# enyen/dppo

Measured on AMD Instinct MI355X. Metric: PPO-update samples/sec (+ env-steps/sec of the K=20 sampler), hopper K=20 n_envs=512, higher is better.
Workload: dtype bf16; 1 GPU; hopper-medium-v2 ft_ppo_diffusion_mlp K=20 Kft=10 Ta=4 (BASELINE configs[1]); n_envs_per_gpu=512, minibatch_per_gpu=50000, rollout_rows_per_gpu=256000, parallelism=dp1 (env-sharded, RCCL grad all-reduce)

## Files before the change

### dppo_amd/csrc/api.hip

```cpp
#include <math.h>
#include <stdarg.h>
#include <stdio.h>
#include <string.h>

#include "fused.h"
#include "gemm.h"
#include "ppo.h"
#include "gaussian.h"
#include "gmm.h"
#include "idql.h"
#include "unet.h"
#include "sampler.h"

using namespace dppo;

static thread_local char g_err[512] = "";
static int fail(int code, const char* fmt, ...) {
  va_list ap;
  va_start(ap, fmt);
  vsnprintf(g_err, sizeof(g_err), fmt, ap);
  va_end(ap);
  return code;
}
namespace dppo {
// ... 321 lines not shown
  void* a1[MAX_BLOCKS];
  void* z1[MAX_BLOCKS];
  void* a2[MAX_BLOCKS];
  void* hpre[MAX_BLOCKS + 1];
  void* hE;
  float* out;
  int ldout;
  void* d_out;
  void* dh;
  void* dz1;
  float* dtemb;
  void* cin;
  void* ca;
  void* cz;
  void* d_enc;
  void* d_cz;
  void* dh_all[MAX_BLOCKS + 1];
  void* dz1_all[MAX_BLOCKS];
  float* ln_stats;
  const void* dh0_final;
  void* w0T;
  float* dobs;
  float* tile_colsum;
  int tiles;
  float* slab;
  size_t slab_used;
  SlabJobs slab_jobs;
  GemmTNGroup tn_group;
  BwdRoute route;
  hipStream_t join_s[2];
  int join_idx[2], n_join;
  float* part;
  float* lowrank;
  float* lowrank_u;
  double* post_counter;
  unsigned* tail_counter;
  size_t slab_floats, part_floats;
};

constexpr int REDUCE_BLOCKS = 256;
constexpr int POST_COUNTER_DOUBLES = 2;

static bool lowrank_top(const dppo_net_desc& d, int64_t M);
template <class P>
static int plan_route(const dppo_net_desc& d, int64_t M, int Kft, int flags, MlpBufs<P>& B);

static int g_dbg = 0;
template <class P>
static void carve_mlp(Carver& c, const dppo_net_desc& d, int64_t M, bool keep, bool bwd, MlpBufs<P>& B) {
  const size_t ES = P::ESIZE;
  const int H = d.hidden, nb = d.n_blocks;
  const int Kp0 = row_kp0(d), Kpo = round_up(d.out_dim, 64);
  memset(&B, 0, sizeof(B));
  BwdRoute& R = B.route;
  R.onehot_col = -1, R.lowrank = lowrank_top(d, M);
  R.one_block = fused_bwd_one_block<P>(d) && d.out_dim <= 128 && R.lowrank;
  R.merged = fused_ok<P>(d) && fused_can_merge<P>(d);
  R.fused = fused_ok<P>(d) && M > 0 && fused_rows_per_tile<P>(d, R.one_block) > 0;
  B.in = c.take((size_t)M * Kp0 * ES);
  const int nh = keep ? nb + 1 : (nb > 0 ? 2 : 1);
  float* hbuf[MAX_BLOCKS + 1];
  for (int i = 0; i < nh; ++i) hbuf[i] = (float*)c.take((size_t)M * H * 4);
  for (int b = 0; b <= nb; ++b) B.h[b] = keep ? hbuf[b] : hbuf[b & 1];
  void* a1s = nullptr;
  void* a2s = nullptr;
  for (int b = 0; b < nb; ++b) {
    if (keep || b == 0) {
      a1s = c.take((size_t)M * H * ES);
      a2s = c.take((size_t)M * H * ES);
    } else if (d.plain) {
      a2s = b == 1 ? c.take((size_t)M * H * ES) : B.a2[b - 2];
    }
    B.a1[b] = a1s;
    B.a2[b] = a2s;
    B.z1[b] = keep ? c.take((size_t)M * H * ES) : nullptr;
  }
  if (d.cond_hidden > 0) {
    const int Kpc = round_up(d.cond_dim, 64), C1p = round_up(d.cond_hidden, 64), Ep = round_up(d.cond_out, 64);
    B.cin = c.take((size_t)M * Kpc * ES);
    B.ca = c.take((size_t)M * C1p * ES);
    B.cz = keep ? c.take((size_t)M * C1p * ES) : nullptr;
    if (bwd) {
      B.d_enc = c.take((size_t)M * Ep * ES);
      B.d_cz = c.take((size_t)M * C1p * ES);
    }
  }
  if (d.use_layernorm && keep) B.ln_stats = (float*)c.take((size_t)nb * 2 * M * 2 * 4);
  B.hE = c.take((size_t)M * H * ES);
  for (int b = 0; b <= nb; ++b) B.hpre[b] = b == nb ? B.hE : (keep ? c.take((size_t)M * H * ES) : nullptr);
  B.ldout = round_up(d.out_dim, 16);
  B.out = (float*)c.take((size_t)M * B.ldout * 4);
  if (bwd) {
    B.d_out = c.take((size_t)M * Kpo * ES);
    B.dh = c.take((size_t)M * H * ES);
    B.dz1 = c.take((size_t)M * H * ES);
    B.dh_all[nb] = B.dh;
    for (int b = 0; b < nb; ++b) {
      B.dh_all[b] = c.take((size_t)M * H * ES);
      B.dz1_all[b] = b == 0 ? B.dz1 : c.take((size_t)M * H * ES);
    }
    const int mt = d.plain || d.out_dim > 128 ? 0 : fused_rows_per_tile<P>(d, R.one_block);
    B.tiles = mt > 0 ? (int)((M + mt - 1) / mt) : 0;
    B.tile_colsum = (float*)c.take((size_t)(2 * nb + 2 + (d.use_layernorm ? 4 * nb : 0)) * (B.tiles > 0 ? B.tiles : 1) * H * 4);
    const int tdp = round_up(d.time_dim > 0 ? d.time_dim : 1, 16);
    B.dtemb = d.kind == 0 ? (float*)c.take((size_t)M * tdp * 4) : nullptr;
    const size_t tiles_hh = (size_t)((H + 127) / 128) * ((H + 127) / 128);
    size_t splits_hh = (512 + tiles_hh - 1) / tiles_hh;
    const size_t alt = (size_t)128 * H * (size_t)(Kp0 > 128 ? Kp0 : 128);
    B.slab_floats = (size_t)2 * (nb > 0 ? nb : 1) * splits_hh * (size_t)H * H + 2 * alt;
    B.slab = (float*)c.take(B.slab_floats * 4);
    B.slab_used = 0, B.slab_jobs.n = 0, B.tn_group.n = 0, B.n_join = 0;
    B.part_floats = (size_t)REDUCE_BLOCKS * (H > 1024 ? H : 1024);
    B.part = (float*)c.take(B.part_floats * 4);
    B.lowrank = (float*)c.take((size_t)round_up(d.out_dim, 16) * H * 4);
    B.lowrank_u = (float*)c.take((size_t)round_up(d.out_dim, 16) * Kp0 * 4);
    B.post_counter = (double*)c.take(POST_COUNTER_DOUBLES * 8);
    B.tail_counter = (unsigned*)(B.post_counter + 1);
    B.w0T = c.take((size_t)round_up(d.cond_dim > 0 ? d.cond_dim : 1, 16) * H * ES);
    B.dobs = (float*)c.take((size_t)M * round_up(d.cond_dim > 0 ? d.cond_dim : 1, 16) * 4);
    plan_route<P>(d, M, 0, 0, B);
  }
}

static void fill_bias_off(const dppo_net_desc& d, const ParamLayout& pl, int* off) {
  off[0] = (int)pl.b0;
  for (int b = 0; b < d.n_blocks; ++b) off[1 + 2 * b] = (int)pl.l1b[b], off[2 + 2 * b] = (int)pl.l2b[b];
  off[1 + 2 * d.n_blocks] = (int)pl.bout;
}
static void fill_ln_off(const dppo_net_desc& d, const ParamLayout& pl, int* off) {
  for (int b = 0; b < d.n_blocks; ++b)
    off[4 * b] = (int)pl.n1w[b], off[4 * b + 1] = (int)pl.n1b[b], off[4 * b + 2] = (int)pl.n2w[b], off[4 * b + 3] = (int)pl.n2b[b];
}

template <class P>
static void cond_encode(const dppo_net_desc& d, const float* prm, const char* pk, const PackLayout& L, int64_t M,
                        const void* cin, MlpBufs<P>& B, void* in, float* enc_f32, int ld_enc, bool keep, hipStream_t s) {
  const ParamLayout pl = param_layout(d);
  GemmNT g;
  memset(&g, 0, sizeof(g));
  g.M = (int)M, g.N = d.cond_hidden, g.Kp = L.Kpc, g.ldx = L.Kpc, g.ldw = L.Kpc, g.ldo = L.C1p, g.act = d.act;
  g.X = cin, g.W = pk + L.Wc1, g.bias = prm + pl.c1b, g.out_act = B.ca, g.out_pre = keep ? B.cz : nullptr;
  launch_gemm_nt<P>(g, s);
  if (L.C1p > round_up(d.cond_hidden, 16)) launch_zero_cols<P>(B.ca, (int)M, round_up(d.cond_hidden, 16), L.C1p, L.C1p, s);
  memset(&g, 0, sizeof(g));
  g.M = (int)M, g.N = d.cond_out, g.Kp = L.C1p, g.ldx = L.C1p, g.ldw = L.C1p;
  g.X = B.ca, g.W = pk + L.Wc2, g.bias = prm + pl.c2b;
  if (in != nullptr) g.out_pre = (char*)in + (size_t)(d.act_flat + d.time_dim) * P::ESIZE, g.ldo = L.Kp0;
  if (enc_f32 != nullptr) g.out_f32 = enc_f32, g.ldo32 = ld_enc;
  launch_gemm_nt<P>(g, s);
}

template <class P>
static void mlp_forward(const dppo_net_desc& d, const float* prm, const char* pk, const PackLayout& L, int64_t M,
                        MlpBufs<P>& B, bool keep, hipStream_t s) {
  const ParamLayout pl = param_layout(d);
  const int H = d.hidden, nb = d.n_blocks;
  if (fused_ok<P>(d)) {
    FusedFwdArgs f;
    memset(&f, 0, sizeof(f));
    f.wstream = (const u32x4*)(pk + L.sstream), f.ostream = (const u32x4*)(pk + L.ostream), f.params = prm;
    fill_bias_off(d, pl, f.bias_off);
    f.in = B.in, f.ld_in = L.Kp0, f.M = (int)M, f.Kp0 = sampler_geom<P>(d).Kp0, f.nb = nb, f.act = d.act;
    f.out_dim = d.out_dim, f.out = B.out, f.ldout = B.ldout, f.in_valid = d.in_dim;
    f.use_ln = d.use_layernorm;
    if (d.use_layernorm) fill_ln_off(d, pl, f.ln_off);
    if (keep) {
      for (int b = 0; b < nb; ++b) {
        f.a1[b] = B.a1[b], f.a2[b] = B.a2[b];
        f.z1[b] = B.z1[b], f.hpre[b] = B.hpre[b];
      }
      f.hpre[nb] = B.hE;
      f.ln_stats = d.use_layernorm ? B.ln_stats : nullptr;
    }
    if (B.route.merged) {
      f.merge_top = 1, f.ks0v = (d.in_dim + P::KB - 1) / P::KB, f.hpre[nb] = nullptr;
      if (g_dbg & 64) f.hpre[0] = nullptr;
      if (g_dbg & 128) f.a2[0] = nullptr;
      if (g_dbg & 256) f.z1[0] = nullptr;
      f.ostream0 = (const u32x4*)(pk + L.ostream0), f.ostream2 = (const u32x4*)(pk + L.ostream2);
      f.cbias2 = (const float*)(pk + L.cbias2);
    }
    g_fused_fault = launch_fused_forward<P>(d, f, s);
    return;
  }
  if (d.plain) {
    GemmNT q;
    memset(&q, 0, sizeof(q));
    q.M = (int)M, q.X = B.in, q.ldx = L.Kp0, q.W = pk + L.W0, q.ldw = L.Kp0, q.Kp = L.Kp0, q.N = H, q.bias = prm + pl.b0;
    q.ldo = H, q.act = d.act, q.out_act = B.a1[0], q.out_pre = keep ? B.hpre[0] : nullptr;
    launch_gemm_nt<P>(q, s);
    for (int b = 0; b < nb; ++b) {
      memset(&q, 0, sizeof(q));
      q.M = (int)M, q.N = H, q.Kp = H, q.ldx = H, q.ldw = H, q.ldo = H, q.act = d.act;
      q.X = b == 0 ? B.a1[0] : B.a2[b - 1], q.W = pk + L.W1[b], q.bias = prm + pl.l1b[b];
      q.out_pre = keep ? B.z1[b] : nullptr, q.out_act = B.a2[b];
      launch_gemm_nt<P>(q, s);
    }
    memset(&q, 0, sizeof(q));
    q.M = (int)M, q.N = d.out_dim, q.Kp = H, q.ldx = H, q.ldw = H;
    q.X = B.a2[nb - 1], q.W = pk + L.Wout, q.bias = prm + pl.bout, q.out_f32 = B.out, q.ldo32 = B.ldout;
    launch_gemm_nt<P>(q, s);
    return;
  }
  GemmNT g;
  memset(&g, 0, sizeof(g));
  g.M = (int)M;
  g.X = B.in, g.ldx = L.Kp0, g.W = pk + L.W0, g.ldw = L.Kp0, g.Kp = L.Kp0, g.N = H, g.bias = prm + pl.b0;
  g.out_f32 = B.h[0], g.ldo32 = H, g.ldo = H, g.act = d.act;
  g.out_act = nb > 0 ? B.a1[0] : nullptr;
  g.out_pre = nb > 0 ? nullptr : B.hE;
  launch_gemm_nt<P>(g, s);
  for (int b = 0; b < nb; ++b) {
    memset(&g, 0, sizeof(g));
    g.M = (int)M, g.N = H, g.Kp = H, g.ldx = H, g.ldw = H, g.ldo = H, g.ldo32 = H, g.act = d.act;
    g.X = B.a1[b], g.W = pk + L.W1[b], g.bias = prm + pl.l1b[b];
    g.out_pre = keep ? B.z1[b] : nullptr, g.out_act = B.a2[b];
    launch_gemm_nt<P>(g, s);
    g.X = B.a2[b], g.W = pk + L.W2[b], g.bias = prm + pl.l2b[b];
    g.res = B.h[b], g.ldres = H;
    g.out_f32 = B.h[b + 1];
    g.out_act = b + 1 < nb ? B.a1[b + 1] : nullptr;
    g.out_pre = b + 1 < nb ? nullptr : B.hE;
    launch_gemm_nt<P>(g, s);
  }
  memset(&g, 0, sizeof(g));
  g.M = (int)M, g.N = d.out_dim, g.Kp = H, g.ldx = H, g.ldw = H;
  g.X = B.hE, g.W = pk + L.Wout, g.bias = prm + pl.bout, g.out_f32 = B.out, g.ldo32 = B.ldout;
  launch_gemm_nt<P>(g, s);
}

static int g_overlap = 1;
struct SideStream {
  hipStream_t s = nullptr;
  hipEvent_t fork = nullptr, join = nullptr;
  bool ok = false;
};
static SideStream* side_stream(int idx) {
  static SideStream tab[16][3];
  int dev = 0;
  if (hipGetDevice(&dev) != hipSuccess || dev < 0 || dev >= 16) return nullptr;
  SideStream& t = tab[dev][idx];
  if (!t.ok) {
    if (hipStreamCreateWithFlags(&t.s, hipStreamNonBlocking) != hipSuccess) return nullptr;
    if (hipEventCreateWithFlags(&t.fork, hipEventDisableTiming) != hipSuccess) return nullptr;
    if (hipEventCreateWithFlags(&t.join, hipEventDisableTiming) != hipSuccess) return nullptr;
    t.ok = true;
  }
  return &t;
}
static hipStream_t fork_side(hipStream_t main, int idx = 0) {
  const int mask = g_overlap == 1 ? 7 : g_overlap >> 1;
  SideStream* t = ((mask >> idx) & 1) ? side_stream(idx) : nullptr;
  if (t == nullptr) return main;
  (void)hipEventRecord(t->fork, main);
  (void)hipStreamWaitEvent(t->s, t->fork, 0);
  return t->s;
}
static void join_side(hipStream_t main, hipStream_t sidestream, int idx = 0) {
  if (sidestream == main) return;
  SideStream* t = side_stream(idx);
  (void)hipEventRecord(t->join, sidestream);
  (void)hipStreamWaitEvent(main, t->join, 0);
}

static int g_post_one = 1;
static int g_merge_top = 1;
static int g_lowrank_top = 1;
static int g_early_join = 1;
static int g_tn_group = 1;
static int g_tn_target = 256;
static int g_tn_max_splits = 128;
static int g_lowrank_ratio = 100;
static bool lowrank_top(const dppo_net_desc& d, int64_t M) {
  return g_lowrank_top && d.n_blocks >= 1 && M >= (int64_t)g_lowrank_ratio * d.out_dim;
}
static int g_mom_rider = 0;
constexpr int64_t MOM_RIDER_MAX_N = 16384;
static int g_temb_onehot = 1;
static int g_dw0 = 1;
static int g_side_tail = 1;
static int g_tail_post = 1;
template <class P>
static int plan_route(const dppo_net_desc& d, int64_t M, int Kft, int flags, MlpBufs<P>& B) {
  BwdRoute& R = B.route;
  const bool zeroed = flags & DPPO_ROUTE_IN_ZEROED, wants_dobs = flags & DPPO_ROUTE_IN_DOBS;
  const int Kp0 = row_kp0(d);
  const bool side = flags & DPPO_ROUTE_IN_SIDE;
  const bool oh = g_temb_onehot && d.kind == 0 && fused_ok<P>(d) && Kft >= 1 && !(d.cond_out > 0 && d.cond_out % 16) &&
                  Kp0 - d.in_dim >= Kft && (size_t)(d.hidden + d.time_dim) * Kft <= B.part_floats;
  R.onehot_col = oh ? d.in_dim : -1;
  const int room = 32 - (d.kind == 0 ? d.act_flat + d.cond_dim : d.in_dim);
  const int nhot = d.kind != 0 ? 0 : (room >= Kft ? Kft : room);
  R.dw0 = g_dw0 && P::ESIZE == 2 && zeroed && !wants_dobs && d.cond_hidden <= 0 && g_tn_group && g_post_one && R.fused &&
          R.one_block && fused_dw0_shape(d) && Kp0 >= 64 &&
          (size_t)fused_bwd_one_grid<P>(d, M) * d.hidden * 32 <= B.slab_floats / 2;
  if (d.kind == 0)
    R.dw0 = R.dw0 && oh && d.in_dim == d.act_flat + d.time_dim + d.cond_dim && d.act_flat % 4 == 0 && d.time_dim % 4 == 0 &&
            32 + d.time_dim <= 64 && nhot >= Kft - 1;
  else
    R.dw0 = R.dw0 && d.in_dim <= 32;
  if (R.dw0 && (g_dbg & 33))
    return fail(-1, "tuning knob 8, bits 0 and 5 (values 1 and 32: no dh_0 store) cannot run with the in-kernel dW0: set knob 37 to 0 first");
  R.dw0_nhot = R.dw0 ? nhot : 0;
  R.dw0_round = R.dw0 && d.kind == 0 && nhot < Kft;
  R.need_aux = d.kind == 0 && !oh;
  R.aux_side = R.need_aux && side;
  R.side_tail = R.dw0 && d.kind == 0 && side && g_side_tail && g_early_join && zeroed && !(g_dbg & 28);
  R.tail_post = R.side_tail && g_tail_post;
  R.post_one = g_post_one && (!oh || zeroed) && (R.lowrank || oh || R.merged || R.one_block);
  return 0;
}
template <class P>
static void flush_slabs(MlpBufs<P>& B, hipStream_t s, const SlotOuts* slots = nullptr, int slot_width = 0,
                        const LossArgs* fin = nullptr, bool defer_reduce = false) {
  if (B.tn_group.n > 0) {
    GemmTNGroup& gr = B.tn_group;
    gemm_tn_group_order(gr);
    launch_gemm_tn_group<P>(gr, s);
    gr.n = 0;
  }
  for (int i = 0; i + 1 < B.n_join; ++i) join_side(B.join_s[B.n_join - 1], B.join_s[i], B.join_idx[i]);
  if (B.n_join > 0) join_side(s, B.join_s[B.n_join - 1], B.join_idx[B.n_join - 1]);
  B.n_join = 0;
  if (defer_reduce) return;
  if (slots != nullptr || fin != nullptr) {
    TailReduce t;
    memset(&t, 0, sizeof(t));
    t.jobs = B.slab_jobs;
    if (slots != nullptr) t.colsum = B.tile_colsum, t.tiles = B.tiles, t.width = slot_width, t.slots = *slots;
    if (g_dbg & 4) t.jobs.n = 0;
    if (g_dbg & 8) t.slots.n_slots = 0;
    if (g_dbg & 16) fin = nullptr;
    launch_tail_reduce(t, fin, s);
  } else {
    launch_slab_reduce_batch(B.slab_jobs, s);
  }
  B.slab_jobs.n = 0, B.slab_used = 0;
}
template <class P>
static void weight_grad(const void* A, int lda, int N1, const void* Bm, int ldb, int N2, int64_t M, MlpBufs<P>& B,
                        float* gw, int ldgw, hipStream_t s, bool defer = false, int n2a = -1, float* gw2 = nullptr,
                        int ldgw2 = 0) {
  const bool swap = N1 <= 64 && N2 > 64;
  if (swap) {
    const void* tp = A;
    A = Bm, Bm = tp;
    int ti = lda;
    lda = ldb, ldb = ti;
    ti = N1, N1 = N2, N2 = ti;
  }
  const bool group = defer && g_tn_group;
  const bool thin = !group && gemm_tn_thin(N1, N2);
  const size_t N1s = (size_t)round_up(N1, 4);
  const size_t tiles = thin ? (size_t)((N1 + 511) / 512) : (size_t)((N1 + 127) / 128) * ((N2 + 127) / 128);
  int64_t splits = (g_tn_target + tiles - 1) / tiles;
  const int64_t max_splits = (M + 63) / 64;
  if (splits > max_splits) splits = max_splits;
  if (splits > g_tn_max_splits) splits = g_tn_max_splits;
  if ((size_t)splits * N1s * N2 > B.slab_floats - B.slab_used || B.slab_jobs.n + 2 > MAX_SLAB_JOBS ||
      B.tn_group.n >= MAX_TN_JOBS)
    flush_slabs(B, s);
  while (splits > 1 && (size_t)splits * N1s * N2 > B.slab_floats) --splits;
  if (splits >= 8) splits = splits / 8 * 8;
  int64_t rps = (M + splits - 1) / splits;
  rps = (rps + 63) / 64 * 64;
  const int64_t need = (M + rps - 1) / rps;
  if (need < splits) splits = need >= 8 ? (need + 7) / 8 * 8 : need;
  GemmTN t;
  memset(&t, 0, sizeof(t));
  t.A = A, t.B = Bm, t.M = (int)M, t.N1 = N1, t.N2 = N2, t.lda = lda, t.ldb = ldb;
  float* sub = B.slab + B.slab_used;
  B.slab_used += (size_t)splits * N1s * N2;
  t.slab = sub, t.ldc = N2, t.splits = (int)splits, t.rows_per_split = (int)rps;
  if (group)
    B.tn_group.j[B.tn_group.n++] = t;
  else
    launch_gemm_tn<P>(t, s);
  SlabJob& j = B.slab_jobs.j[B.slab_jobs.n++];
  j.slab = sub, j.out = gw, j.splits = (int)splits, j.rows = N1, j.cols = N2, j.lds = N2, j.ldo = ldgw, j.transpose = swap ? 1 : 0;
  j.c0 = 0, j.wide = 0;
  if (n2a >= 0 && !swap) {
    j.cols = n2a;
    SlabJob& j2 = B.slab_jobs.j[B.slab_jobs.n++];
    j2 = j;
    j2.out = gw2, j2.ldo = ldgw2, j2.c0 = n2a, j2.cols = N2 - n2a;
  }
  if (!defer) flush_slabs(B, s);
}

template <class P>
static void time_embedding_grad(const dppo_net_desc& d, const float* prm, const char* pk, const PackLayout& L, int64_t M,
                                MlpBufs<P>& B, const void* dh0, float* grad, const int32_t* krow, const dppo_step* ksteps,
                                int Kft, hipStream_t s) {
  const ParamLayout pl = param_layout(d);
  const int H = d.hidden, td = d.time_dim;
  GemmNT g;
  memset(&g, 0, sizeof(g));
  g.M = (int)M, g.N = td, g.Kp = H, g.ldx = H, g.ldw = H;
  g.X = dh0, g.W = pk + L.W0tT, g.out_f32 = B.dtemb, g.ldo32 = L.tdp;
  launch_gemm_nt<P>(g, s);
  int sblocks = (int)(B.part_floats / ((size_t)Kft * td)) - 1;
  sblocks = sblocks > REDUCE_BLOCKS ? REDUCE_BLOCKS : (sblocks < 1 ? 1 : sblocks);
  launch_temb_segsum(B.dtemb, L.tdp, krow, M, Kft, td, B.part, sblocks, s);
  float* G = B.part + (size_t)sblocks * Kft * td;
  launch_slab_reduce(B.part, sblocks, (size_t)Kft * td, G, 1.f, s);
  launch_time_backward(prm + pl.te1_w, prm + pl.te1_b, prm + pl.te2_w, G, ksteps, Kft, td, grad + pl.te1_w,
                       grad + pl.te1_b, grad + pl.te2_w, grad + pl.te2_b, s);
}

template <class P>
static void cond_backward(const dppo_net_desc& d, const float* prm, const char* pk, const PackLayout& L, int64_t M,
                          MlpBufs<P>& B, const void* dh0, const void* cin, float* grad, hipStream_t s) {
  const ParamLayout pl = param_layout(d);
  const int H = d.hidden;
  GemmNT g;
  memset(&g, 0, sizeof(g));
  g.M = (int)M, g.N = d.cond_out, g.Kp = H, g.ldx = H, g.ldw = H, g.ldo = L.Ep;
  g.X = dh0, g.W = pk + L.W0eT, g.out_pre = B.d_enc;
  launch_gemm_nt<P>(g, s);
  if (L.Ep > round_up(d.cond_out, 16))
    launch_zero_cols<P>(B.d_enc, (int)M, round_up(d.cond_out, 16), L.Ep, L.Ep, s);
  weight_grad<P>(B.d_enc, L.Ep, d.cond_out, B.ca, L.C1p, d.cond_hidden, M, B, grad + pl.c2w, d.cond_hidden, s);
  launch_colsum<P>(B.d_enc, (int)M, d.cond_out, L.Ep, B.part, REDUCE_BLOCKS, grad + pl.c2b, 1.f, s);
  memset(&g, 0, sizeof(g));
  g.M = (int)M, g.N = d.cond_hidden, g.Kp = L.Ep, g.ldx = L.Ep, g.ldw = L.Ep, g.ldo = L.C1p;
  g.X = B.d_enc, g.W = pk + L.Wc2T, g.out_pre = B.d_cz, g.dsrc_kind = 2, g.dsrc_ld = L.C1p, g.dact = d.act;
  g.dsrc = d.act == DPPO_ACT_RELU ? B.ca : B.cz;
  launch_gemm_nt<P>(g, s);
  weight_grad<P>(B.d_cz, L.C1p, d.cond_hidden, cin, L.Kpc, d.cond_dim, M, B, grad + pl.c1w, d.cond_dim, s);
  launch_colsum<P>(B.d_cz, (int)M, d.cond_hidden, L.C1p, B.part, REDUCE_BLOCKS, grad + pl.c1b, 1.f, s);
// ... 673 lines not shown
  double* partial;
  const size_t need = carve_bc<P>(c, d, M, B, brow, krow, &partial);
  if ((int64_t)need > wsb) return fail(-1, "workspace too small: need %zu bytes, got %lld", need, (long long)wsb);
  if (int e = plan_route<P>(d, M, Kft, DPPO_ROUTE_IN_SIDE | (d_obs ? DPPO_ROUTE_IN_DOBS : 0), B)) return e;
  const PackLayout L = pack_layout<P>(d, 0);
  br.temb = (const float*)(pk + L.temb), br.ksteps = steps;
  br.Kft = Kft, br.AF = d.act_flat, br.td = d.time_dim, br.cond = d.cond_dim, br.M = M, br.obs_in_a = 1;
  br.inA = B.in, br.KpA = L.Kp0, br.brow = brow, br.krow = krow, br.onehot0 = B.route.onehot_col;
  if (d.cond_hidden > 0) br.obs_in_a = 0, br.inC = B.cin, br.KpC = L.Kpc;
  launch_build_rows<P>(br, s);
  if (d.cond_hidden > 0) cond_encode<P>(d, prm, pk, L, M, B.cin, B, B.in, nullptr, 0, true, s);
  mlp_forward<P>(d, prm, pk, L, M, B, true, s);
  loss(B, L, partial);
  mlp_backward<P>(d, prm, pk, L, M, B, grad, krow, steps, Kft, s);
  if (d.cond_hidden > 0) cond_backward<P>(d, prm, pk, L, M, B, B.dh0_final, B.cin, grad, s);
  if (d_obs) obs_grad<P>(d, prm, M, B, d_obs, s);
  return check_launch();
}
template <class P>
static int bc_impl(const dppo_net_desc& d, const float* prm, const char* pk, const dppo_diffusion_cfg& cfg,
                   const dppo_step* ksteps, int Kft, const float* obs, const float* chains, int64_t Bn, float* grad,
                   double* loss, void* ws, int64_t wsb, hipStream_t s) {
  const int64_t M = Bn * Kft;
  BuildRows br;
  memset(&br, 0, sizeof(br));
  br.chains = chains, br.obs = obs;
  return denoise_train<P>(d, prm, pk, br, ksteps, Kft, M, grad, nullptr, ws, wsb, s,
                          [&](MlpBufs<P>& B, const PackLayout& L, double* partial) {
                            BcArgs ba;
                            ba.eps = B.out, ba.lde = B.ldout, ba.chains = chains, ba.ksteps = ksteps, ba.cfg = cfg, ba.Kft = Kft;
                            ba.AF = d.act_flat, ba.M = M, ba.d_eps = B.d_out, ba.ldde = L.Kpo, ba.loss = loss, ba.partial = partial;
                            launch_bc_loss<P>(ba, s);
                          });
}
int dppo_bc_loss_fwd_bwd(const dppo_net_desc* actor, int prec, const float* params, const void* packed,
                         const dppo_diffusion_cfg* cfg, const dppo_step* ksteps, int Kft, const float* obs,
                         const float* chains, int64_t B, float* grad, double* loss, void* workspace,
                         int64_t workspace_bytes, dppo_stream_t stream) {
  if (int e = check_net(actor)) return e;
  if (int e = check_prec(prec)) return e;
  if (actor->kind != 0) return fail(-1, "dppo_bc_loss_fwd_bwd needs an actor descriptor");
  if (!params || !packed || !cfg || !ksteps || !obs || !chains || !grad || !loss || !workspace) return fail(-1, "null pointer");
  if (B < 1 || Kft < 1 || B * Kft > 0x7fffffff) return fail(-1, "B*Kft out of range");
  if (Kft > 1024) return fail(-1, "Kft out of range");
  if ((int64_t)Kft * actor->time_dim > 65536 || time_backward_lds_bytes(Kft, actor->time_dim) > 156 * 1024)
    return fail(-1, "Kft * time_dim = %d too large for the time-embedding backward (LDS)", Kft * actor->time_dim);
#define CALL(P)                                                                                                       \
  bc_impl<P>(*actor, params, (const char*)packed, *cfg, ksteps, Kft, obs, chains, B, grad, loss, workspace, workspace_bytes, \
             (hipStream_t)stream)
  return DPPO_DISPATCH(prec, CALL);
#undef CALL
}
int dppo_axpy(float* y, const float* x, double alpha, int64_t n, dppo_stream_t stream) {
  if (!y || !x || n < 0) return fail(-1, "bad argument");
  launch_axpy(y, x, (float)alpha, n, (hipStream_t)stream);
  return check_launch();
}

int64_t dppo_denoise_mse_workspace_bytes(const dppo_net_desc* actor, int prec, int64_t N) {
  return dppo_bc_loss_workspace_bytes(actor, prec, N, 1);
}
template <class P>
static int mse_impl(const dppo_net_desc& d, const float* prm, const char* pk, const dppo_step* tsteps, int n_time,
                    const float* obs, const float* pairs, const int64_t* kinds, int64_t M, float* grad, double* loss,
                    void* ws, int64_t wsb, hipStream_t s, float* d_obs = nullptr) {
  BuildRows br;
  memset(&br, 0, sizeof(br));
  br.kinds = kinds, br.chains = pairs, br.obs = obs;
  return denoise_train<P>(d, prm, pk, br, tsteps, n_time, M, grad, d_obs, ws, wsb, s,
                          [&](MlpBufs<P>& B, const PackLayout& L, double* partial) {
                            MseArgs ma;
                            ma.eps = B.out, ma.lde = B.ldout, ma.pairs = pairs, ma.AF = d.act_flat, ma.M = M, ma.d_eps = B.d_out;
                            ma.ldde = L.Kpo, ma.loss = loss, ma.partial = partial;
                            launch_mse_loss<P>(ma, s);
                          });
}
static int mse_entry(const dppo_net_desc* actor, int prec, const float* params, const void* packed,
                             const dppo_step* tsteps, int n_time, const float* obs, const float* pairs,
                             const int64_t* kinds, int64_t N, float* grad, double* loss, void* workspace,
                             int64_t workspace_bytes, dppo_stream_t stream, float* d_obs) {
  if (int e = check_net(actor)) return e;
  if (int e = check_prec(prec)) return e;
  if (actor->kind != 0) return fail(-1, "dppo_denoise_mse_fwd_bwd needs an actor descriptor");
  if (d_obs && actor->cond_hidden > 0) return fail(-1, "d_obs with a cond_mlp actor is not built");
  if (!params || !packed || !tsteps || !obs || !pairs || !kinds || !grad || !loss || !workspace)
    return fail(-1, "null pointer");
  if (N < 1 || N > 0x7fffffff || n_time < 1 || n_time > 1024) return fail(-1, "N / n_time out of range");
  if (time_backward_lds_bytes(n_time, actor->time_dim) > 156 * 1024)
    return fail(-1, "n_time * time_dim = %d too large for the time-embedding backward (LDS)", n_time * actor->time_dim);
#define CALL(P)                                                                                                        \
  mse_impl<P>(*actor, params, (const char*)packed, tsteps, n_time, obs, pairs, kinds, N, grad, loss, workspace, \
              workspace_bytes, (hipStream_t)stream, d_obs)
  return DPPO_DISPATCH(prec, CALL);
#undef CALL
}
int dppo_denoise_mse_fwd_bwd(const dppo_net_desc* actor, int prec, const float* params, const void* packed,
                             const dppo_step* tsteps, int n_time, const float* obs, const float* pairs,
                             const int64_t* kinds, int64_t N, float* grad, double* loss, void* workspace,
                             int64_t workspace_bytes, dppo_stream_t stream) {
  return mse_entry(actor, prec, params, packed, tsteps, n_time, obs, pairs, kinds, N, grad, loss, workspace, workspace_bytes,
                   stream, nullptr);
}
int dppo_denoise_mse_fwd_bwd_obs(const dppo_net_desc* actor, int prec, const float* params, const void* packed,
                                 const dppo_step* tsteps, int n_time, const float* obs, const float* pairs,
                                 const int64_t* kinds, int64_t N, float* grad, double* loss, void* workspace,
                                 int64_t workspace_bytes, dppo_stream_t stream, float* d_obs) {
  if (!d_obs) return fail(-1, "null pointer");
  return mse_entry(actor, prec, params, packed, tsteps, n_time, obs, pairs, kinds, N, grad, loss, workspace, workspace_bytes,
                   stream, d_obs);
}

int dppo_gae(const double* reward, const float* values, const float* terminated, const float* last_values, int n_steps,
             int n_envs, double gamma, double gae_lambda, double reward_scale_const, double* adv64, double* ret64,
             float* adv32, float* ret32, dppo_stream_t stream) {
  if (!reward || !values || !terminated || !last_values) return fail(-1, "null pointer");
  if (n_steps < 1 || n_envs < 1) return fail(-1, "empty rollout");
  launch_gae(reward, values, terminated, last_values, n_steps, n_envs, gamma, gae_lambda, reward_scale_const, adv64,
             ret64, adv32, ret32, (hipStream_t)stream);
  return check_launch();
}

template <class P>
struct PpoWs {
  MlpBufs<P> A, C;
  int32_t *brow, *krow;
  int32_t* brow_c;
  double* moments;
  float* loss_tab;
  double* loss_partial;
  double* loss_partial_v;
};
template <class P>
static size_t carve_ppo(Carver& c, const dppo_net_desc& a, const dppo_net_desc& cr, int64_t N, PpoWs<P>& W) {
  W.moments = (double*)c.take((8 + 2 * ADV_MOMENT_BLOCKS) * sizeof(double));
  W.loss_tab = (float*)c.take(2 * 1024 * sizeof(float));
  W.loss_partial = (double*)c.take((size_t)loss_blocks(N) * 8 * sizeof(double));
  W.loss_partial_v = (double*)c.take((size_t)loss_blocks(N) * 8 * sizeof(double));
  W.brow = (int32_t*)c.take((size_t)N * 4);
  W.brow_c = (int32_t*)c.take((size_t)N * 4);
  W.krow = (int32_t*)c.take((size_t)N * 4);
  carve_mlp<P>(c, a, N, true, true, W.A);
  carve_mlp<P>(c, cr, N, true, true, W.C);
  return al256(c.off);
}
int64_t dppo_ppo_workspace_bytes(const dppo_net_desc* actor, const dppo_net_desc* critic, int prec, int64_t N) {
  if (check_net(actor) || check_net(critic) || check_prec(prec)) return -1;
  if (N < 2 || N > 0x7fffffff) return fail(-1, "N out of range");
  return ws_bytes(prec, [&](Carver& c, auto p) {
    PpoWs<decltype(p)> W;
    return carve_ppo<decltype(p)>(c, *actor, *critic, N, W);
  });
}

template <class P>
static int ppo_impl(const dppo_net_desc& a, const dppo_net_desc& cr, const float* ap, const char* ak, const float* cp,
                    const char* ck, const dppo_diffusion_cfg& dcfg, const dppo_ppo_cfg& pcfg, const dppo_step* ksteps,
                    const float* obs_k, const float* chains_k, const float* returns_k, const float* values_k,
                    const float* adv_k, const float* logprobs_k, const int64_t* inds, const int64_t* kinds, int64_t N,
                    const double* gmom, float* agrad, float* cgrad, double* stats, void* ws, int64_t wsb, hipStream_t s,
                    const dppo_obs_io* oio = nullptr, const dppo_dp_hook* hook = nullptr) {
  Carver c{(char*)ws, 0, (size_t)wsb};
  PpoWs<P> W;
  const size_t need = carve_ppo<P>(c, a, cr, N, W);
  if ((int64_t)need > wsb) return fail(-1, "workspace too small: need %zu bytes, got %lld", need, (long long)wsb);
  const PackLayout LA = pack_layout<P>(a, 0), LC = pack_layout<P>(cr, 0);
  const int Kft = pcfg.ft_denoising_steps;
  const int dobs_a = oio && oio->d_obs_actor ? DPPO_ROUTE_IN_DOBS : 0, dobs_c = oio && oio->d_obs_critic ? DPPO_ROUTE_IN_DOBS : 0;
  if (int e = plan_route<P>(a, N, Kft, DPPO_ROUTE_IN_ZEROED | DPPO_ROUTE_IN_SIDE | dobs_a, W.A)) return e;
  if (int e = plan_route<P>(cr, N, Kft, DPPO_ROUTE_IN_ZEROED | dobs_c, W.C)) return e;
  const bool own_rows = a.cond_hidden == 0;
  hipStream_t s2 = own_rows ? fork_side(s) : s;
  BuildRows br;
  memset(&br, 0, sizeof(br));
  br.zero_b = W.moments, br.n_zero_b = 32;
  br.zero_a = W.A.post_counter, br.n_zero_a = POST_COUNTER_DOUBLES;
  br.zero_c = W.C.post_counter, br.n_zero_c = POST_COUNTER_DOUBLES;
  if (Kft <= 1024) br.loss_tab = W.loss_tab, br.pcfg = pcfg;
  br.inds = inds, br.kinds = kinds, br.chains = chains_k, br.obs = obs_k, br.temb = (const float*)(ak + LA.temb);
  br.ksteps = ksteps;
  br.Kft = Kft, br.AF = a.act_flat, br.td = a.time_dim, br.cond = a.cond_dim, br.M = N;
  br.inA = W.A.in, br.KpA = LA.Kp0, br.inC = W.C.in, br.KpC = LC.Kp0, br.brow = W.brow, br.krow = W.krow;
  br.obs_in_a = a.cond_hidden > 0 ? 0 : 1;
  br.onehot0 = W.A.route.onehot_col;
  const bool mom_rider = gmom == nullptr && (g_mom_rider == 1 || (g_mom_rider == 0 && N <= MOM_RIDER_MAX_N));
  if (mom_rider) br.mom_adv = adv_k, br.mom_out = W.moments, br.n_zero_b = 8;
  const float* obs_c = oio && oio->obs_critic ? oio->obs_critic : nullptr;
  const bool split = s2 != s || obs_c != nullptr;
  if (split) {
    BuildRows bc = br;
    bc.zero_a = bc.zero_b = nullptr, bc.n_zero_a = bc.n_zero_b = 0, bc.loss_tab = nullptr, bc.mom_adv = nullptr;
    br.zero_c = nullptr, br.n_zero_c = 0;
    bc.inA = nullptr, bc.brow = W.brow_c, bc.krow = nullptr;
    if (obs_c) bc.obs = obs_c;
    bc.cond = cr.cond_dim;
    launch_build_rows<P>(bc, s2);
    br.inC = nullptr;
  }
  launch_build_rows<P>(br, s);
  if (a.cond_hidden > 0) cond_encode<P>(a, ap, ak, LA, N, W.C.in, W.A, W.A.in, nullptr, 0, true, s);
  if (gmom == nullptr && !mom_rider) launch_adv_moments(adv_k, W.brow, N, W.moments, s);
  if (!own_rows) s2 = fork_side(s);
  LossArgs la;
  memset(&la, 0, sizeof(la));
  la.eps = W.A.out, la.lde = W.A.ldout, la.vnew = W.C.out, la.ldv = W.C.ldout, la.brow = W.brow, la.krow = W.krow;
  la.gathered = kinds != nullptr;
  la.chains = chains_k, la.logprobs_k = logprobs_k, la.returns_k = returns_k, la.values_k = values_k, la.adv_k = adv_k;
  la.ksteps = ksteps, la.dcfg = dcfg, la.pcfg = pcfg, la.AF = a.act_flat, la.N = N;
  la.moments = gmom ? gmom : W.moments;
  if (mom_rider) la.mom_blocks = ADV_RIDER_BLOCKS, la.moments_out = W.moments;
  la.tab = Kft <= 1024 ? W.loss_tab : nullptr;
  la.d_eps = W.A.d_out, la.ldde = LA.Kpo, la.d_v = W.C.d_out, la.lddv = LC.Kpo, la.stats = stats;
  const bool two_streams = s2 != s;
  mlp_forward<P>(cr, cp, ck, LC, N, W.C, true, s2);
  if (two_streams) {
    la.part = 2, la.partial = W.loss_partial_v;
    if (split) la.brow = W.brow_c;
    if (gmom == nullptr) la.n_count = (double)N;
    launch_ppo_loss<P>(la, s2);
    const LossArgs lv = la;
    la.brow = W.brow, la.n_count = 0;
    mlp_backward<P>(cr, cp, ck, LC, N, W.C, cgrad, nullptr, nullptr, 0, s2, &lv);
    if (oio && oio->d_obs_critic) obs_grad<P>(cr, cp, N, W.C, oio->d_obs_critic, s2);
    if (hook && hook->critic_grads_enqueued) hook->critic_grads_enqueued(hook->user, (dppo_stream_t)s2);
  }
  mlp_forward<P>(a, ap, ak, LA, N, W.A, true, s);
  la.part = two_streams ? 1 : 3, la.partial = W.loss_partial;
  launch_ppo_loss<P>(la, s);
  if (!two_streams) {
    mlp_backward<P>(cr, cp, ck, LC, N, W.C, cgrad, nullptr, nullptr, 0, s);
    if (oio && oio->d_obs_critic) obs_grad<P>(cr, cp, N, W.C, oio->d_obs_critic, s);
    if (hook && hook->critic_grads_enqueued) hook->critic_grads_enqueued(hook->user, (dppo_stream_t)s);
  }
  if (two_streams && g_early_join) W.A.join_s[W.A.n_join] = s2, W.A.join_idx[W.A.n_join++] = 0;
  mlp_backward<P>(a, ap, ak, LA, N, W.A, agrad, W.krow, ksteps, Kft, s, &la);
  if (a.cond_hidden > 0) cond_backward<P>(a, ap, ak, LA, N, W.A, W.A.dh0_final, W.C.in, agrad, s);
  if (oio && oio->d_obs_actor) obs_grad<P>(a, ap, N, W.A, oio->d_obs_actor, s);
  if (!(two_streams && g_early_join) || W.A.n_join > 0) join_side(s, s2);
  W.A.n_join = 0;
  return check_launch();
}

static bool hipStreamIsCapturing_safe(hipStream_t s) {
  hipStreamCaptureStatus st = hipStreamCaptureStatusNone;
  return hipStreamIsCapturing(s, &st) == hipSuccess && st != hipStreamCaptureStatusNone;
}
static int check_obs_io(const dppo_obs_io* io, const int64_t* kinds, bool actor_has_encoder) {
  if (!io) return 0;
  if (kinds == nullptr) return fail(-1, "the _obs entries take pre-gathered samples (kinds), one observation row per sample");
  if (actor_has_encoder && (io->obs_critic || io->d_obs_actor)) return fail(-1, "d_obs / obs_critic with a cond_mlp actor is not built");
  return 0;
}
static int ppo_entry(const dppo_net_desc* actor, const dppo_net_desc* critic, int prec, const float* actor_params,
                          const void* actor_packed, const float* critic_params, const void* critic_packed,
                          const dppo_diffusion_cfg* dcfg, const dppo_ppo_cfg* pcfg, const dppo_step* ksteps,
                          const float* obs_k, const float* chains_k, const float* returns_k, const float* values_k,
                          const float* adv_k, const float* logprobs_k, const int64_t* inds, const int64_t* kinds,
                          int64_t N, const double* global_moments, float* actor_grad, float* critic_grad,
                          double* stats, void* workspace, int64_t workspace_bytes, dppo_stream_t stream, const dppo_obs_io* io,
                          const dppo_dp_hook* hook = nullptr) {
  if (int e = check_net(actor)) return e;
  if (int e = check_net(critic)) return e;
  if (int e = check_prec(prec)) return e;
  if (actor->kind != 0 || critic->kind != 1 || critic->out_dim != 1)
    return fail(-1, "descriptor kinds must be (actor, critic with out_dim 1)");
  if (actor->cond_dim != critic->cond_dim && !(io && io->obs_critic))
    return fail(-1, "actor and critic observe different cond_dim");
  if (!actor_params || !actor_packed || !critic_params || !critic_packed || !dcfg || !pcfg || !ksteps || !obs_k ||
      !chains_k || !returns_k || !values_k || !adv_k || !logprobs_k || !actor_grad || !critic_grad || !stats ||
      !workspace)
    return fail(-1, "null pointer");
  if (int e = check_obs_io(io, kinds, actor->cond_hidden > 0)) return e;
  if ((inds == nullptr) == (kinds == nullptr)) return fail(-1, "pass exactly one of inds (rollout mode) / kinds (gathered mode)");
  if (N < 2 || N > 0x7fffffff) return fail(-1, "N out of range");
  if (pcfg->ft_denoising_steps < 1 || pcfg->ft_denoising_steps > 1024) return fail(-1, "Kft out of range");
  if ((int64_t)pcfg->ft_denoising_steps * actor->time_dim > 65536 ||
      time_backward_lds_bytes(pcfg->ft_denoising_steps, actor->time_dim) > 156 * 1024)
    return fail(-1, "Kft * time_dim too large");
  if (pcfg->horizon_steps * pcfg->action_dim != actor->act_flat) return fail(-1, "Ta*Da != act_flat");
  if (pcfg->reward_horizon < 1) return fail(-1, "reward_horizon must be >= 1");
#define CALL(P)                                                                                                        \
  ppo_impl<P>(*actor, *critic, actor_params, (const char*)actor_packed, critic_params, (const char*)critic_packed, *dcfg,     \
              *pcfg, ksteps, obs_k, chains_k, returns_k, values_k, adv_k, logprobs_k, inds, kinds, N, global_moments, actor_grad, critic_grad, stats, \
              workspace, workspace_bytes, (hipStream_t)stream, io, hook)
  return DPPO_DISPATCH(prec, CALL);
#undef CALL
}
int dppo_ppo_loss_fwd_bwd_dp(const dppo_net_desc* actor, const dppo_net_desc* critic, int prec, const float* actor_params,
                             const void* actor_packed, const float* critic_params, const void* critic_packed,
                             const dppo_diffusion_cfg* dcfg, const dppo_ppo_cfg* pcfg, const dppo_step* ksteps,
                             const float* obs_k, const float* chains_k, const float* returns_k, const float* values_k,
                             const float* adv_k, const float* logprobs_k, const int64_t* inds, const int64_t* kinds,
                             int64_t N, const double* global_moments, float* actor_grad, float* critic_grad,
                             double* stats, void* workspace, int64_t workspace_bytes, dppo_stream_t stream,
                             const dppo_dp_hook* hook) {
  if (hipStreamIsCapturing_safe((hipStream_t)stream) && hook && hook->critic_grads_enqueued)
    return fail(-1, "dppo_ppo_loss_fwd_bwd_dp: a collective cannot be queued from inside a stream capture");
  return ppo_entry(actor, critic, prec, actor_params, actor_packed, critic_params, critic_packed, dcfg, pcfg, ksteps, obs_k,
                   chains_k, returns_k, values_k, adv_k, logprobs_k, inds, kinds, N, global_moments, actor_grad, critic_grad,
                   stats, workspace, workspace_bytes, stream, nullptr, hook);
}
int dppo_ppo_loss_fwd_bwd(const dppo_net_desc* actor, const dppo_net_desc* critic, int prec, const float* actor_params,
                          const void* actor_packed, const float* critic_params, const void* critic_packed,
                          const dppo_diffusion_cfg* dcfg, const dppo_ppo_cfg* pcfg, const dppo_step* ksteps,
                          const float* obs_k, const float* chains_k, const float* returns_k, const float* values_k,
                          const float* adv_k, const float* logprobs_k, const int64_t* inds, const int64_t* kinds,
                          int64_t N, const double* global_moments, float* actor_grad, float* critic_grad,
                          double* stats, void* workspace, int64_t workspace_bytes, dppo_stream_t stream) {
  return ppo_entry(actor, critic, prec, actor_params, actor_packed, critic_params, critic_packed, dcfg, pcfg, ksteps, obs_k,
                   chains_k, returns_k, values_k, adv_k, logprobs_k, inds, kinds, N, global_moments, actor_grad, critic_grad,
                   stats, workspace, workspace_bytes, stream, nullptr);
}
int dppo_ppo_loss_fwd_bwd_obs(const dppo_net_desc* actor, const dppo_net_desc* critic, int prec, const float* actor_params,
                              const void* actor_packed, const float* critic_params, const void* critic_packed,
                              const dppo_diffusion_cfg* dcfg, const dppo_ppo_cfg* pcfg, const dppo_step* ksteps,
                              const float* obs_k, const float* chains_k, const float* returns_k, const float* values_k,
                              const float* adv_k, const float* logprobs_k, const int64_t* kinds, int64_t N,
                              const double* global_moments, float* actor_grad, float* critic_grad, double* stats,
                              void* workspace, int64_t workspace_bytes, dppo_stream_t stream, const dppo_obs_io* io) {
  if (!io) return fail(-1, "null pointer");
  return ppo_entry(actor, critic, prec, actor_params, actor_packed, critic_params, critic_packed, dcfg, pcfg, ksteps, obs_k,
                   chains_k, returns_k, values_k, adv_k, logprobs_k, nullptr, kinds, N, global_moments, actor_grad, critic_grad,
                   stats, workspace, workspace_bytes, stream, io);
}

static int check_gauss(const dppo_net_desc* actor, const dppo_gaussian_cfg* cfg, const float* logvar) {
  if (int e = check_net(actor)) return e;
  if (actor->kind != 1) return fail(-1, "the Gaussian actor is a kind-1 (observation trunk) descriptor");
  if (!cfg) return fail(-1, "null cfg");
  if (cfg->horizon_steps * cfg->action_dim != actor->out_dim) return fail(-1, "Ta*Da != actor out_dim");
  if (cfg->std_mode != 0 && cfg->std_mode != 1) return fail(-1, "std_mode must be 0 (fixed) or 1 (learned per dimension)");
  if (cfg->std_mode == 1 && !logvar) return fail(-1, "std_mode 1 needs logvar");
  if (cfg->std_mode == 0 && !(cfg->fixed_std > 0)) return fail(-1, "fixed_std must be positive");
  return 0;
}
template <class P>
static size_t carve_gauss(Carver& c, const dppo_net_desc& a, const dppo_net_desc* cr, int64_t N, bool train, MlpBufs<P>& A,
                          MlpBufs<P>& Cb, double*& moments, double*& scratch, double*& partial) {
  moments = (double*)c.take(4 * sizeof(double));
  scratch = (double*)c.take(2 * 64 * sizeof(double));
  partial = (double*)c.take((size_t)gauss_blocks(N) * (8 + a.out_dim) * sizeof(double));
  carve_mlp<P>(c, a, N, train, train, A);
  if (cr) carve_mlp<P>(c, *cr, N, train, train, Cb);
  return al256(c.off);
}
int64_t dppo_gaussian_workspace_bytes(const dppo_net_desc* actor, const dppo_net_desc* critic, int prec, int64_t N) {
  if (check_net(actor) || (critic && check_net(critic)) || check_prec(prec)) return -1;
  if (N < 1 || N > 0x7fffffff) return fail(-1, "N out of range");
  return ws_bytes(prec, [&](Carver& c, auto p) {
    MlpBufs<decltype(p)> A, Cb;
    double *m, *sc, *pa;
    return carve_gauss<decltype(p)>(c, *actor, critic, N, critic != nullptr, A, Cb, m, sc, pa);
  });
}
template <class P>
static int gauss_infer_impl(const dppo_net_desc& d, const float* prm, const char* pk, const dppo_gaussian_cfg& cfg,
                            const float* logvar, const float* obs, const float* noise, const float* actions, int64_t N,
                            float* out_actions, float* out_mean, float* out_logp, void* ws, int64_t wsb, hipStream_t s) {
  Carver c{(char*)ws, 0, (size_t)wsb};
  MlpBufs<P> A, Cb;
  double *m, *sc, *pa;
  const size_t need = carve_gauss<P>(c, d, nullptr, N, false, A, Cb, m, sc, pa);
  if (!ws || (int64_t)need > wsb) return fail(-1, "workspace too small: need %zu bytes, got %lld", need, (long long)wsb);
  const PackLayout L = pack_layout<P>(d, 0);
  launch_build_direct<P>(nullptr, nullptr, obs, nullptr, 0, 0, d.cond_dim, N, A.in, L.Kp0, s);
  mlp_forward<P>(d, prm, pk, L, N, A, false, s);
  GaussArgs g;
  memset(&g, 0, sizeof(g));
  g.cfg = cfg, g.mean_pre = A.out, g.ldm = A.ldout, g.logvar = logvar, g.N = N, g.AF = d.out_dim;
  if (out_actions) {
    g.noise = noise, g.out_actions = out_actions, g.out_mean = out_mean;
    launch_gauss_sample(g, s);
  } else {
    g.actions = actions, g.out_logp = out_logp;
    launch_gauss_logprob(g, s);
  }
  return check_launch();
}
int dppo_gaussian_sample(const dppo_net_desc* actor, int prec, const float* params, const void* packed,
                         const dppo_gaussian_cfg* cfg, const float* logvar, const float* obs, const float* noise,
                         int64_t B, float* actions, float* mean_out, void* workspace, int64_t workspace_bytes,
// ... 774 lines not shown
    return fail(-1, "Q descriptor does not pair with obs_dim=%d: in_dim=%d must be obs_dim + the action width", obs_dim, q->in_dim);
#define CALL(P)                                                                                                                  \
  idql_fwd_impl<P>(*q, q_params, (const char*)q1_packed, (const char*)q2_packed, obs, obs_dim, obs_rows, actions, N, double_q != 0, \
                   q1_out, q2_out, workspace, workspace_bytes, (hipStream_t)stream)
  return DPPO_DISPATCH(prec, CALL);
#undef CALL
}
int dppo_idql_select(const float* q1, const float* q2, const float* v, int v_per_env, const float* candidates, const float* u,
                     int64_t B, int S, int width, int mode, double h, uint64_t seed, float* actions, int32_t* idx,
                     dppo_stream_t stream) {
  if (!q1 || !candidates || !actions) return fail(-1, "null pointer");
  if (mode != 0 && mode != 1) return fail(-1, "mode must be 0 (argmax) or 1 (expectile exploration)");
  if (mode == 1 && !v) return fail(-1, "mode 1 needs v");
  if (B < 1 || S < 1 || width < 1 || B * (int64_t)S > 0x7fffffff) return fail(-1, "B, S, width out of range");
  if (!(h >= 0.0 && h <= 1.0)) return fail(-1, "critic_hyperparam tau=%g outside [0, 1]", h);
  IdqlSelect a;
  memset(&a, 0, sizeof(a));
  a.q1 = q1, a.q2 = q2, a.v = v, a.cand = candidates, a.u = u, a.B = B, a.S = S, a.AF = width, a.mode = mode;
  a.v_per_env = v_per_env ? 1 : 0, a.h = (float)h, a.seed_lo = (uint32_t)seed, a.seed_hi = (uint32_t)(seed >> 32);
  a.actions = actions, a.idx = idx;
  launch_idql_select(a, (hipStream_t)stream);
  return check_launch();
}
int dppo_polyak(float* target, const float* source, double tau, int64_t n, dppo_stream_t stream) {
  if (!target || !source) return fail(-1, "null pointer");
  if (n < 1) return fail(-1, "n out of range");
  if (!(tau >= 0.0 && tau <= 1.0)) return fail(-1, "tau=%g outside [0, 1]", tau);
  launch_polyak(target, source, (float)(1.0 - tau), (float)tau, n, (hipStream_t)stream);
  return check_launch();
}

int dppo_grad_sq_norm(const float* grad, int64_t n, double* scratch, double* out, dppo_stream_t stream) {
  if (!grad || !scratch || !out || n < 1) return fail(-1, "bad argument");
  launch_sq_norm(grad, n, scratch, out, (hipStream_t)stream);
  return check_launch();
}

int dppo_adamw_step(float* params, const float* grad, float* exp_avg, float* exp_avg_sq, int64_t n, int step, double lr,
                    double beta1, double beta2, double eps, double weight_decay, const double* sq_norm, double max_norm,
                    dppo_stream_t stream) {
  if (!params || !grad || !exp_avg || !exp_avg_sq || n < 1 || step < 1) return fail(-1, "bad argument");
  const double bc1 = 1.0 - pow(beta1, (double)step), bc2 = 1.0 - pow(beta2, (double)step);
  launch_adamw(params, grad, exp_avg, exp_avg_sq, n, (float)(1.0 - lr * weight_decay), (float)(1.0 - beta1), (float)beta2,
               (float)(1.0 - beta2), (float)(lr / bc1), (float)sqrt(bc2), (float)eps, sq_norm, (float)max_norm,
               (hipStream_t)stream);
  return check_launch();
}


int dppo_adamw_step_dev(float* params, const float* grad, float* exp_avg, float* exp_avg_sq, int64_t n, int32_t* step_dev,
                        const float* lr_dev, double beta1, double beta2, double eps, double weight_decay,
                        const double* sq_norm, double max_norm, dppo_stream_t stream) {
  if (!params || !grad || !exp_avg || !exp_avg_sq || !step_dev || !lr_dev || n < 1) return fail(-1, "bad argument");
  launch_adamw_dev(params, grad, exp_avg, exp_avg_sq, n, step_dev, lr_dev, beta1, beta2, (float)eps, weight_decay, sq_norm,
                   (float)max_norm, (hipStream_t)stream);
  return check_launch();
}

int dppo_adamw_step_multi(const dppo_adamw_slot* slots, int n_slots, dppo_stream_t stream) {
  if (!slots || n_slots < 1 || n_slots > 4) return fail(-1, "1..4 slots");
  AdamwSlots a;
  memset(&a, 0, sizeof(a));
  for (int i = 0; i < n_slots; ++i) {
    const dppo_adamw_slot& q = slots[i];
    if (!q.params || !q.grad || !q.exp_avg || !q.exp_avg_sq || !q.step_dev || !q.lr_dev || q.n < 1)
      return fail(-1, "bad argument in slot %d", i);
    AdamwSlot& t = a.s[i];
    t.p = q.params, t.g = q.grad, t.m = q.exp_avg, t.v = q.exp_avg_sq, t.n = q.n, t.step_dev = q.step_dev;
    t.lr_dev = q.lr_dev, t.beta1 = q.beta1, t.beta2 = q.beta2, t.weight_decay = q.weight_decay, t.eps = (float)q.eps;
    t.max_norm = (float)q.max_norm, t.sq_norm = q.sq_norm;
  }
  a.n = n_slots;
  launch_adamw_multi(a, (hipStream_t)stream);
  return check_launch();
}

int dppo_stats_split(const double* stats, float* hi_lo, dppo_stream_t stream) {
  if (!stats || !hi_lo) return fail(-1, "null pointer");
  launch_stats_split(stats, hi_lo, DPPO_STAT_COUNT, (hipStream_t)stream);
  return check_launch();
}
int dppo_stats_merge(const float* hi_lo, double* stats, int world, dppo_stream_t stream) {
  return dppo_stats_merge_n(hi_lo, stats, world, 2, stream);
}
int dppo_stats_merge_n(const float* hi_lo, double* stats, int world, int n_avg, dppo_stream_t stream) {
  if (!stats || !hi_lo || world < 1 || n_avg < 0 || DPPO_STAT_ADV_MEAN + n_avg > DPPO_STAT_COUNT) return fail(-1, "bad argument");
  launch_stats_merge(hi_lo, stats, DPPO_STAT_COUNT, DPPO_STAT_ADV_MEAN, n_avg, 1.0 / world, (hipStream_t)stream);
  return check_launch();
}

int dppo_probe_arm(int kernel_id, int max_launches) {
  if (probe_arm(kernel_id, max_launches)) return fail(-1, "probe already armed or bad size");
  return 0;
}
int dppo_probe_collect(double* total_ms_host, int* launches_host, double* flops_host) {
  if (!total_ms_host || !launches_host || !flops_host) return fail(-1, "null pointer");
  if (probe_collect(total_ms_host, launches_host, flops_host)) return fail(-1, "probe not armed / event error");
  return 0;
}
int dppo_probe_collect_bytes(double* total_ms_host, int* launches_host, double* flops_host, double* bytes_host) {
  if (!total_ms_host || !launches_host || !flops_host || !bytes_host) return fail(-1, "null pointer");
  if (probe_collect(total_ms_host, launches_host, flops_host, bytes_host)) return fail(-1, "probe not armed / event error");
  return 0;
}

static int retired_knob(int knob) {
  return fail(-1, "tuning knob %d is retired: the code it selected was removed (DESIGN.md section 13)", knob);
}
int dppo_tune_set(int knob, int value) {
  switch (knob) {
    case 0: set_gemm_nt_variant(value); return 0;
    case 1: g_use_fused = value; return 0;
    case 2: g_overlap = value; return 0;
    case 3:
      if (value < 1) break;
      g_tn_target = value;
      return 0;
    case 4:
      if (value < 1) break;
      g_tn_max_splits = value;
      return 0;
    case 5: set_gemm_tn_variant(value); return 0;
    case 6: set_gemm_tn_thin(value); return 0;
    case 7: set_fused_short_tiles(value); return 0;
    case 8: g_dbg = value; return 0;
    case 9: case 10: return retired_knob(knob);
    case 11: g_temb_onehot = value; return 0;
    case 12: g_tn_group = value; return 0;
    case 13: g_pack_one = value; return 0;
    case 14: g_early_join = value; return 0;
    case 15: set_sampler_l0_lds(value); return 0;
    case 16: g_lowrank_top = value; return 0;
    case 17: g_merge_top = value; return 0;
    case 18: g_post_one = value; return 0;
    case 20: dppo::set_vis_mfma_attn(value); return 0;
    case 21: set_gemm_nt_small(value); return 0;
    case 22: set_fused_merge_fwd(value); return 0;
    case 23: set_fused_bwd_one(value); return 0;
    case 25: set_fused_compact(value); return 0;
    case 26: set_gemm_tn_nbuf(value); return 0;
    case 27: set_sampler_split(value); return 0;
    case 28: set_sampler_split_pre_sweep(value); return 0;
    case 29: set_sampler_split_spin_limit(value); return 0;
    case 30:
      if (value < 1) break;
      g_lowrank_ratio = value;
      return 0;
    case 31: case 32: case 33: case 34: case 35: return retired_knob(knob);
    case 36: g_mom_rider = value; return 0;
    case 37: g_dw0 = value; return 0;
    case 38: g_side_tail = value; return 0;
    case 39: case 40: return retired_knob(knob);
    case 41: g_tail_post = value; return 0;
    default: break;
  }
  return fail(-1, "unknown tuning knob %d", knob);
}

template <class P>
static int route_mask(const dppo_net_desc& d, int64_t M, int Kft, int flags, int* mask_out) {
  Carver c{nullptr, 0, 0};
  MlpBufs<P> B;
  carve_mlp<P>(c, d, M, true, true, B);
  if (int e = plan_route<P>(d, M, Kft, flags, B)) return e;
  const BwdRoute& R = B.route;
  const bool bit[12] = {R.fused,   R.one_block,    R.lowrank,   R.merged,   R.onehot_col >= 0, R.dw0,
                        R.dw0_nhot > 0, R.dw0_round, R.need_aux, R.side_tail, R.tail_post, R.post_one};
  *mask_out = 0;
  for (int i = 0; i < 12; ++i) *mask_out |= bit[i] ? 1 << i : 0;
  return 0;
}
int dppo_backward_route(const dppo_net_desc* net, int prec, int64_t M, int Kft, int flags, int* mask_out) {
  if (int e = check_net(net)) return e;
  if (int e = check_prec(prec)) return e;
  if (!mask_out || M < 1 || M > 0x7fffffff || Kft < 0 || Kft > 1024 || (flags & ~7)) return fail(-1, "bad argument");
#define CALL(P) route_mask<P>(*net, M, Kft, flags, mask_out)
  return DPPO_DISPATCH(prec, CALL);
#undef CALL
}

int dppo_gemm_nt_raw(int prec, const void* X, const void* W, const float* bias, int64_t M, int N, int Kp, float* out_f32,
                     void* out_elem, int ldo, int act, dppo_stream_t stream) {
  if (int e = check_prec(prec)) return e;
  if (!X || !W || M < 1 || M > 0x7fffffff || N < 1) return fail(-1, "bad argument");
  const int es = prec == DPPO_PREC_F32 ? 4 : 2;
  if (Kp < 1 || (Kp * es) % 128) return fail(-1, "Kp must be a multiple of %d", 128 / es);
  if (ldo < ((N + 15) & ~15)) return fail(-1, "ldo too small");
  GemmNT g;
  memset(&g, 0, sizeof(g));
  g.X = X, g.W = W, g.bias = bias, g.M = (int)M, g.N = N, g.Kp = Kp, g.ldx = Kp, g.ldw = Kp;
  g.out_f32 = out_f32, g.ldo32 = ldo, g.out_act = out_elem, g.ldo = ldo, g.act = act;
  if (prec == DPPO_PREC_F32)
    launch_gemm_nt<F32>(g, (hipStream_t)stream);
  else
    launch_gemm_nt<BF16>(g, (hipStream_t)stream);
  return check_launch();
}

int dppo_gemm_tn_raw(int prec, const void* A, int lda, int N1, const void* B, int ldb, int N2, int64_t M,
                     int rows_per_split, float* slab, float* C, dppo_stream_t stream) {
  if (int e = check_prec(prec)) return e;
  if (!A || !B || !slab || !C || M < 1 || M > 0x7fffffff || N1 < 1 || N2 < 1) return fail(-1, "bad argument");
  if (rows_per_split < 64 || rows_per_split % 64) return fail(-1, "rows_per_split must be a multiple of 64");
  const int es = prec == DPPO_PREC_F32 ? 4 : 2;
  if (lda < N1 || ldb < N2) return fail(-1, "lda / ldb smaller than N1 / N2");
  if ((lda * es) % 16 || (ldb * es) % 16) return fail(-1, "lda and ldb must be multiples of %d", 16 / es);
  GemmTN t;
  memset(&t, 0, sizeof(t));
  t.A = A, t.B = B, t.M = (int)M, t.N1 = N1, t.N2 = N2, t.lda = lda, t.ldb = ldb, t.slab = slab, t.ldc = N2;
  t.rows_per_split = rows_per_split, t.splits = (int)((M + rows_per_split - 1) / rows_per_split);
  if (prec == DPPO_PREC_F32)
    launch_gemm_tn<F32>(t, (hipStream_t)stream);
  else
    launch_gemm_tn<BF16>(t, (hipStream_t)stream);
  launch_slab_reduce_2d(slab, t.splits, N1, N2, N2, C, N2, 1.f, (hipStream_t)stream);
  return check_launch();
}

int dppo_gemm_nt_desc_raw(int prec, const dppo_gemm_nt_desc* d, dppo_stream_t stream) {
  if (int e = check_prec(prec)) return e;
  if (!d || !d->X || !d->W) return fail(-1, "null pointer");
  if (!d->out_f32 && !d->out_pre && !d->out_act) return fail(-1, "null pointer: no output");
  if (d->M < 1 || d->M > 0x7fffffff || d->N < 1) return fail(-1, "bad argument: M / N");
  const int es = prec == DPPO_PREC_F32 ? 4 : 2;
  if (d->Kp < 1 || (d->Kp * es) % 128) return fail(-1, "Kp must be a multiple of %d", 128 / es);
  if (d->ldx < d->Kp || d->ldw < d->Kp) return fail(-1, "ldx / ldw smaller than Kp");
  if ((d->ldx * es) % 16 || (d->ldw * es) % 16) return fail(-1, "ldx and ldw must be multiples of %d", 16 / es);
  const int nst = (d->N + 15) & ~15;
  if (d->dsrc_kind < 0 || d->dsrc_kind > 2) return fail(-1, "dsrc_kind must be 0, 1 or 2");
  if (d->dsrc_kind != 0 && !d->dsrc) return fail(-1, "null pointer: dsrc");
  if (d->dsrc_kind != 0 && (d->dsrc_ld < nst || d->dsrc_ld % 4)) return fail(-1, "dsrc_ld too small or not a multiple of 4");
  if (d->res && (d->ldres < nst || d->ldres % 4)) return fail(-1, "ldres too small or not a multiple of 4");
  if (d->add && (d->ldadd < nst || d->ldadd % 4)) return fail(-1, "ldadd too small or not a multiple of 4");
  if (d->out_f32 && (d->ldo32 < nst || d->ldo32 % 4)) return fail(-1, "ldo32 too small or not a multiple of 4");
  if ((d->out_pre || d->out_act) && (d->ldo < nst || d->ldo % 4)) return fail(-1, "ldo too small or not a multiple of 4");
  if (d->act < 0 || d->act > ACT_NONE || d->dact < 0 || d->dact > ACT_NONE) return fail(-1, "act / dact must be 0, 1 or 2");
  GemmNT g;
  memset(&g, 0, sizeof(g));
  g.X = d->X, g.W = d->W, g.bias = d->bias, g.M = (int)d->M, g.N = d->N, g.Kp = d->Kp, g.ldx = d->ldx, g.ldw = d->ldw;
  g.dsrc = d->dsrc_kind ? d->dsrc : nullptr, g.dsrc_kind = d->dsrc_kind, g.dsrc_ld = d->dsrc_ld, g.dact = d->dact;
  g.res = d->res, g.ldres = d->ldres, g.add = d->add, g.ldadd = d->ldadd;
  g.out_f32 = d->out_f32, g.ldo32 = d->ldo32, g.out_pre = d->out_pre, g.out_act = d->out_act, g.ldo = d->ldo, g.act = d->act;
  if (prec == DPPO_PREC_F32)
    launch_gemm_nt<F32>(g, (hipStream_t)stream);
  else
    launch_gemm_nt<BF16>(g, (hipStream_t)stream);
  return check_launch();
}

static int tn_job_checked(const dppo_gemm_tn_job& j, int es, GemmTN& t) {
  if (!j.A || !j.B || !j.slab) return fail(-1, "null pointer");
  if (j.M < 1 || j.M > 0x7fffffff || j.N1 < 1 || j.N2 < 1) return fail(-1, "bad argument: M / N1 / N2");
  if (j.rows_per_split < 64 || j.rows_per_split % 64) return fail(-1, "rows_per_split must be a multiple of 64");
  if (j.lda < 1 || j.ldb < 1 || (j.lda * es) % 16 || (j.ldb * es) % 16)
    return fail(-1, "lda and ldb must be multiples of %d", 16 / es);
  if (j.ncol_a < 0 || j.ncol_b < 0 || (j.ncol_a * es) % 16 || (j.ncol_b * es) % 16)
    return fail(-1, "ncol_a and ncol_b must be multiples of %d", 16 / es);
  if ((j.ncol_a > 0 ? j.ncol_a : j.lda) < j.N1 || (j.ncol_b > 0 ? j.ncol_b : j.ldb) < j.N2)
    return fail(-1, "lda / ldb (ncol_a / ncol_b) smaller than N1 / N2");
  memset(&t, 0, sizeof(t));
  t.A = j.A, t.B = j.B, t.M = (int)j.M, t.N1 = j.N1, t.N2 = j.N2, t.lda = j.lda, t.ldb = j.ldb, t.slab = j.slab, t.ldc = j.N2;
  t.rows_per_split = j.rows_per_split, t.splits = (int)((j.M + j.rows_per_split - 1) / j.rows_per_split);
  t.ncol_a = j.ncol_a, t.ncol_b = j.ncol_b;
  return 0;
}

int dppo_gemm_tn_group_raw(int prec, const dppo_gemm_tn_job* jobs, int n, float* const* C_out, dppo_stream_t stream) {
  if (int e = check_prec(prec)) return e;
  if (!jobs || !C_out) return fail(-1, "null pointer");
  if (n < 1 || n > MAX_TN_JOBS) return fail(-1, "n must be 1..%d", MAX_TN_JOBS);
  const int es = prec == DPPO_PREC_F32 ? 4 : 2;
  GemmTNGroup gr;
  memset(&gr, 0, sizeof(gr));
  for (int i = 0; i < n; ++i) {
    if (!C_out[i]) return fail(-1, "null pointer: C_out[%d]", i);
    if (int e = tn_job_checked(jobs[i], es, gr.j[i])) return e;
  }
  gr.n = n;
  gemm_tn_group_order(gr);
  if (prec == DPPO_PREC_F32)
    launch_gemm_tn_group<F32>(gr, (hipStream_t)stream);
  else
    launch_gemm_tn_group<BF16>(gr, (hipStream_t)stream);
  for (int i = 0; i < n; ++i) {
    const dppo_gemm_tn_job& j = jobs[i];
    const int splits = (int)((j.M + j.rows_per_split - 1) / j.rows_per_split);
    launch_slab_reduce_2d(j.slab, splits, j.N1, j.N2, j.N2, C_out[i], j.N2, 1.f, (hipStream_t)stream);
  }
  return check_launch();
}

int dppo_gemm_tn_job_raw(int prec, const dppo_gemm_tn_job* job, float* C, dppo_stream_t stream) {
  if (int e = check_prec(prec)) return e;
  if (!job || !C) return fail(-1, "null pointer");
  GemmTN t;
  if (int e = tn_job_checked(*job, prec == DPPO_PREC_F32 ? 4 : 2, t)) return e;
  if (prec == DPPO_PREC_F32)
    launch_gemm_tn<F32>(t, (hipStream_t)stream);
  else
    launch_gemm_tn<BF16>(t, (hipStream_t)stream);
  launch_slab_reduce_2d(t.slab, t.splits, t.N1, t.N2, t.N2, C, t.N2, 1.f, (hipStream_t)stream);
  return check_launch();
}
```

### dppo_amd/csrc/fused.h

```cpp
#pragma once
#include "common.h"
#include "sampler.h"

namespace dppo {

struct FusedGeom {
  int KSB0;
  int KpB0;
  int total_pos;
  size_t frags_per_wave;
};
template <class P>
FusedGeom fused_geom(const dppo_net_desc& d);

struct FusedFwdArgs {
  const u32x4* wstream;
  const u32x4* ostream;
  const float* params;
  int bias_off[2 + 2 * MAX_BLOCKS];
  int ln_off[4 * MAX_BLOCKS];
  int use_ln;
  float* ln_stats;
  const void* in;
  int ld_in;
  int M, Kp0, nb, act, out_dim;
  int in_valid;
  int consts_lds;
  void* a1[MAX_BLOCKS];
  void* a2[MAX_BLOCKS];
  void* z1[MAX_BLOCKS];
  void* hpre[MAX_BLOCKS + 1];
  float* out;
  int ldout;
  int merge_top, ks0v;
  const u32x4* ostream0;
  const u32x4* ostream2;
  const float* cbias2;
};

struct FusedBwdArgs {
  const u32x4* bstream;
  const void* d_out;
  int ld_dout;
  int M, KpB0, nb, act;
  int out_valid;
  const float* params;
  int ln_off[4 * MAX_BLOCKS];
  int use_ln;
  const float* ln_stats;
  const void* m1[MAX_BLOCKS];
  const void* m0[MAX_BLOCKS];
  void* dh[MAX_BLOCKS + 1];
  void* dz1[MAX_BLOCKS];
  float* colsum;
  int dout_slot;
  int dbg;
  int one_block;
  float* dw0_slab;
  const void* xc;
  int ld_xc, xc_af, xc_skip, dw0_round;
};
template <class P>
int fused_bwd_one_grid(const dppo_net_desc& d, int64_t M);
bool fused_dw0_shape(const dppo_net_desc& d);

template <class P>
int launch_fused_forward(const dppo_net_desc& d, const FusedFwdArgs& a, hipStream_t s);
template <class P>
int launch_fused_backward(const dppo_net_desc& d, const FusedBwdArgs& a, hipStream_t s);
void set_fused_short_tiles(int v);
void set_fused_merge_fwd(int v);
template <class P>
bool fused_can_merge(const dppo_net_desc& d);
template <class P>
int fused_rows_per_tile(const dppo_net_desc& d, bool one_block = false);
template <class P>
bool fused_bwd_one_block(const dppo_net_desc& d);
void set_fused_bwd_one(int v);
void set_fused_compact(int v);

struct PackLayer {
  const float* W;
  u32x4* stream;
  int rs, cs;
  int in_valid, KS, pos0;
  int total_pos;
};
inline PackLayer pack_layer(const float* W, int rs, int cs, int in_valid, int KS, int pos0, u32x4* stream, int total_pos) {
  PackLayer L;
  L.W = W, L.stream = stream, L.rs = rs, L.cs = cs, L.in_valid = in_valid, L.KS = KS, L.pos0 = pos0, L.total_pos = total_pos;
  return L;
}
struct PackStream {
  PackLayer layer[2 * (1 + 2 * MAX_BLOCKS)];
  int n_layers, TPW;
};
template <class P>
void launch_pack_stream(const PackStream& d, hipStream_t s);

struct SlotOuts {
  float* out[6 * MAX_BLOCKS + 2];
  int n[6 * MAX_BLOCKS + 2];
  int n_slots;
};
void launch_reduce_slots(const float* in, int tiles, int n, const SlotOuts& o, hipStream_t s);

}
```

### dppo_amd/csrc/fused.hip

```cpp
#include <type_traits>

#include "fused.h"
#include "gemm.h"
#include "tile_ln.h"
#include "pack_dev.h"

#ifndef DPPO_BWD_LATE
#define DPPO_BWD_LATE 1
#endif
#ifndef DPPO_BWD_PREFETCH
#define DPPO_BWD_PREFETCH 1
#endif
#ifndef DPPO_FLAGS
#define DPPO_FLAGS 1
#endif

namespace dppo {

#ifdef DPPO_STAMPS
__device__ unsigned long long g_stamps[8][32];
#define STAMP(i)                                                                   \
  do {                                                                             \
    if (blockIdx.x == 0 && lane == 0 && tile == (int)gridDim.x) g_stamps[wid][i] = clock64(); \
  } while (0)
#else
#define STAMP(i) \
  do {           \
  } while (0)
#endif

namespace {

typedef __attribute__((address_space(3))) uint32_t lds_u32;
__device__ __forceinline__ uint32_t flag_load(lds_u32* f) {
  return (uint32_t)__builtin_amdgcn_readfirstlane((int)__hip_atomic_load(f, __ATOMIC_RELAXED, __HIP_MEMORY_SCOPE_WORKGROUP));
}

__device__ __forceinline__ int kmask16(int rb) {
  const int n = rb >> 4;
  const int p = n & (-n);
  return (p > 16 ? 16 : p) - 1;
}

template <int TPW, int MR>
constexpr int ring_depth() {
  return (TPW >= 8 || TPW * MR > 16) ? 2 : 4;
}

template <int MT>
__device__ __forceinline__ void load_tile(char* dst, int rb, int km, const char* src, int ld_bytes, int row0, int M) {
  const int nch = rb >> 4, vch = ld_bytes >> 4;
  int t0 = threadIdx.x;
  asm volatile("" : "+v"(t0));
  for (int q = t0; q < MT * nch; q += 512) {
    const int row = q / nch, c = q - row * nch;
    const int grow = row0 + row;
    u32x4 v = (u32x4){0, 0, 0, 0};
    if (c < vch && grow < M) v = *(const u32x4*)(src + (size_t)grow * ld_bytes + c * 16);
    *(u32x4*)(dst + row * rb + ((c ^ (row & km)) << 4)) = v;
  }
}

template <class P, int TPW, int MR, int PD>
struct Engine {
  u32x4 ring[PD][TPW];
  const u32x4* stream;
  int total, pos;

  __device__ __forceinline__ void prime(const u32x4* s, int total_pos, int pos0 = 0) {
    stream = s;
    total = total_pos;
    pos = pos0;
#pragma unroll
    for (int p = 0; p < PD; ++p)
#pragma unroll
      for (int tp = 0; tp < TPW; ++tp) ring[p][tp] = s[((size_t)(pos0 + p) * TPW + tp) * 64];
  }
  __device__ __forceinline__ void run(f32x4 (&acc)[TPW][MR], const char* src, int rb, int km, int nks, int r, int g,
                                      lds_u32* flags = nullptr, uint32_t need = 0) {
    uint32_t ready = 0xffu;
    const int kpp_shift = 28 - __builtin_clz((unsigned)(nks | 8));
    if (flags != nullptr) {
      ready = 0;
#pragma unroll
      for (int i = 0; i < 8; ++i)
        if ((int32_t)(flag_load(flags + i) - need) >= 0) ready |= 1u << i;
      asm volatile("" ::: "memory");
    }
    for (int k0 = 0; k0 < nks; k0 += PD) {
      if (ready != 0xffu) {
        const int p_lo = k0 >> kpp_shift, p_hi = (k0 + PD - 1) >> kpp_shift;
        const uint32_t grp = ((2u << p_hi) - 1u) & ~((1u << p_lo) - 1u);
        if (grp & ~ready) {
          for (int p = p_lo; p <= p_hi; ++p)
            while ((int32_t)(flag_load(flags + p) - need) < 0) __builtin_amdgcn_s_sleep(1);
          ready |= grp;
          asm volatile("" ::: "memory");
        }
      }
#pragma unroll
      for (int p = 0; p < PD; ++p) {
        const int ks = k0 + p;
        u32x4 xb[MR];
#pragma unroll
        for (int m = 0; m < MR; ++m) xb[m] = *(const u32x4*)(src + (16 * m + r) * rb + (((ks * 4 + g) ^ (r & km)) << 4));
#pragma unroll
        for (int tp = 0; tp < TPW; ++tp)
#pragma unroll
          for (int m = 0; m < MR; ++m) acc[tp][m] = P::mma(ring[p][tp], xb[m], acc[tp][m]);
        int np = pos + ks + PD;
        np = np < total ? np : np - total;
        const u32x4* w = stream + (size_t)np * TPW * 64;
#pragma unroll
        for (int tp = 0; tp < TPW; ++tp) ring[p][tp] = w[tp * 64];
      }
    }
    pos += nks;
    if (pos >= total) pos -= total;
  }
};

__device__ __forceinline__ void hand_over(lds_u32* flags, int wid, int lane, uint32_t seq) {
  asm volatile("" ::: "memory");
  if (lane == 0) __hip_atomic_store(flags + wid, seq, __ATOMIC_RELAXED, __HIP_MEMORY_SCOPE_WORKGROUP);
  asm volatile("" ::: "memory");
}

template <class P, int TPW, int MR, int S1, int KSH, int S2, bool AUX = false>
struct CEngine {
  static constexpr int PD = 4, T = S1 + KSH + S2, HOLES = (PD - T % PD) % PD, TT = T + HOLES;
  static_assert(KSH % PD == 0 && KSH >= 2 * PD && S1 >= 1 && S1 <= PD && S2 >= 0 && S2 <= PD && T >= PD, "CEngine layout");
  u32x4 ring[PD][TPW];
  const u32x4* stream;
  const u32x4* aux;
  int aux_stride;
  unsigned ln;
  int p1, pl, p2;

  template <int SLOT, int N>
  __device__ __forceinline__ void fetch_ct() {
    unsigned ln = this->ln;
    asm volatile("" : "+v"(ln));
    if constexpr (N < S1 + KSH || (N < T && !(AUX && S2 > 0))) {
      const int q = N < S1 ? p1 + N : (N < S1 + KSH ? pl + (N - S1) : p2 + (N - S1 - KSH));
      const u32x4* w = stream + (size_t)q * TPW * 64;
#pragma unroll
      for (int tp = 0; tp < TPW; ++tp) ring[SLOT][tp] = (w + tp * 64)[ln];
    } else if constexpr (N < T) {
      const u32x4* w = aux + (size_t)((N - S1 - KSH) * TPW) * aux_stride;
#pragma unroll
      for (int tp = 0; tp < TPW; ++tp) ring[SLOT][tp] = (w + (size_t)tp * aux_stride)[ln];
    }
  }
  template <int SLOT, int C>
  __device__ __forceinline__ void refill_ct() {
    fetch_ct<SLOT, (C + PD >= TT ? C + PD - TT : C + PD)>();
  }
  template <int SLOT>
// ... 352 lines not shown
  Engine<P, TPW, MR, PD> eng;
  eng.prime(a.wstream + (size_t)wid * total * TPW * 64 + lane, total);

  const int ntiles = (M + MT - 1) / MT;
  for (int tile = blockIdx.x; tile < ntiles; tile += gridDim.x) {
    const int row0 = tile * MT;
    STAMP(0);
    load_tile<MT>(xin, in_rb, in_km, (const char*)a.in, a.ld_in * ES, row0, M);
    __syncthreads();
    STAMP(1);

    f32x4 h[TPW][MR], acc[TPW][MR];
    auto bias_init = [&](int layer) {
      const float* srcL = biasL + layer * H;
      const float* srcG = a.params + a.bias_off[layer];
#pragma unroll
      for (int tp = 0; tp < TPW; ++tp) {
        f32x4 b;
        if (bias_lds) {
          b = lds_load((const f32x4*)(srcL + wbase + feat_off<P>(g, tp)));
        } else {
#pragma unroll
          for (int e = 0; e < 4; ++e) b[e] = glb_load(srcG + wbase + feat_off<P>(g, tp) + e);
        }
#pragma unroll
        for (int m = 0; m < MR; ++m) acc[tp][m] = b;
      }
    };
    auto put_block_input = [&](int b) {
      if constexpr (LN) {
        if (a.hpre[b] != nullptr) emit<P, TPW, MR>(h, ACT_NONE, nullptr, a.hpre[b], H, wbase, g, r, row0, M);
        float mean[MR], rstd[MR];
        ln_forward<P, TPW, MR>(h, acc, a.params + a.ln_off[4 * b], a.params + a.ln_off[4 * b + 1], H, wbase, g, r, wid,
                               lnred, mean, rstd);
        if (a.ln_stats != nullptr && wid == 0 && g == 0) {
#pragma unroll
          for (int m = 0; m < MR; ++m)
            if (row0 + 16 * m + r < M)
              *(float2*)(a.ln_stats + (((size_t)(2 * b) * M) + row0 + 16 * m + r) * 2) = make_float2(mean[m], rstd[m]);
        }
        emit<P, TPW, MR>(acc, ACT, bufA, a.a1[b], H, wbase, g, r, row0, M);
      } else {
        emit<P, TPW, MR>(h, ACT, bufA, a.a1[b], H, wbase, g, r, row0, M, a.hpre[b]);
      }
    };
    bias_init(0);
    eng.run(acc, xin, in_rb, in_km, KS0, r, g);
    STAMP(2);
#pragma unroll
    for (int tp = 0; tp < TPW; ++tp)
#pragma unroll
      for (int m = 0; m < MR; ++m) h[tp][m] = acc[tp][m];
    if (nb > 0)
      put_block_input(0);
    else
      emit<P, TPW, MR>(h, ACT_NONE, bufA, a.hpre[0], H, wbase, g, r, row0, M);
    STAMP(3);
    if (FLAGS && nb > 0)
      hand_over(flags, wid, lane, ++seq);
    else
      __syncthreads();
    STAMP(4);
    for (int b = 0; b < nb; ++b) {
      bias_init(1 + 2 * b);
      eng.run(acc, bufA, HRB, 15, KSH, r, g, FLAGS ? flags : nullptr, seq);
      STAMP(5);
      if constexpr (LN) {
        if (a.z1[b] != nullptr) emit<P, TPW, MR>(acc, ACT_NONE, nullptr, a.z1[b], H, wbase, g, r, row0, M);
        float mean[MR], rstd[MR];
        ln_forward<P, TPW, MR>(acc, acc, a.params + a.ln_off[4 * b + 2], a.params + a.ln_off[4 * b + 3], H, wbase, g, r,
                               wid, lnred, mean, rstd);
        if (a.ln_stats != nullptr && wid == 0 && g == 0) {
#pragma unroll
          for (int m = 0; m < MR; ++m)
            if (row0 + 16 * m + r < M)
              *(float2*)(a.ln_stats + (((size_t)(2 * b + 1) * M) + row0 + 16 * m + r) * 2) = make_float2(mean[m], rstd[m]);
        }
      }
      emit<P, TPW, MR>(acc, ACT, bufB, a.a2[b], H, wbase, g, r, row0, M, LN ? nullptr : a.z1[b]);
      STAMP(6);
      if constexpr (FLAGS)
        hand_over(flags, wid, lane, ++seq);
      else
        __syncthreads();
      STAMP(7);
      bias_init(2 + 2 * b);
      eng.run(acc, bufB, HRB, 15, KSH, r, g, FLAGS ? flags : nullptr, seq);
      STAMP(8);
#pragma unroll
      for (int tp = 0; tp < TPW; ++tp)
#pragma unroll
        for (int m = 0; m < MR; ++m) h[tp][m] += acc[tp][m];
      if (b + 1 < nb)
        put_block_input(b + 1);
      else
        emit<P, TPW, MR>(h, ACT_NONE, bufA, a.hpre[nb], H, wbase, g, r, row0, M);
      STAMP(9);
      if (FLAGS && b + 1 < nb)
        hand_over(flags, wid, lane, ++seq);
      else
        __syncthreads();
      STAMP(10);
    }
    int r_ = r, g_ = g, lane_ = lane;
    asm volatile("" : "+v"(r_), "+v"(g_), "+v"(lane_));
    auto out_items = [&](auto from_lds) {
      const int r = r_, g = g_, lane = lane_;
      const u32x4* os = a.ostream + lane;
      for (int it = wid; it < MR * OT * KSPLIT; it += SAMPLER_WAVES) {
        const int m = it % MR, to = (it / MR) % OT, kh = it / (MR * OT);
        f32x4 oacc = (f32x4){0.f, 0.f, 0.f, 0.f};
#pragma unroll 8
        for (int c = 0; c < KPER; ++c) {
          const int ks = kh * KPER + c;
          u32x4 wf;
          if constexpr (decltype(from_lds)::value)
            wf = woutL[(ks * OT + to) * 64 + lane];
          else
            wf = os[(size_t)(ks * OT + to) * 64];
          const u32x4 xb = *(const u32x4*)(bufA + (16 * m + r) * HRB + (((ks * 4 + g) ^ (r & 15)) << 4));
          oacc = P::mma(wf, xb, oacc);
        }
#pragma unroll
        for (int e = 0; e < 4; ++e) part[(((kh * MR + m) * OT + to) * 16 + 4 * g + e) * 16 + r] = oacc[e];
      }
    };
    if (wout_lds)
      out_items(std::true_type{});
    else
      out_items(std::false_type{});
    STAMP(11);
    __syncthreads();
    STAMP(12);
    int tid_ = tid;
    asm volatile("" : "+v"(tid_));
    for (int idx = tid_; idx < MT * a.out_dim; idx += 512) {
      const int row = idx / a.out_dim, j = idx - row * a.out_dim;
      const int m = row >> 4, rr = row & 15, to = j >> 4, jj = j & 15;
      float s;
      if (bias_lds)
        s = lds_load(biasL + (1 + 2 * nb) * H + j);
      else
        s = glb_load(a.params + a.bias_off[1 + 2 * nb] + j);
#pragma unroll
      for (int kh = 0; kh < KSPLIT; ++kh) s += part[(((kh * MR + m) * OT + to) * 16 + jj) * 16 + rr];
      if (row0 + row < M) a.out[(size_t)(row0 + row) * a.ldout + j] = s;
    }
    STAMP(13);
    __syncthreads();
    STAMP(14);
  }
}

template <class P, int TPW, int MR, int OT, int ACT, int S1>
__device__ __forceinline__ void fused_forward_merged_body(const FusedFwdArgs& a) {
  constexpr int PD = ring_depth<TPW, MR>(), ES = P::ESIZE, KB = P::KB;
  static_assert(S1 == 0 || PD == 4, "the compact walk is written for a ring of four positions");
  constexpr int H = 128 * TPW, KSH = H / KB, HRB = H * ES, MT = 16 * MR;
  constexpr bool WIDE = OT > 1;
  constexpr int KSPLIT = WIDE ? SAMPLER_WAVES / OT : (MR * OT >= 8 ? 1 : 8 / (MR * OT));
  constexpr int KPER = KSH / KSPLIT, NITEMS = MR * OT * KSPLIT, NI = (NITEMS + SAMPLER_WAVES - 1) / SAMPLER_WAVES;
  constexpr int S2 = WIDE ? KPER / TPW : 0;
  static_assert(!WIDE || (S1 > 0 && SAMPLER_WAVES % OT == 0 && KPER % TPW == 0 && S2 >= 1 && S2 <= 4), "wide merged head: layout");
  constexpr bool FLAGS = DPPO_FLAGS;
  extern __shared__ __attribute__((aligned(16))) char smem[];
  const int tid = threadIdx.x, lane = tid & 63;
  const int wid = __builtin_amdgcn_readfirstlane(tid >> 6);
  const int r = lane & 15, g = lane >> 4;
  const int Kp0 = a.Kp0, M = a.M, ks0v = a.ks0v;
  const int in_rb = WIDE ? ks0v * 64 : Kp0 * ES, in_km = kmask16(in_rb), KS0 = Kp0 / KB;
  const int total = KS0 + 2 * KSH;
  char* bufA = smem;
  char* bufB = bufA + MT * HRB;
  float* part = (float*)bufA;
  static_assert(KSPLIT * MR * OT * 16 * 16 * 4 <= MT * HRB, "out-layer partials must fit in buffer A");
  lds_u32* flags = (lds_u32*)(bufB + MT * HRB);
  float* biasL = (float*)(bufB + MT * HRB + 64);
  u32x4* woutL = (u32x4*)(biasL + ((2 * H + OT * 16 + 3) & ~3));
  u32x4* w0cL = woutL + (WIDE ? 0 : KSH * OT * 64);
  char* xin = WIDE ? (char*)(w0cL + ks0v * OT * 64) : bufB;
  const int wbase = wid * 16 * TPW;
  const int to_w = wid % OT, kh_w = wid / OT;
  for (int idx = tid; idx < 2 * H; idx += 512) biasL[idx] = a.params[a.bias_off[idx / H] + idx % H];
  for (int idx = tid; idx < OT * 16; idx += 512) biasL[2 * H + idx] = idx < a.out_dim ? a.cbias2[idx] : 0.f;
  if constexpr (!WIDE)
    for (int idx = tid; idx < KSH * OT * 64; idx += 512) woutL[idx] = a.ostream2[idx];
  for (int idx = tid; idx < ks0v * OT * 64; idx += 512) w0cL[idx] = a.ostream0[idx];
  if (tid < 16) flags[tid] = 0;
  uint32_t seq = 0;

  typename std::conditional<(S1 > 0), CEngine<P, TPW, MR, (S1 > 0 ? S1 : 1), KSH, S2, WIDE>, Engine<P, TPW, MR, PD>>::type eng;
  if constexpr (S1 > 0) {
    if constexpr (WIDE) eng.set_aux(a.ostream2 + ((size_t)(kh_w * KPER) * OT + to_w) * 64, OT * 64);
    eng.prime(a.wstream + (size_t)wid * total * TPW * 64, lane, 0, KS0, 0);
  } else {
    eng.prime(a.wstream + (size_t)wid * total * TPW * 64 + lane, total - KSH);
  }

  const int ntiles = (M + MT - 1) / MT;
  for (int tile = blockIdx.x; tile < ntiles; tile += gridDim.x) {
    const int row0 = tile * MT;
    STAMP(0);
    load_tile<MT>(xin, in_rb, in_km, (const char*)a.in, a.ld_in * ES, row0, M);
    __syncthreads();
    STAMP(1);
    f32x4 acc[TPW][MR];
    auto bias_init = [&](int layer) {
#pragma unroll
      for (int tp = 0; tp < TPW; ++tp) {
        const f32x4 b = *(const f32x4*)(biasL + layer * H + wbase + feat_off<P>(g, tp));
#pragma unroll
        for (int m = 0; m < MR; ++m) acc[tp][m] = b;
      }
    };
    bias_init(0);
    if constexpr (S1 > 0)
      eng.short1(acc, xin, in_rb, in_km, r, g);
    else
      eng.run(acc, xin, in_rb, in_km, KS0, r, g);
    STAMP(2);
    f32x4 o1[WIDE ? 1 : NI];
    if constexpr (!WIDE) {
#pragma unroll
      for (int i = 0; i < NI; ++i) {
        const int it = wid + SAMPLER_WAVES * i;
        o1[i] = (f32x4){0.f, 0.f, 0.f, 0.f};
        if (it < MR * OT) {
          const int m = it % MR, to = it / MR;
          for (int ks = 0; ks < ks0v; ++ks) {
            const u32x4 xb = *(const u32x4*)(xin + (16 * m + r) * in_rb + (((ks * 4 + g) ^ (r & in_km)) << 4));
            o1[i] = P::mma(w0cL[(ks * OT + to) * 64 + lane], xb, o1[i]);
          }
        }
      }
    }
    emit<P, TPW, MR>(acc, ACT, bufA, a.a1[0], H, wbase, g, r, row0, M, a.hpre[0]);
    STAMP(3);
    if constexpr (FLAGS)
      hand_over(flags, wid, lane, ++seq);
    else
      __syncthreads();
    STAMP(4);
    bias_init(1);
    if constexpr (S1 > 0) {
      eng.wide(acc, bufA, HRB, 15, r, g, FLAGS ? flags : nullptr, seq);
      if constexpr (!WIDE) eng.end_tile();
    } else {
      eng.run(acc, bufA, HRB, 15, KSH, r, g, FLAGS ? flags : nullptr, seq);
    }
    STAMP(5);
    emit<P, TPW, MR>(acc, ACT, bufB, a.a2[0], H, wbase, g, r, row0, M, a.z1[0]);
    STAMP(6);
    __syncthreads();
    STAMP(7);
    int r_ = r, g_ = g, lane_ = lane;
    asm volatile("" : "+v"(r_), "+v"(g_), "+v"(lane_));
    if constexpr (WIDE) {
      f32x4 ow[MR];
#pragma unroll
      for (int m = 0; m < MR; ++m) ow[m] = (f32x4){0.f, 0.f, 0.f, 0.f};
      if (kh_w == 0) {
        for (int ks = 0; ks < ks0v; ++ks) {
          const u32x4 wf = w0cL[(ks * OT + to_w) * 64 + lane_];
#pragma unroll
          for (int m = 0; m < MR; ++m) {
            const u32x4 xb = *(const u32x4*)(xin + (16 * m + r_) * in_rb + (((ks * 4 + g_) ^ (r_ & in_km)) << 4));
            ow[m] = P::mma(wf, xb, ow[m]);
          }
        }
      }
      if constexpr (S1 > 0) {
        eng.aux_all(ow, bufB, HRB, 15, kh_w * KPER, r_, g_);
        eng.end_tile();
      }
#pragma unroll
      for (int m = 0; m < MR; ++m)
#pragma unroll
        for (int e = 0; e < 4; ++e) part[(((kh_w * MR + m) * OT + to_w) * 16 + 4 * g_ + e) * 16 + r_] = ow[m][e];
    } else
#pragma unroll
    for (int i = 0; i < NI; ++i) {
      const int it = wid + SAMPLER_WAVES * i;
      if (it < NITEMS) {
        const int m = it % MR, to = (it / MR) % OT, kh = it / (MR * OT);
        f32x4 oacc = o1[i];
#pragma unroll 8
        for (int c = 0; c < KPER; ++c) {
          const int ks = kh * KPER + c;
          const u32x4 xb = *(const u32x4*)(bufB + (16 * m + r_) * HRB + (((ks * 4 + g_) ^ (r_ & 15)) << 4));
          oacc = P::mma(woutL[(ks * OT + to) * 64 + lane_], xb, oacc);
        }
#pragma unroll
        for (int e = 0; e < 4; ++e) part[(((kh * MR + m) * OT + to) * 16 + 4 * g_ + e) * 16 + r_] = oacc[e];
      }
    }
    STAMP(11);
    __syncthreads();
    STAMP(12);
    int tid_ = tid;
    asm volatile("" : "+v"(tid_));
    for (int idx = tid_; idx < MT * a.out_dim; idx += 512) {
      const int row = idx / a.out_dim, j = idx - row * a.out_dim;
      const int m = row >> 4, rr = row & 15, to = j >> 4, jj = j & 15;
      float s = biasL[2 * H + j];
#pragma unroll
      for (int kh = 0; kh < KSPLIT; ++kh) s += part[(((kh * MR + m) * OT + to) * 16 + jj) * 16 + rr];
      if (row0 + row < M)
        a.out[(size_t)(row0 + row) * a.ldout + j] = s;
    }
    STAMP(13);
    __syncthreads();
    STAMP(14);
  }
}

template <class P, int TPW, int MR, int OT, int ACT, int S1>
__global__ __launch_bounds__(512, 2) void fused_forward_merged_kernel(const FusedFwdArgs a) {
  fused_forward_merged_body<P, TPW, MR, OT, ACT, S1>(a);
}

template <class P, int TPW, int MR, bool LN, int ACT, int OCC>
__global__ __launch_bounds__(512, 2 * OCC) void fused_backward_kernel(const FusedBwdArgs a) {
  constexpr int ES = P::ESIZE, KB = P::KB;
  constexpr bool FETCH_LATE = OCC > 1 || (DPPO_BWD_LATE && TPW * MR >= 16 && ES == 2 && !LN);
  constexpr int PD = (FETCH_LATE && OCC == 1) ? 4 : 2;
  constexpr int H = 128 * TPW, KSH = H / KB, HRB = H * ES, MT = 16 * MR;
  extern __shared__ __attribute__((aligned(16))) char smem[];
  const int tid = threadIdx.x, lane = tid & 63;
  const int wid = __builtin_amdgcn_readfirstlane(tid >> 6);
  constexpr bool FLAGS = !LN && DPPO_FLAGS;
#ifndef DPPO_NO_SETPRIO
  if (!FLAGS && wid >= 4) __builtin_amdgcn_s_setprio(1);
#endif
  const int r = lane & 15, g = lane >> 4;
  const int nb = a.nb, M = a.M;
  const int in_rb = a.KpB0 * ES, in_km = kmask16(in_rb), KSB0 = a.KpB0 / KB;
  const int total = nb >= 1 ? 2 * KSB0 + (2 * nb - 1) * KSH : KSB0;
  char* bufA = smem;
  char* bufB = bufA + MT * HRB;
  char* xin = bufB;
  lds_u32* flags = (lds_u32*)(bufB + MT * HRB);
  float* lnred = (float*)(bufB + MT * HRB + 64);
  constexpr int DRED_COLS = 128;
  float* dred = lnred + (LN ? LN_WAVES * 2 * MR * 16 : 0);
  const int wbase = wid * 16 * TPW;
  const int ntiles = (M + MT - 1) / MT;

  Engine<P, TPW, MR, PD> eng;
  eng.prime(a.bstream + (size_t)wid * total * TPW * 64 + lane, total);
  if (tid < 16) flags[tid] = 0;
  uint32_t seq = 0;

  auto colsum = [&](const f32x4 (&v)[TPW][MR], int slot, int tile) {
#pragma unroll
    for (int tp = 0; tp < TPW; ++tp) {
      f32x4 s = v[tp][0];
#pragma unroll
      for (int m = 1; m < MR; ++m) s += v[tp][m];
#pragma unroll
      for (int e = 0; e < 4; ++e) {
        s[e] = row16_sum(s[e]);
      }
      if (r == 0) *(f32x4*)(a.colsum + ((size_t)slot * ntiles + tile) * H + wbase + feat_off<P>(g, tp)) = s;
    }
  };
  auto colsum1 = [&](const f32x4 (&v)[TPW], int slot, int tile) {
#pragma unroll
    for (int tp = 0; tp < TPW; ++tp) {
      f32x4 s = v[tp];
#pragma unroll
      for (int e = 0; e < 4; ++e) {
        s[e] = row16_sum(s[e]);
      }
      if (r == 0) *(f32x4*)(a.colsum + ((size_t)slot * ntiles + tile) * H + wbase + feat_off<P>(g, tp)) = s;
    }
  };
  auto load_stats = [&](int which, int row0, float (&mean)[MR], float (&rstd)[MR]) {
#pragma unroll
    for (int m = 0; m < MR; ++m) {
      const int grow = row0 + 16 * m + r;
      const float2 st = *(const float2*)(a.ln_stats + ((size_t)which * M + (grow < M ? grow : M - 1)) * 2);
      mean[m] = st.x, rstd[m] = st.y;
    }
  };

  for (int tile = blockIdx.x; tile < ntiles; tile += gridDim.x) {
    const int row0 = tile * MT;
    STAMP(16);
    load_tile<MT>(xin, in_rb, in_km, (const char*)a.d_out, a.ld_dout * ES, row0, M);
    __syncthreads();
    STAMP(17);
    if (a.dout_slot >= 0) {
      typedef typename P::elem_t E;
      for (int c = lane; c < a.out_valid; c += 64) {
        const int cb = c * ES;
        float t = 0.f;
        for (int row = wid; row < MT; row += SAMPLER_WAVES)
          t += P::to_f32(*(const E*)(xin + row * in_rb + ((((cb >> 4) ^ (row & in_km)) << 4) | (cb & 15))));
        dred[wid * DRED_COLS + c] = t;
      }
    }
    f32x4 dh[TPW][MR], acc[TPW][MR];
    auto zero_acc = [&]() {
#pragma unroll
      for (int tp = 0; tp < TPW; ++tp)
#pragma unroll
        for (int m = 0; m < MR; ++m) acc[tp][m] = (f32x4){0.f, 0.f, 0.f, 0.f};
    };
    zero_acc();
    eng.run(acc, xin, in_rb, in_km, KSB0, r, g);
    STAMP(18);
#pragma unroll
    for (int tp = 0; tp < TPW; ++tp)
#pragma unroll
      for (int m = 0; m < MR; ++m) dh[tp][m] = acc[tp][m];
    emit<P, TPW, MR>(dh, ACT_NONE, nb >= 1 ? nullptr : bufA, a.dh[nb], H, wbase, g, r, row0, M);
    STAMP(19);
    colsum(dh, 0, tile);
    STAMP(20);
    auto dout_sums = [&]() {
      if (a.dout_slot >= 0 && tid < a.out_valid) {
        float t = 0.f;
#pragma unroll
        for (int w = 0; w < SAMPLER_WAVES; ++w) t += dred[w * DRED_COLS + tid];
        a.colsum[((size_t)a.dout_slot * ntiles + tile) * H + tid] = t;
      }
    };
    const bool defer_sums = FLAGS && nb >= 1;
    if (!defer_sums) {
      __syncthreads();
      dout_sums();
    }
    STAMP(21);
    char* pa = bufA;
    char* pb = bufB;
    for (int b = nb - 1; b >= 0; --b) {
      const bool top = b == nb - 1;
      u32x4 d[MR][Chunks<P, TPW>::CH];
      if constexpr (!FETCH_LATE) fetch<P, ACT == ACT_RELU && !LN, TPW>(d, a.m1[b], H, wbase, g, r, row0, M);
      zero_acc();
      eng.run(acc, top ? xin : pa, top ? in_rb : HRB, top ? in_km : 15, top ? KSB0 : KSH, r, g,
              FLAGS && !top ? flags : nullptr, seq);
      if constexpr (FETCH_LATE) fetch<P, ACT == ACT_RELU && !LN, TPW>(d, a.m1[b], H, wbase, g, r, row0, M);
      STAMP(22);
      if constexpr (LN) {
        float mean[MR], rstd[MR];
        f32x4 dga[TPW], dbe[TPW];
        load_stats(2 * b + 1, row0, mean, rstd);
        ln_backward<P, TPW, MR>(acc, d, a.params + a.ln_off[4 * b + 2], a.params + a.ln_off[4 * b + 3], mean, rstd, ACT, H,
                                wbase, g, r, wid, lnred, dga, dbe);
        const int ls = (2 * nb + 1) + 4 * (nb - 1 - b);
        colsum1(dga, ls + 2, tile);
        colsum1(dbe, ls + 3, tile);
      } else {
#pragma unroll
        for (int tp = 0; tp < TPW; ++tp)
#pragma unroll
          for (int m = 0; m < MR; ++m)
#pragma unroll
            for (int e = 0; e < 4; ++e) acc[tp][m][e] *= grad_at<P, ACT>(d, tp, m, e);
      }
      if (top) {
        char* t = pa;
        pa = pb, pb = t;
      }
      emit<P, TPW, MR>(acc, ACT_NONE, pb, a.dz1[b], H, wbase, g, r, row0, M);
      STAMP(23);
      colsum(acc, (nb + 1) + (nb - 1 - b), tile);
      STAMP(24);
      if constexpr (FLAGS)
        hand_over(flags, wid, lane, ++seq);
// ... 214 lines not shown
        for (int e = 0; e < 4; ++e) acc[tp][m][e] *= grad_at<P, ACT>(d, tp, m, e);
    if constexpr (COMPACT) {
      eng.short2(acc, xin, in_rb, in_km, r, g);
      eng.end_tile();
    } else {
      eng.run(acc, xin, in_rb, in_km, KSB0, r, g);
    }
    if constexpr (PF) {
      if (tile + (int)gridDim.x < ntiles) {
        tile_prefetch(tile + gridDim.x);
        warm_rows(a.m1[0], tile + gridDim.x);
      }
    }
    if constexpr (DW0) {
      dw0_accumulate<TPW, MR, DW0 == 2>(acc, stage_w, xw, cacc, lane, a.xc_af, a.xc_skip);
    } else {
      emit<P, TPW, MR>(acc, ACT_NONE, nullptr, a.dh[0], H, wbase, g, r, row0, M);
    }
    STAMP(27);
    colsum(acc, 1, tile);
    STAMP(28);
    __syncthreads();
    STAMP(29);
  }
  if constexpr (DW0) {
    float* sl = a.dw0_slab + (size_t)blockIdx.x * H * 32;
#pragma unroll
    for (int i = 0; i < TPW * 2; ++i) {
      const f32x4 c = cacc[i * 64 + lane];
#pragma unroll
      for (int e = 0; e < 4; ++e) sl[(size_t)(wbase + 16 * (i >> 1) + 4 * g + e) * 32 + 16 * (i & 1) + r] = c[e];
    }
  }
}

#ifdef DPPO_STAMPS
extern "C" int dppo_debug_stamps(unsigned long long* out) {
  return (int)hipMemcpyFromSymbol(out, HIP_SYMBOL(g_stamps), sizeof(unsigned long long) * 8 * 32);
}
#endif

static int g_short_tiles = 0;
void set_fused_short_tiles(int v) { g_short_tiles = v; }
template <class P>
static bool short_tiles(int hidden, int ln, int bit) {
  return P::ESIZE == 2 && hidden == 512 && !ln && ((g_short_tiles >> bit) & 1);
}
template <class P>
static int pick_mr(int hidden) {
  const int tpw = hidden / 128;
  if (hidden % 128) return 0;
  if (P::ESIZE == 2) return tpw == 2 ? 8 : (tpw == 4 ? 4 : (tpw == 8 ? 2 : 0));
  return tpw == 2 ? 4 : (tpw == 4 ? 2 : (tpw == 8 ? 1 : 0));
}
template <class P>
static int pick_mr_bwd(int hidden, int ln) {
  if (short_tiles<P>(hidden, ln, 0)) return 2;
  if (P::ESIZE == 2 && hidden == 256 && !ln && ((g_short_tiles >> 3) & 1)) return 2;
  int mr = pick_mr<P>(hidden);
  if (hidden >= 1024 && mr > 1) mr /= 2;
  if (P::ESIZE == 2 && hidden == 256) mr /= 2;
  if (ln && mr > 1) mr /= 2;
  return mr;
}
static int g_bwd_one = 1;
void set_fused_bwd_one(int v) { g_bwd_one = v; }
template <class P>
bool fused_bwd_one_block(const dppo_net_desc& d) {
  return g_bwd_one && !d.plain && !d.use_layernorm && d.n_blocks == 1 && d.hidden % 128 == 0 && d.hidden <= 1024 &&
         pick_mr<P>(d.hidden) > 0;
}
template bool fused_bwd_one_block<F32>(const dppo_net_desc&);
template bool fused_bwd_one_block<BF16>(const dppo_net_desc&);
template <class P>
int fused_rows_per_tile(const dppo_net_desc& d, bool one_block) {
  return 16 * (one_block ? pick_mr<P>(d.hidden) : pick_mr_bwd<P>(d.hidden, d.use_layernorm));
}
template int fused_rows_per_tile<F32>(const dppo_net_desc&, bool);
template int fused_rows_per_tile<BF16>(const dppo_net_desc&, bool);

template <class P>
FusedGeom fused_geom(const dppo_net_desc& d) {
  FusedGeom g;
  const int pd = sampler_pd(d.hidden);
  g.KpB0 = round_up(round_up(d.out_dim, 64), pd * P::KB);
  g.KSB0 = g.KpB0 / P::KB;
  g.total_pos = d.n_blocks >= 1 ? 2 * g.KSB0 + (2 * d.n_blocks - 1) * (d.hidden / P::KB) : g.KSB0;
  g.frags_per_wave = (size_t)g.total_pos * (d.hidden / 128);
  return g;
}
template FusedGeom fused_geom<F32>(const dppo_net_desc&);
template FusedGeom fused_geom<BF16>(const dppo_net_desc&);

constexpr int NUM_CUS = 256;

template <class K>
static void raise_lds(K kern, DevLatch& done) {
  if (done.need()) {
    (void)hipFuncSetAttribute((const void*)kern, hipFuncAttributeMaxDynamicSharedMemorySize, 160 * 1024);
    done.done();
  }
}

template <class P, int TPW, int MR, int OT, bool LN, int ACT, int OCC = 1>
static int launch_fwd_cfg(const FusedFwdArgs& a, hipStream_t s) {
  constexpr int ES = P::ESIZE, MT = 16 * MR, H = 128 * TPW;
  size_t lds = 2 * (size_t)MT * H * ES + 64 + (LN ? (size_t)LN_WAVES * MR * 16 * 4 : 0);
  constexpr size_t cap = 160 * 1024 / OCC;
  if (lds > cap || a.Kp0 > H) return -2;
  FusedFwdArgs b = a;
  const size_t bias_bytes = ((size_t)((1 + 2 * a.nb) * H + OT * 16 + 3) & ~(size_t)3) * 4;
  const size_t wout_bytes = (size_t)(H / P::KB) * OT * 64 * 16;
  b.consts_lds = 0;
  if (lds + bias_bytes <= cap) {
    b.consts_lds |= 1, lds += bias_bytes;
    if (lds + wout_bytes <= cap) b.consts_lds |= 2, lds += wout_bytes;
  }
  static DevLatch attr;
  raise_lds(fused_forward_kernel<P, TPW, MR, OT, LN, ACT, OCC>, attr);
  const int ntiles = (a.M + MT - 1) / MT;
  const bool probe = probe_begin(PROBE_FUSED_FWD, s);
  hipLaunchKernelGGL((fused_forward_kernel<P, TPW, MR, OT, LN, ACT, OCC>),
                     dim3(ntiles < NUM_CUS * OCC ? ntiles : NUM_CUS * OCC), dim3(512), lds, s, b);
  if (probe) probe_end(s, 2.0 * a.M * ((double)a.in_valid * H + 2.0 * a.nb * H * H + (double)H * a.out_dim));
  return 0;
}

template <class P>
static size_t merged_lds(int hidden, int out_tiles, int ks0v) {
  const int mr = pick_mr<P>(hidden);
  return 2 * (size_t)16 * mr * hidden * P::ESIZE + 64 + (((size_t)2 * hidden + out_tiles * 16 + 3) & ~(size_t)3) * 4 +
         ((size_t)(out_tiles > 1 ? 0 : hidden / P::KB) + ks0v) * out_tiles * 64 * 16 +
         (out_tiles > 1 ? (size_t)16 * mr * ks0v * 64 : 0);
}
static int g_merge_fwd = 1;
static int g_merge_wide = 1;
void set_fused_merge_fwd(int v) { g_merge_fwd = v & 1, g_merge_wide = (v & 2) ? 0 : 1; }
int fused_compact_on();
static int round_up_i(int x, int m) { return (x + m - 1) / m * m; }
template <class P>
bool fused_can_merge(const dppo_net_desc& d) {
  if (!g_merge_fwd || d.plain || d.use_layernorm || d.n_blocks != 1 || d.hidden % 128 || pick_mr<P>(d.hidden) == 0) return false;
  const int ks0v = (d.in_dim + P::KB - 1) / P::KB;
  if (d.out_dim > 16) {
    constexpr int PD = 4;
    return g_merge_wide && fused_compact_on() && d.out_dim <= 64 && d.hidden == 512 && ks0v >= 1 && ks0v <= 3 &&
           round_up_i(d.in_dim, PD * P::KB) / P::KB >= ks0v && merged_lds<P>(d.hidden, 4, ks0v) <= 160 * 1024;
  }
  return d.hidden <= 512 && merged_lds<P>(d.hidden, 1, ks0v) <= 160 * 1024;
}
template bool fused_can_merge<F32>(const dppo_net_desc&);
template bool fused_can_merge<BF16>(const dppo_net_desc&);

template <class P, int TPW, int MR, int ACT, int S1, int OT = 1>
static int launch_fwd_merged_cfg2(const FusedFwdArgs& a, hipStream_t s) {
  constexpr int MT = 16 * MR, H = 128 * TPW;
  const size_t lds = merged_lds<P>(H, OT, a.ks0v);
  if (lds > 160 * 1024 || a.Kp0 > H || a.nb != 1) return -2;
  static DevLatch attr;
  const int ntiles = (a.M + MT - 1) / MT;
  raise_lds(fused_forward_merged_kernel<P, TPW, MR, OT, ACT, S1>, attr);
  const bool probe = probe_begin(PROBE_FUSED_FWD, s);
  hipLaunchKernelGGL((fused_forward_merged_kernel<P, TPW, MR, OT, ACT, S1>), dim3(ntiles < NUM_CUS ? ntiles : NUM_CUS), dim3(512),
                     lds, s, a);
  if (probe) probe_end(s, 2.0 * a.M * ((double)a.in_valid * H + 2.0 * a.nb * H * H + (double)H * a.out_dim));
  return 0;
}
template <class P, int TPW, int MR, int ACT>
static int launch_fwd_merged_cfg(const FusedFwdArgs& a, hipStream_t s) {
  if (a.out_dim > 16) {
    if constexpr (TPW == 4) {
      if (a.ks0v == 1) return launch_fwd_merged_cfg2<P, TPW, MR, ACT, 1, 4>(a, s);
      if (a.ks0v == 2) return launch_fwd_merged_cfg2<P, TPW, MR, ACT, 2, 4>(a, s);
      if (a.ks0v == 3) return launch_fwd_merged_cfg2<P, TPW, MR, ACT, 3, 4>(a, s);
    }
    return -1;
  }
  if constexpr (ring_depth<TPW, MR>() == 4) {
    if (fused_compact_on() && a.ks0v == 1) return launch_fwd_merged_cfg2<P, TPW, MR, ACT, 1>(a, s);
    if (fused_compact_on() && a.ks0v == 2) return launch_fwd_merged_cfg2<P, TPW, MR, ACT, 2>(a, s);
  }
  return launch_fwd_merged_cfg2<P, TPW, MR, ACT, 0>(a, s);
}

template <class P>
int launch_fused_forward(const dppo_net_desc& d, const FusedFwdArgs& a, hipStream_t s) {
  const int tpw = d.hidden / 128, mr = pick_mr<P>(d.hidden);
  const int nt = (d.out_dim + 15) / 16, ot = nt <= 1 ? 1 : (nt <= 4 ? 4 : (nt <= 8 ? 8 : 0));
  if (mr == 0 || ot == 0 || a.M <= 0) return -1;
  const bool relu = a.act == ACT_RELU;
  if (a.merge_top) {
#define DPPO_FWDM(T, R) \
  if (tpw == T && mr == R) return relu ? launch_fwd_merged_cfg<P, T, R, ACT_RELU>(a, s) : launch_fwd_merged_cfg<P, T, R, ACT_MISH>(a, s);
    if constexpr (P::ESIZE == 2) {
      DPPO_FWDM(2, 8) DPPO_FWDM(4, 4)
    } else {
      DPPO_FWDM(2, 4) DPPO_FWDM(4, 2)
    }
#undef DPPO_FWDM
    return -1;
  }
  if constexpr (P::ESIZE == 2) {
    if (short_tiles<P>(d.hidden, a.use_ln, 1) && ot == 1)
      return relu ? launch_fwd_cfg<P, 4, 2, 1, false, ACT_RELU, 2>(a, s) : launch_fwd_cfg<P, 4, 2, 1, false, ACT_MISH, 2>(a, s);
    if (d.hidden == 256 && !a.use_ln && ot == 1 && ((g_short_tiles >> 2) & 1))
      return relu ? launch_fwd_cfg<P, 2, 4, 1, false, ACT_RELU, 2>(a, s) : launch_fwd_cfg<P, 2, 4, 1, false, ACT_MISH, 2>(a, s);
  }
#define DPPO_FWD(T, R, O) \
  if (tpw == T && mr == R && ot == O)                                                                                  \
    return a.use_ln ? (relu ? launch_fwd_cfg<P, T, R, O, true, ACT_RELU>(a, s) : launch_fwd_cfg<P, T, R, O, true, ACT_MISH>(a, s)) \
                    : (relu ? launch_fwd_cfg<P, T, R, O, false, ACT_RELU>(a, s) : launch_fwd_cfg<P, T, R, O, false, ACT_MISH>(a, s));
  if constexpr (P::ESIZE == 2) {
    DPPO_FWD(2, 8, 1) DPPO_FWD(2, 8, 4) DPPO_FWD(4, 4, 1) DPPO_FWD(4, 4, 4) DPPO_FWD(8, 2, 1) DPPO_FWD(8, 2, 4)
    DPPO_FWD(2, 8, 8) DPPO_FWD(4, 4, 8) DPPO_FWD(8, 2, 8)
  } else {
    DPPO_FWD(2, 4, 1) DPPO_FWD(2, 4, 4) DPPO_FWD(4, 2, 1) DPPO_FWD(4, 2, 4) DPPO_FWD(8, 1, 1) DPPO_FWD(8, 1, 4)
    DPPO_FWD(2, 4, 8) DPPO_FWD(4, 2, 8) DPPO_FWD(8, 1, 8)
  }
#undef DPPO_FWD
  return -1;
}
template int launch_fused_forward<F32>(const dppo_net_desc&, const FusedFwdArgs&, hipStream_t);
template int launch_fused_forward<BF16>(const dppo_net_desc&, const FusedFwdArgs&, hipStream_t);

template <class P, int TPW, int MR, bool LN, int ACT, int OCC = 1>
static int launch_bwd_cfg(const FusedBwdArgs& a, hipStream_t s) {
  constexpr int ES = P::ESIZE, MT = 16 * MR, H = 128 * TPW;
  const size_t lds = 2 * (size_t)MT * H * ES + 64 + (LN ? (size_t)LN_WAVES * 2 * MR * 16 * 4 : 0) + SAMPLER_WAVES * 128 * 4;
  if (lds > 160 * 1024 / OCC || a.KpB0 > H || a.KpB0 > 128) return -2;
  static DevLatch attr;
  raise_lds(fused_backward_kernel<P, TPW, MR, LN, ACT, OCC>, attr);
  const int ntiles = (a.M + MT - 1) / MT;
  const bool probe = probe_begin(PROBE_FUSED_BWD, s);
  hipLaunchKernelGGL((fused_backward_kernel<P, TPW, MR, LN, ACT, OCC>), dim3(ntiles < NUM_CUS * OCC ? ntiles : NUM_CUS * OCC),
                     dim3(512), lds, s, a);
  if (probe) probe_end(s, 2.0 * a.M * ((double)a.out_valid * H + 2.0 * a.nb * H * H));
  return 0;
}

static int g_compact = 1;
void set_fused_compact(int v) { g_compact = v; }
int fused_compact_on() { return g_compact; }
static size_t bwd_one_dw0_lds(int MT, int H) {
  return (size_t)MT * H * 2 + (size_t)MT * 64 + 64 + SAMPLER_WAVES * 32 * 4 + (size_t)MT * 128 + SAMPLER_WAVES * 2048 +
         (size_t)SAMPLER_WAVES * (H / 128) * 2 * 64 * 16;
}
template <class P, int TPW, int MR, int ACT, bool COMPACT, int DW0 = 0>
static int launch_bwd_one_cfg2(const FusedBwdArgs& a, hipStream_t s) {
  constexpr int ES = P::ESIZE, MT = 16 * MR, H = 128 * TPW;
  const size_t lds = DW0 ? bwd_one_dw0_lds(MT, H) : 2 * (size_t)MT * H * ES + 64 + SAMPLER_WAVES * 128 * 4;
  if (lds > 160 * 1024 || a.KpB0 > H || a.KpB0 > 128 || a.nb != 1) return -2;
  if ((DW0 != 0) != (a.dw0_slab != nullptr) || (DW0 == 2) != (a.dw0_round != 0)) return -4;
  if (DW0 && (a.xc == nullptr || a.ld_xc < 64 || a.ld_xc % 8 || a.xc_af % 4 || a.xc_skip % 4 || a.xc_skip < 0 || a.dh[0] != nullptr ||
              32 + a.xc_skip > 64 || a.out_valid > 32))
    return -4;
  static DevLatch attr;
  raise_lds(fused_backward_one_kernel<P, TPW, MR, ACT, COMPACT, DW0>, attr);
  const int ntiles = (a.M + MT - 1) / MT;
  const bool probe = probe_begin(PROBE_FUSED_BWD, s);
  hipLaunchKernelGGL((fused_backward_one_kernel<P, TPW, MR, ACT, COMPACT, DW0>), dim3(ntiles < NUM_CUS ? ntiles : NUM_CUS),
                     dim3(512), lds, s, a);
  if (probe) probe_end(s, 2.0 * a.M * ((double)a.out_valid * H + 2.0 * a.nb * H * H));
  return 0;
}
template <class P, int TPW, int MR, int ACT>
static int launch_bwd_one_cfg(const FusedBwdArgs& a, hipStream_t s) {
  if constexpr (ring_depth<TPW, MR>() == 4) {
    if constexpr (P::ESIZE == 2) {
      if (a.dw0_slab != nullptr)
        return !(g_compact && a.out_valid <= P::KB) ? -4
               : a.dw0_round                        ? launch_bwd_one_cfg2<P, TPW, MR, ACT, true, 2>(a, s)
                                                    : launch_bwd_one_cfg2<P, TPW, MR, ACT, true, 1>(a, s);
    }
    if (a.dw0_slab != nullptr) return -4;
    if (g_compact && a.out_valid <= P::KB) return launch_bwd_one_cfg2<P, TPW, MR, ACT, true>(a, s);
  }
  return launch_bwd_one_cfg2<P, TPW, MR, ACT, false>(a, s);
}

template <class P>
int fused_bwd_one_grid(const dppo_net_desc& d, int64_t M) {
  const int mt = 16 * pick_mr<P>(d.hidden);
  if (mt <= 0 || M <= 0) return 0;
  const int64_t ntiles = (M + mt - 1) / mt;
  return (int)(ntiles < NUM_CUS ? ntiles : NUM_CUS);
}
template int fused_bwd_one_grid<F32>(const dppo_net_desc&, int64_t);
template int fused_bwd_one_grid<BF16>(const dppo_net_desc&, int64_t);
bool fused_dw0_shape(const dppo_net_desc& d) {
  if (!g_compact || !fused_bwd_one_block<BF16>(d) || d.out_dim > BF16::KB || (d.hidden != 512 && d.hidden != 256)) return false;
  return bwd_one_dw0_lds(16 * pick_mr<BF16>(d.hidden), d.hidden) <= 160 * 1024;
}
template <class P>
int launch_fused_backward(const dppo_net_desc& d, const FusedBwdArgs& a, hipStream_t s) {
  const bool relu = a.act == ACT_RELU;
  if (a.one_block) {
    const int t = d.hidden / 128, q = pick_mr<P>(d.hidden);
    if (a.M <= 0) return -1;
#define DPPO_BWD1(T, R) \
  if (t == T && q == R) return relu ? launch_bwd_one_cfg<P, T, R, ACT_RELU>(a, s) : launch_bwd_one_cfg<P, T, R, ACT_MISH>(a, s);
    if constexpr (P::ESIZE == 2) {
      DPPO_BWD1(2, 8) DPPO_BWD1(4, 4) DPPO_BWD1(8, 2)
    } else {
      DPPO_BWD1(2, 4) DPPO_BWD1(4, 2) DPPO_BWD1(8, 1)
    }
#undef DPPO_BWD1
    return -1;
  }
  const int tpw = d.hidden / 128, mr = pick_mr_bwd<P>(d.hidden, a.use_ln);
  if (mr == 0 || a.M <= 0) return -1;
  if constexpr (P::ESIZE == 2) {
    if (short_tiles<P>(d.hidden, a.use_ln, 0))
      return relu ? launch_bwd_cfg<P, 4, 2, false, ACT_RELU, 2>(a, s) : launch_bwd_cfg<P, 4, 2, false, ACT_MISH, 2>(a, s);
    if (d.hidden == 256 && !a.use_ln && ((g_short_tiles >> 3) & 1))
      return relu ? launch_bwd_cfg<P, 2, 2, false, ACT_RELU, 2>(a, s) : launch_bwd_cfg<P, 2, 2, false, ACT_MISH, 2>(a, s);
  }
#define DPPO_BWD(T, R, L) \
  if (tpw == T && mr == R && (a.use_ln != 0) == L) \
    return relu ? launch_bwd_cfg<P, T, R, L, ACT_RELU>(a, s) : launch_bwd_cfg<P, T, R, L, ACT_MISH>(a, s);
  if constexpr (P::ESIZE == 2) {
    DPPO_BWD(2, 4, false) DPPO_BWD(2, 2, true) DPPO_BWD(4, 4, false) DPPO_BWD(4, 2, true) DPPO_BWD(8, 1, false)
    DPPO_BWD(8, 1, true)
  } else {
    DPPO_BWD(2, 4, false) DPPO_BWD(2, 2, true) DPPO_BWD(4, 2, false) DPPO_BWD(4, 1, true) DPPO_BWD(8, 1, false)
    DPPO_BWD(8, 1, true)
  }
#undef DPPO_BWD
  return -1;
}
template int launch_fused_backward<F32>(const dppo_net_desc&, const FusedBwdArgs&, hipStream_t);
template int launch_fused_backward<BF16>(const dppo_net_desc&, const FusedBwdArgs&, hipStream_t);

template <class P>
__global__ void pack_stream_kernel(const PackStream d) {
  pack_stream_block<P>(d.layer[blockIdx.y], d.TPW, blockIdx.x);
}
template <class P>
void launch_pack_stream(const PackStream& d, hipStream_t s) {
  int maxks = 0;
  for (int l = 0; l < d.n_layers; ++l) maxks = d.layer[l].KS > maxks ? d.layer[l].KS : maxks;
  hipLaunchKernelGGL((pack_stream_kernel<P>), dim3(SAMPLER_WAVES * maxks * d.TPW, d.n_layers), dim3(64), 0, s, d);
}
template void launch_pack_stream<F32>(const PackStream&, hipStream_t);
template void launch_pack_stream<BF16>(const PackStream&, hipStream_t);

__global__ __launch_bounds__(1024) void reduce_slots_kernel(const float* in, int tiles, int n, const SlotOuts o) {
  __shared__ float red[16][65];
  const int cl = threadIdx.x & 63, rl = threadIdx.x >> 6;
  const int c = blockIdx.x * 64 + cl;
  const float* src = in + (size_t)blockIdx.y * tiles * n;
  float p[4] = {0.f, 0.f, 0.f, 0.f};
  if (c < n) {
    int r = rl;
    for (; r + 48 < tiles; r += 64) {
#pragma unroll
      for (int u = 0; u < 4; ++u) p[u] += src[(size_t)(r + 16 * u) * n + c];
    }
    for (; r < tiles; r += 16) p[0] += src[(size_t)r * n + c];
  }
  red[rl][cl] = (p[0] + p[1]) + (p[2] + p[3]);
  __syncthreads();
  if (rl == 0 && c < n) {
    float s = 0.f;
#pragma unroll
    for (int i = 0; i < 16; ++i) s += red[i][cl];
    if (c < o.n[blockIdx.y]) o.out[blockIdx.y][c] = s;
  }
}
void launch_reduce_slots(const float* in, int tiles, int n, const SlotOuts& o, hipStream_t s) {
  hipLaunchKernelGGL(reduce_slots_kernel, dim3((n + 63) / 64, o.n_slots), dim3(1024), 0, s, in, tiles, n, o);
}

}
```

### dppo_amd/hip.py

```python
from __future__ import annotations

import ctypes as C
import os
from typing import Optional

import numpy as np
import torch

LIB_PATH = os.environ.get("DPPO_HIP_LIB") or os.path.join(os.path.dirname(os.path.abspath(__file__)), "lib",
                                                          "libdppo_hip.so")

PREC_F32, PREC_BF16 = 0, 1
ACT_RELU, ACT_MISH = 0, 1
STAT_PG_LOSS, STAT_V_LOSS, STAT_APPROX_KL, STAT_CLIPFRAC, STAT_RATIO, STAT_ADV_MEAN, STAT_ADV_STD = range(7)
STAT_COUNT = 8

PREC_BY_NAME = {"fp32": PREC_F32, "f32": PREC_F32, "float32": PREC_F32, "bf16": PREC_BF16, "bfloat16": PREC_BF16}


class NetDesc(C.Structure):
    _fields_ = [(n, C.c_int32) for n in
                ("kind", "in_dim", "hidden", "n_blocks", "out_dim", "act", "time_dim", "act_flat", "cond_dim",
                 "cond_hidden", "cond_out", "use_layernorm", "plain")]

# ... 36 lines not shown
                ("dim", C.c_int32), ("n_levels", C.c_int32), ("mults", C.c_int32 * 4), ("kernel_size", C.c_int32),
                ("n_groups", C.c_int32), ("larger_encoder", C.c_int32), ("cond_predict_scale", C.c_int32),
                ("act", C.c_int32), ("groupnorm_eps", C.c_float)]

class VisDesc(C.Structure):
    _fields_ = [("in_ch", C.c_int32), ("img_h", C.c_int32), ("img_w", C.c_int32), ("embed_dim", C.c_int32),
                ("num_heads", C.c_int32), ("depth", C.c_int32), ("embed_norm", C.c_int32), ("prop_dim", C.c_int32),
                ("spatial_emb", C.c_int32), ("num_img", C.c_int32)]


class GmmCfg(C.Structure):
    _fields_ = [("horizon_steps", C.c_int32), ("action_dim", C.c_int32), ("num_modes", C.c_int32), ("std_mode", C.c_int32),
                ("norm_adv", C.c_int32), ("has_vclip", C.c_int32), ("deterministic", C.c_int32), ("pad", C.c_int32),
                ("fixed_std", C.c_float), ("logvar_min", C.c_float), ("logvar_max", C.c_float), ("ent_coef", C.c_float),
                ("clip_ploss_coef", C.c_double), ("clip_vloss_coef", C.c_double), ("seed_lo", C.c_uint32),
                ("seed_hi", C.c_uint32)]


class GemmNTDesc(C.Structure):
    _fields_ = [("X", C.c_void_p), ("W", C.c_void_p), ("bias", C.c_void_p), ("M", C.c_int64), ("N", C.c_int32),
                ("Kp", C.c_int32), ("ldx", C.c_int32), ("ldw", C.c_int32), ("dsrc", C.c_void_p), ("dsrc_kind", C.c_int32),
                ("dsrc_ld", C.c_int32), ("dact", C.c_int32), ("ldres", C.c_int32), ("res", C.c_void_p), ("add", C.c_void_p),
                ("out_f32", C.c_void_p), ("out_pre", C.c_void_p), ("out_act", C.c_void_p), ("ldadd", C.c_int32),
                ("ldo32", C.c_int32), ("ldo", C.c_int32), ("act", C.c_int32)]


class GemmTNJob(C.Structure):
    _fields_ = [("A", C.c_void_p), ("B", C.c_void_p), ("slab", C.c_void_p), ("M", C.c_int64), ("lda", C.c_int32),
                ("N1", C.c_int32), ("ldb", C.c_int32), ("N2", C.c_int32), ("rows_per_split", C.c_int32),
                ("ncol_a", C.c_int32), ("ncol_b", C.c_int32), ("pad", C.c_int32)]


class IdqlBatch(C.Structure):
    _fields_ = [("obs", C.c_void_p), ("next_obs", C.c_void_p), ("actions", C.c_void_p), ("reward", C.c_void_p),
                ("terminated", C.c_void_p), ("inds", C.c_void_p), ("cap", C.c_int64), ("n_envs", C.c_int64),
                ("head", C.c_int64), ("count", C.c_int64)]


IDQL_STAT_COUNT = 3

DP_HOOK_FN = C.CFUNCTYPE(None, C.c_void_p, C.c_void_p)


class DpHook(C.Structure):
    _fields_ = [("critic_grads_enqueued", DP_HOOK_FN), ("user", C.c_void_p)]


class ObsIO(C.Structure):
    _fields_ = [("obs_critic", C.c_void_p), ("d_obs_actor", C.c_void_p), ("d_obs_critic", C.c_void_p)]


STEP_DTYPE = np.dtype([("net", "<i4"), ("t", "<i4"), ("chain_slot", "<i4"), ("final_clip", "<i4"),
                       ("c0", "<f4"), ("c1", "<f4"), ("c2", "<f4"), ("c3", "<f4"), ("std", "<f4"), ("pad", "<f4")])
assert STEP_DTYPE.itemsize == 40

_P, _I, _L, _D = C.c_void_p, C.c_int, C.c_int64, C.c_double
_ND = C.POINTER(NetDesc)
SYMBOLS = {
    "dppo_version": (C.c_int, []),
    "dppo_last_error": (C.c_char_p, []),
    "dppo_net_param_count": (_L, [_ND]),
    "dppo_packed_bytes": (_L, [_ND, _I, _I]),
    "dppo_pack_net": (_I, [_ND, _I, _I, _P, _P, _P]),
    "dppo_mlp_forward_workspace_bytes": (_L, [_ND, _I, _L]),
    "dppo_actor_forward": (_I, [_ND, _I, _P, _P, _P, _P, _P, _L, _P, _P, _L, _P]),
    "dppo_critic_forward": (_I, [_ND, _I, _P, _P, _P, _L, _P, _P, _L, _P]),
    "dppo_sample_chain_workspace_bytes": (_L, [_ND, _I, _L]),
    "dppo_sample_chain_exchange_bytes": (_L, [_ND, _I, _L]),
    "dppo_sample_chain": (_I, [_ND, _I, _P, _P, _P, _P, C.POINTER(DiffusionCfg), _P, _I, _P, _P, _L, _P, _P, _I, _I,
                               _P, _L, _P]),
    "dppo_plain_sample_workspace_bytes": (_L, [_ND, _I, _L]),
    "dppo_plain_sample_chain": (_I, [_ND, _I, _P, _P, _P, _P, C.POINTER(DiffusionCfg), _P, _I, _P, _P, _L, _P, _P, _I, _I, _P,
                                     _L, _P]),
    "dppo_chain_logprob_workspace_bytes": (_L, [_ND, _I, _L, _I]),
    "dppo_chain_logprob": (_I, [_ND, _I, _P, _P, C.POINTER(DiffusionCfg), _P, _I, _P, _P, _L, _P, _P, _L, _P]),
    "dppo_bc_loss_workspace_bytes": (_L, [_ND, _I, _L, _I]),
    "dppo_bc_loss_fwd_bwd": (_I, [_ND, _I, _P, _P, C.POINTER(DiffusionCfg), _P, _I, _P, _P, _L, _P, _P, _P, _L, _P]),
    "dppo_axpy": (_I, [_P, _P, _D, _L, _P]),
    "dppo_denoise_mse_workspace_bytes": (_L, [_ND, _I, _L]),
    "dppo_denoise_mse_fwd_bwd": (_I, [_ND, _I, _P, _P, _P, _I, _P, _P, _P, _L, _P, _P, _P, _L, _P]),
    "dppo_gae": (_I, [_P, _P, _P, _P, _I, _I, _D, _D, _D, _P, _P, _P, _P, _P]),
    "dppo_ppo_workspace_bytes": (_L, [_ND, _ND, _I, _L]),
    "dppo_ppo_loss_fwd_bwd": (_I, [_ND, _ND, _I, _P, _P, _P, _P, C.POINTER(DiffusionCfg), C.POINTER(PpoCfg), _P,
                                   _P, _P, _P, _P, _P, _P, _P, _P, _L, _P, _P, _P, _P, _P, _L, _P]),
    "dppo_ppo_loss_fwd_bwd_dp": (_I, [_ND, _ND, _I, _P, _P, _P, _P, C.POINTER(DiffusionCfg), C.POINTER(PpoCfg), _P,
                                      _P, _P, _P, _P, _P, _P, _P, _P, _L, _P, _P, _P, _P, _P, _L, _P, C.POINTER(DpHook)]),
    "dppo_gaussian_workspace_bytes": (_L, [_ND, _ND, _I, _L]),
    "dppo_gaussian_sample": (_I, [_ND, _I, _P, _P, C.POINTER(GaussianCfg), _P, _P, _P, _L, _P, _P, _P, _L, _P]),
    "dppo_gaussian_logprob": (_I, [_ND, _I, _P, _P, C.POINTER(GaussianCfg), _P, _P, _P, _L, _P, _P, _L, _P]),
    "dppo_gaussian_ppo_loss_fwd_bwd": (_I, [_ND, _ND, _I, _P, _P, _P, _P, C.POINTER(GaussianCfg), _P, _P, _P, _P, _P, _P,
                                            _P, _L, _P, _P, _P, _P, _P, _P, _L, _P]),
    "dppo_unet_param_count": (_L, [C.POINTER(UnetDesc)]),
    "dppo_unet_packed_bytes": (_L, [C.POINTER(UnetDesc), _I, _I]),
    "dppo_gmm_workspace_bytes": (_L, [_ND, _ND, _ND, _I, _L]),
    "dppo_gmm_sample": (_I, [_ND, _ND, _I, _P, _P, _P, _P, C.POINTER(GmmCfg), _P, _P, _P, _P, _L, _P, _P, _L, _P]),
    "dppo_gmm_logprob": (_I, [_ND, _ND, _I, _P, _P, _P, _P, C.POINTER(GmmCfg), _P, _P, _P, _L, _P, _P, _L, _P]),
    "dppo_gmm_ppo_loss_fwd_bwd": (_I, [_ND, _ND, _ND, _I, _P, _P, _P, _P, _P, _P, C.POINTER(GmmCfg), _P, _P, _P, _P, _P, _P, _P,
                                       _L, _P, _P, _P, _P, _P, _P, _P, _L, _P]),
    "dppo_gaussian_bc_workspace_bytes": (_L, [_ND, _I, _L]),
    "dppo_gaussian_bc_loss_fwd_bwd": (_I, [_ND, _I, _P, _P, C.POINTER(GaussianCfg), _P, _P, _P, _L, _D, _P, _P, _P, _P, _L, _P]),
    "dppo_gmm_bc_workspace_bytes": (_L, [_ND, _ND, _I, _L]),
    "dppo_gmm_bc_loss_fwd_bwd": (_I, [_ND, _ND, _I, _P, _P, _P, _P, C.POINTER(GmmCfg), _P, _P, _P, _L, _P, _P, _P, _P, _P, _L,
                                      _P]),
    "dppo_idql_v_loss_workspace_bytes": (_L, [_ND, _ND, _I, _L, _I]),
    "dppo_idql_v_loss_fwd_bwd": (_I, [_ND, _ND, _I, _P, _P, _P, _P, _P, C.POINTER(IdqlBatch), _L, _D, _I, _P, _P, _P, _P, _L, _P]),
    "dppo_idql_q_loss_workspace_bytes": (_L, [_ND, _ND, _I, _L, _I]),
    "dppo_idql_q_loss_fwd_bwd": (_I, [_ND, _ND, _I, _P, _P, _P, _P, _P, C.POINTER(IdqlBatch), _L, _D, _I, _P, _P, _P, _L, _P]),
    "dppo_idql_q_forward_workspace_bytes": (_L, [_ND, _I, _L, _I]),
    "dppo_idql_q_forward": (_I, [_ND, _I, _P, _P, _P, _P, _I, _L, _P, _L, _I, _P, _P, _P, _L, _P]),
    "dppo_idql_select": (_I, [_P, _P, _P, _I, _P, _P, _L, _I, _I, _I, _D, C.c_uint64, _P, _P, _P]),
    "dppo_polyak": (_I, [_P, _P, _D, _L, _P]),
    "dppo_ppo_loss_fwd_bwd_obs": (_I, [_ND, _ND, _I, _P, _P, _P, _P, C.POINTER(DiffusionCfg), C.POINTER(PpoCfg), _P,
                                       _P, _P, _P, _P, _P, _P, _P, _L, _P, _P, _P, _P, _P, _L, _P, C.POINTER(ObsIO)]),
    "dppo_unet_ppo_loss_fwd_bwd_obs": (_I, [C.POINTER(UnetDesc), _ND, _I, _P, _P, _P, _P, C.POINTER(DiffusionCfg),
                                            C.POINTER(PpoCfg), _P, _P, _P, _P, _P, _P, _P, _P, _L, _P, _P, _P, _P, _P, _L, _P,
                                            C.POINTER(ObsIO)]),
    "dppo_gaussian_ppo_loss_fwd_bwd_obs": (_I, [_ND, _ND, _I, _P, _P, _P, _P, C.POINTER(GaussianCfg), _P, _P, _P, _P, _P, _P,
                                            _P, _L, _P, _P, _P, _P, _P, _P, _L, _P, C.POINTER(ObsIO)]),
    "dppo_denoise_mse_fwd_bwd_obs": (_I, [_ND, _I, _P, _P, _P, _I, _P, _P, _P, _L, _P, _P, _P, _L, _P, _P]),
    "dppo_unet_denoise_mse_fwd_bwd_obs": (_I, [C.POINTER(UnetDesc), _I, _P, _P, _P, _I, _P, _P, _P, _L, _P, _P, _P, _L, _P, _P]),
    "dppo_vis_param_count": (_L, [C.POINTER(VisDesc)]),
    "dppo_vis_packed_bytes": (_L, [C.POINTER(VisDesc), _I]),
    "dppo_vis_pack": (_I, [C.POINTER(VisDesc), _I, _P, _P, _P]),
    "dppo_vis_workspace_bytes": (_L, [C.POINTER(VisDesc), _I, _L, _I]),
    "dppo_vis_encode": (_I, [C.POINTER(VisDesc), _I, _P, _P, _P, _I, _P, _L, _P, _I, _I, _P, _L, _P]),
    "dppo_vis_backward": (_I, [C.POINTER(VisDesc), _I, _P, _P, _P, _I, _L, _P, _P, _L, _P]),
    "dppo_unet_pack": (_I, [C.POINTER(UnetDesc), _I, _I, _P, _P, _P]),
    "dppo_unet_workspace_bytes": (_L, [C.POINTER(UnetDesc), _I, _L]),
    "dppo_unet_sample_workspace_bytes": (_L, [C.POINTER(UnetDesc), _I, _L, _I]),
    "dppo_unet_forward": (_I, [C.POINTER(UnetDesc), _I, _P, _P, _P, _P, _P, _L, _P, _P, _L, _P]),
    "dppo_unet_sample_chain": (_I, [C.POINTER(UnetDesc), _I, _P, _P, _P, _P, C.POINTER(DiffusionCfg), _P, _I, _P, _P, _L, _P,
                                    _P, _I, _I, _P, _L, _P]),
    "dppo_unet_chain_logprob": (_I, [C.POINTER(UnetDesc), _I, _P, _P, C.POINTER(DiffusionCfg), _P, _P, _I, _P, _P, _L, _P, _P,
                                     _L, _P]),
    "dppo_unet_ppo_workspace_bytes": (_L, [C.POINTER(UnetDesc), _ND, _I, _L]),
    "dppo_unet_ppo_loss_fwd_bwd": (_I, [C.POINTER(UnetDesc), _ND, _I, _P, _P, _P, _P, C.POINTER(DiffusionCfg),
                                        C.POINTER(PpoCfg), _P, _P, _P, _P, _P, _P, _P, _P, _P, _L, _P, _P, _P, _P, _P, _L, _P]),
    "dppo_unet_denoise_mse_workspace_bytes": (_L, [C.POINTER(UnetDesc), _I, _L]),
    "dppo_unet_denoise_mse_fwd_bwd": (_I, [C.POINTER(UnetDesc), _I, _P, _P, _P, _I, _P, _P, _P, _L, _P, _P, _P, _L, _P]),
    "dppo_grad_sq_norm": (_I, [_P, _L, _P, _P, _P]),
    "dppo_adamw_step": (_I, [_P, _P, _P, _P, _L, _I, _D, _D, _D, _D, _D, _P, _D, _P]),
    "dppo_adamw_step_dev": (_I, [_P, _P, _P, _P, _L, _P, _P, _D, _D, _D, _D, _P, _D, _P]),
    "dppo_adamw_step_multi": (_I, [_P, _I, _P]),
    "dppo_pack_nets": (_I, [_ND, _I, _P, _P, _ND, _I, _P, _P, _I, _P]),
    "dppo_stats_split": (_I, [_P, _P, _P]),
    "dppo_stats_merge": (_I, [_P, _P, _I, _P]),
    "dppo_stats_merge_n": (_I, [_P, _P, _I, _I, _P]),
    "dppo_probe_arm": (_I, [_I, _I]),
    "dppo_probe_collect": (_I, [C.POINTER(C.c_double), C.POINTER(C.c_int), C.POINTER(C.c_double)]),
    "dppo_probe_collect_bytes": (_I, [C.POINTER(C.c_double), C.POINTER(C.c_int), C.POINTER(C.c_double),
                                      C.POINTER(C.c_double)]),
    "dppo_tune_set": (_I, [_I, _I]),
    "dppo_backward_route": (_I, [_ND, _I, _L, _I, _I, C.POINTER(C.c_int)]),
    "dppo_gemm_nt_raw": (_I, [_I, _P, _P, _P, _L, _I, _I, _P, _P, _I, _I, _P]),
    "dppo_gemm_tn_raw": (_I, [_I, _P, _I, _I, _P, _I, _I, _L, _I, _P, _P, _P]),
    "dppo_gemm_nt_desc_raw": (_I, [_I, C.POINTER(GemmNTDesc), _P]),
    "dppo_gemm_tn_group_raw": (_I, [_I, C.POINTER(GemmTNJob), _I, C.POINTER(C.c_void_p), _P]),
    "dppo_gemm_tn_job_raw": (_I, [_I, C.POINTER(GemmTNJob), _P, _P]),
}

_lib: Optional[C.CDLL] = None


class DppoHipError(RuntimeError):
    pass


def load() -> C.CDLL:
    global _lib
    if _lib is None:
        if not os.path.exists(LIB_PATH):
            raise DppoHipError(
                f"{LIB_PATH} not found: build it with dppo_amd/csrc/build.sh (or __graft_entry__.build()). "
                "dppo_amd has no CPU fallback.")
        lib = C.CDLL(LIB_PATH)
        for name, (res, args) in SYMBOLS.items():
            fn = getattr(lib, name)
            fn.restype, fn.argtypes = res, args
        for kv in filter(None, os.environ.get("DPPO_TUNE", "").split(",")):
            k, v = kv.split("=")
            if lib.dppo_tune_set(int(k), int(v)) != 0:
                raise DppoHipError(f"DPPO_TUNE: bad knob {kv!r}: {lib.dppo_last_error().decode()}")
        _lib = lib
    return _lib


def check(rc: int, what: str) -> None:
    if rc != 0:
        msg = load().dppo_last_error().decode()
        raise DppoHipError(f"{what} failed (rc={rc}): {msg}")


def ptr(t: Optional[torch.Tensor]) -> Optional[int]:
    if t is None:
        return None
    assert t.is_contiguous(), "dppo_amd kernels take contiguous tensors"
    return t.data_ptr()


_raw_stream = getattr(torch._C, "_cuda_getCurrentRawStream", None)


def stream() -> int:
    if _raw_stream is not None:
        return _raw_stream(torch.cuda.current_device())
    return torch.cuda.current_stream().cuda_stream


def require_gpu(t: torch.Tensor, what: str) -> None:
    if not t.is_cuda:
        raise DppoHipError(f"{what}: tensor is on {t.device}; the DPPO hot path runs on an MI355X only "
                           "(no CPU fallback)")


class Workspace:

    def __init__(self):
        self.buf: Optional[torch.Tensor] = None

    def get(self, nbytes: int, device) -> torch.Tensor:
        if self.buf is None or self.buf.numel() < nbytes or self.buf.device != torch.device(device):
            self.buf = torch.zeros(max(int(nbytes), 256), dtype=torch.uint8, device=device)
        return self.buf
```

### include/dppo_hip.h

```cpp
#ifndef DPPO_HIP_H
#define DPPO_HIP_H

#include <stddef.h>
#include <stdint.h>

#ifdef __cplusplus
extern "C" {
#endif

#define DPPO_PREC_F32 0
#define DPPO_PREC_BF16 1

#define DPPO_ACT_RELU 0
#define DPPO_ACT_MISH 1

typedef void* dppo_stream_t;

typedef struct dppo_net_desc {
  int32_t kind;
  int32_t in_dim;
  int32_t hidden;
  int32_t n_blocks;
  int32_t out_dim;
  int32_t act;
// ... 105 lines not shown
int dppo_gae(const double* reward, const float* values, const float* terminated, const float* last_values,
             int n_steps, int n_envs, double gamma, double gae_lambda, double reward_scale_const, double* adv64,
             double* ret64, float* adv32, float* ret32, dppo_stream_t stream);

int64_t dppo_ppo_workspace_bytes(const dppo_net_desc* actor, const dppo_net_desc* critic, int prec, int64_t N);
int dppo_ppo_loss_fwd_bwd(const dppo_net_desc* actor, const dppo_net_desc* critic, int prec,
                          const float* actor_params, const void* actor_packed, const float* critic_params,
                          const void* critic_packed, const dppo_diffusion_cfg* dcfg, const dppo_ppo_cfg* pcfg,
                          const dppo_step* ksteps, const float* obs_k, const float* chains_k,
                          const float* returns_k, const float* values_k, const float* adv_k,
                          const float* logprobs_k, const int64_t* inds, const int64_t* kinds, int64_t N,
                          const double* global_moments, float* actor_grad, float* critic_grad, double* stats,
                          void* workspace, int64_t workspace_bytes, dppo_stream_t stream);

typedef struct dppo_dp_hook {
  void (*critic_grads_enqueued)(void* user, dppo_stream_t side);
  void* user;
} dppo_dp_hook;
int dppo_ppo_loss_fwd_bwd_dp(const dppo_net_desc* actor, const dppo_net_desc* critic, int prec, const float* actor_params,
                             const void* actor_packed, const float* critic_params, const void* critic_packed,
                             const dppo_diffusion_cfg* dcfg, const dppo_ppo_cfg* pcfg, const dppo_step* ksteps,
                             const float* obs_k, const float* chains_k, const float* returns_k, const float* values_k,
                             const float* adv_k, const float* logprobs_k, const int64_t* inds, const int64_t* kinds,
                             int64_t N, const double* global_moments, float* actor_grad, float* critic_grad,
                             double* stats, void* workspace, int64_t workspace_bytes, dppo_stream_t stream,
                             const dppo_dp_hook* hook);

typedef struct dppo_gaussian_cfg {
  int32_t horizon_steps, action_dim;
  int32_t tanh_mean;
  int32_t std_mode;
  int32_t norm_adv, has_vclip;
  int32_t deterministic;
  int32_t pad;
  float fixed_std, logvar_min, logvar_max, randn_clip;
  double clip_ploss_coef, clip_vloss_coef;
  uint32_t seed_lo, seed_hi;
} dppo_gaussian_cfg;
#define DPPO_GAUSS_STAT_ENTROPY 7
#define DPPO_GAUSS_STAT_STD 8
#define DPPO_GAUSS_STAT_COUNT 9
int64_t dppo_gaussian_workspace_bytes(const dppo_net_desc* actor, const dppo_net_desc* critic, int prec, int64_t N);
int dppo_gaussian_sample(const dppo_net_desc* actor, int prec, const float* params, const void* packed,
                         const dppo_gaussian_cfg* cfg, const float* logvar, const float* obs, const float* noise,
                         int64_t B, float* actions, float* mean_out, void* workspace, int64_t workspace_bytes,
                         dppo_stream_t stream);
int dppo_gaussian_logprob(const dppo_net_desc* actor, int prec, const float* params, const void* packed,
                          const dppo_gaussian_cfg* cfg, const float* logvar, const float* obs, const float* actions,
                          int64_t N, float* logp, void* workspace, int64_t workspace_bytes, dppo_stream_t stream);
int dppo_gaussian_ppo_loss_fwd_bwd(const dppo_net_desc* actor, const dppo_net_desc* critic, int prec,
                                   const float* actor_params, const void* actor_packed, const float* critic_params,
                                   const void* critic_packed, const dppo_gaussian_cfg* cfg, const float* logvar,
                                   const float* obs, const float* actions, const float* returns,
                                   const float* oldvalues, const float* adv, const float* oldlogp, int64_t N,
                                   const double* global_moments, float* actor_grad, float* critic_grad,
                                   float* logvar_grad, double* stats, void* workspace, int64_t workspace_bytes,
                                   dppo_stream_t stream);
int64_t dppo_gaussian_bc_workspace_bytes(const dppo_net_desc* actor, int prec, int64_t N);
int dppo_gaussian_bc_loss_fwd_bwd(const dppo_net_desc* actor, int prec, const float* params, const void* packed,
                                  const dppo_gaussian_cfg* cfg, const float* logvar, const float* obs, const float* actions,
                                  int64_t N, double ent_coef, float* grad, float* logvar_grad, double* loss_entropy,
                                  void* workspace, int64_t workspace_bytes, dppo_stream_t stream);

typedef struct dppo_unet_desc {
  int32_t action_dim, cond_dim, horizon_steps;
  int32_t time_dim;
  int32_t dim, n_levels;
  int32_t mults[4];
  int32_t kernel_size, n_groups;
  int32_t larger_encoder;
  int32_t cond_predict_scale;
  int32_t act;
  float groupnorm_eps;
} dppo_unet_desc;
int64_t dppo_unet_param_count(const dppo_unet_desc* net);
int64_t dppo_unet_packed_bytes(const dppo_unet_desc* net, int prec, int n_time);
int dppo_unet_pack(const dppo_unet_desc* net, int prec, int n_time, const float* params, void* packed,
                   dppo_stream_t stream);
int64_t dppo_unet_workspace_bytes(const dppo_unet_desc* net, int prec, int64_t rows);
int64_t dppo_unet_sample_workspace_bytes(const dppo_unet_desc* net, int prec, int64_t B, int n_steps);
int dppo_unet_forward(const dppo_unet_desc* net, int prec, const float* params, const void* packed, const float* x,
                      const int64_t* t, const float* state, int64_t rows, float* eps, void* workspace,
                      int64_t workspace_bytes, dppo_stream_t stream);
int dppo_unet_sample_chain(const dppo_unet_desc* net, int prec, const float* params_base, const void* packed_base,
                           const float* params_ft, const void* packed_ft, const dppo_diffusion_cfg* cfg,
                           const dppo_step* sched_host, int n_steps, const float* obs, const float* noise, int64_t B,
                           float* traj, float* chains, int chain_len, int init_slot, void* workspace,
                           int64_t workspace_bytes, dppo_stream_t stream);
int64_t dppo_unet_ppo_workspace_bytes(const dppo_unet_desc* actor, const dppo_net_desc* critic, int prec, int64_t N);
int dppo_unet_ppo_loss_fwd_bwd(const dppo_unet_desc* actor, const dppo_net_desc* critic, int prec, const float* actor_params,
                               const void* actor_packed, const float* critic_params, const void* critic_packed,
                               const dppo_diffusion_cfg* dcfg, const dppo_ppo_cfg* pcfg, const dppo_step* ksteps,
                               const float* obs_k, const float* chains_k, const float* returns_k, const float* values_k,
                               const float* adv_k, const float* logprobs_k, const int64_t* inds, const int64_t* kinds,
                               int64_t N, const double* global_moments, float* actor_grad, float* critic_grad,
                               double* stats, void* workspace, int64_t workspace_bytes, dppo_stream_t stream);
int64_t dppo_unet_denoise_mse_workspace_bytes(const dppo_unet_desc* net, int prec, int64_t N);
int dppo_unet_denoise_mse_fwd_bwd(const dppo_unet_desc* net, int prec, const float* params, const void* packed,
                                  const dppo_step* tsteps, int n_time, const float* obs, const float* pairs,
                                  const int64_t* kinds, int64_t N, float* grad, double* loss, void* workspace,
                                  int64_t workspace_bytes, dppo_stream_t stream);
int dppo_unet_chain_logprob(const dppo_unet_desc* net, int prec, const float* params, const void* packed,
                            const dppo_diffusion_cfg* cfg, const dppo_step* ksteps, const dppo_step* ksteps_host,
                            int Kft, const float* obs, const float* chains, int64_t B, float* logp, void* workspace,
                            int64_t workspace_bytes, dppo_stream_t stream);

int dppo_grad_sq_norm(const float* grad, int64_t n, double* scratch, double* out, dppo_stream_t stream);
int dppo_adamw_step(float* params, const float* grad, float* exp_avg, float* exp_avg_sq, int64_t n, int step,
                    double lr, double beta1, double beta2, double eps, double weight_decay, const double* sq_norm,
                    double max_norm, dppo_stream_t stream);
int dppo_adamw_step_dev(float* params, const float* grad, float* exp_avg, float* exp_avg_sq, int64_t n, int32_t* step_dev,
                        const float* lr_dev, double beta1, double beta2, double eps, double weight_decay,
                        const double* sq_norm, double max_norm, dppo_stream_t stream);

typedef struct dppo_adamw_slot {
  float* params;
  const float* grad;
  float* exp_avg;
  float* exp_avg_sq;
  int64_t n;
  int32_t* step_dev;
  const float* lr_dev;
  double beta1, beta2, eps, weight_decay;
  const double* sq_norm;
  double max_norm;
} dppo_adamw_slot;
int dppo_adamw_step_multi(const dppo_adamw_slot* slots, int n_slots, dppo_stream_t stream);

int dppo_stats_split(const double* stats, float* hi_lo, dppo_stream_t stream);
int dppo_stats_merge(const float* hi_lo, double* stats, int world, dppo_stream_t stream);
int dppo_stats_merge_n(const float* hi_lo, double* stats, int world, int n_avg, dppo_stream_t stream);

int dppo_probe_arm(int kernel_id, int max_launches);
int dppo_probe_collect(double* total_ms_host, int* launches_host, double* flops_host);
int dppo_probe_collect_bytes(double* total_ms_host, int* launches_host, double* flops_host, double* bytes_host);

int dppo_tune_set(int knob, int value);
#define DPPO_ROUTE_IN_ZEROED 1
#define DPPO_ROUTE_IN_DOBS 2
#define DPPO_ROUTE_IN_SIDE 4
#define DPPO_ROUTE_FUSED 0x001
#define DPPO_ROUTE_ONE_BLOCK 0x002
#define DPPO_ROUTE_LOWRANK 0x004
#define DPPO_ROUTE_MERGED 0x008
#define DPPO_ROUTE_ONEHOT 0x010
#define DPPO_ROUTE_DW0 0x020
#define DPPO_ROUTE_DW0_NHOT 0x040
#define DPPO_ROUTE_DW0_ROUND 0x080
#define DPPO_ROUTE_NEED_AUX 0x100
#define DPPO_ROUTE_SIDE_TAIL 0x200
#define DPPO_ROUTE_TAIL_POST 0x400
#define DPPO_ROUTE_POST_ONE 0x800
int dppo_backward_route(const dppo_net_desc* net, int prec, int64_t M, int Kft, int flags, int* mask_out);
int dppo_gemm_nt_raw(int prec, const void* X, const void* W, const float* bias, int64_t M, int N, int Kp,
                     float* out_f32, void* out_elem, int ldo, int act, dppo_stream_t stream);
int dppo_gemm_tn_raw(int prec, const void* A, int lda, int N1, const void* B, int ldb, int N2, int64_t M,
                     int rows_per_split, float* slab, float* C, dppo_stream_t stream);
typedef struct dppo_gemm_nt_desc {
  const void* X;
  const void* W;
  const float* bias;
  int64_t M;
  int32_t N, Kp, ldx, ldw;
  const void* dsrc;
  int32_t dsrc_kind, dsrc_ld, dact, ldres;
  const float* res;
  const void* add;
  float* out_f32;
  void* out_pre;
  void* out_act;
  int32_t ldadd, ldo32, ldo, act;
} dppo_gemm_nt_desc;
int dppo_gemm_nt_desc_raw(int prec, const dppo_gemm_nt_desc* desc, dppo_stream_t stream);
typedef struct dppo_gemm_tn_job {
  const void* A;
  const void* B;
  float* slab;
  int64_t M;
  int32_t lda, N1, ldb, N2, rows_per_split, ncol_a, ncol_b, pad;
} dppo_gemm_tn_job;
int dppo_gemm_tn_group_raw(int prec, const dppo_gemm_tn_job* jobs, int n, float* const* C_out, dppo_stream_t stream);
int dppo_gemm_tn_job_raw(int prec, const dppo_gemm_tn_job* job, float* C, dppo_stream_t stream);

typedef struct dppo_gmm_cfg {
  int32_t horizon_steps, action_dim, num_modes;
  int32_t std_mode;
  int32_t norm_adv, has_vclip;
  int32_t deterministic;
  int32_t pad;
  float fixed_std, logvar_min, logvar_max;
  float ent_coef;
  double clip_ploss_coef, clip_vloss_coef;
  uint32_t seed_lo, seed_hi;
} dppo_gmm_cfg;
int64_t dppo_gmm_workspace_bytes(const dppo_net_desc* mean, const dppo_net_desc* weights, const dppo_net_desc* critic, int prec,
                                 int64_t N);
int dppo_gmm_sample(const dppo_net_desc* mean, const dppo_net_desc* weights, int prec, const float* mean_params,
                    const void* mean_packed, const float* weights_params, const void* weights_packed, const dppo_gmm_cfg* cfg,
                    const float* logvar, const float* obs, const int64_t* modes, const float* noise, int64_t B, float* actions,
                    void* workspace, int64_t workspace_bytes, dppo_stream_t stream);
int dppo_gmm_logprob(const dppo_net_desc* mean, const dppo_net_desc* weights, int prec, const float* mean_params,
                     const void* mean_packed, const float* weights_params, const void* weights_packed, const dppo_gmm_cfg* cfg,
                     const float* logvar, const float* obs, const float* actions, int64_t N, float* logp, void* workspace,
                     int64_t workspace_bytes, dppo_stream_t stream);
int dppo_gmm_ppo_loss_fwd_bwd(const dppo_net_desc* mean, const dppo_net_desc* weights, const dppo_net_desc* critic, int prec,
                              const float* mean_params, const void* mean_packed, const float* weights_params,
                              const void* weights_packed, const float* critic_params, const void* critic_packed,
                              const dppo_gmm_cfg* cfg, const float* logvar, const float* obs, const float* actions,
                              const float* returns, const float* oldvalues, const float* adv, const float* oldlogp, int64_t N,
                              const double* global_moments, float* mean_grad, float* weights_grad, float* critic_grad,
                              float* logvar_grad, double* stats, void* workspace, int64_t workspace_bytes, dppo_stream_t stream);
int64_t dppo_gmm_bc_workspace_bytes(const dppo_net_desc* mean, const dppo_net_desc* weights, int prec, int64_t N);
int dppo_gmm_bc_loss_fwd_bwd(const dppo_net_desc* mean, const dppo_net_desc* weights, int prec, const float* mean_params,
                             const void* mean_packed, const float* weights_params, const void* weights_packed,
                             const dppo_gmm_cfg* cfg, const float* logvar, const float* obs, const float* actions, int64_t N,
                             float* mean_grad, float* weights_grad, float* logvar_grad, double* loss_entropy, void* workspace,
                             int64_t workspace_bytes, dppo_stream_t stream);

typedef struct dppo_obs_io {
  const float* obs_critic;
  float* d_obs_actor;
  float* d_obs_critic;
} dppo_obs_io;
int dppo_ppo_loss_fwd_bwd_obs(const dppo_net_desc* actor, const dppo_net_desc* critic, int prec, const float* actor_params,
                              const void* actor_packed, const float* critic_params, const void* critic_packed,
                              const dppo_diffusion_cfg* dcfg, const dppo_ppo_cfg* pcfg, const dppo_step* ksteps,
                              const float* obs_k, const float* chains_k, const float* returns_k, const float* values_k,
                              const float* adv_k, const float* logprobs_k, const int64_t* kinds, int64_t N,
                              const double* global_moments, float* actor_grad, float* critic_grad, double* stats,
                              void* workspace, int64_t workspace_bytes, dppo_stream_t stream, const dppo_obs_io* io);
int dppo_unet_ppo_loss_fwd_bwd_obs(const dppo_unet_desc* actor, const dppo_net_desc* critic, int prec, const float* actor_params,
                                   const void* actor_packed, const float* critic_params, const void* critic_packed,
                                   const dppo_diffusion_cfg* dcfg, const dppo_ppo_cfg* pcfg, const dppo_step* ksteps,
                                   const float* obs_k, const float* chains_k, const float* returns_k, const float* values_k,
                                   const float* adv_k, const float* logprobs_k, const int64_t* kinds, int64_t N,
                                   const double* global_moments, float* actor_grad, float* critic_grad, double* stats,
                                   void* workspace, int64_t workspace_bytes, dppo_stream_t stream, const dppo_obs_io* io);
int dppo_gaussian_ppo_loss_fwd_bwd_obs(const dppo_net_desc* actor, const dppo_net_desc* critic, int prec,
                                       const float* actor_params, const void* actor_packed, const float* critic_params,
                                       const void* critic_packed, const dppo_gaussian_cfg* cfg, const float* logvar,
                                       const float* obs, const float* actions, const float* returns,
                                       const float* oldvalues, const float* adv, const float* oldlogp, int64_t N,
                                       const double* global_moments, float* actor_grad, float* critic_grad,
                                       float* logvar_grad, double* stats, void* workspace, int64_t workspace_bytes,
                                       dppo_stream_t stream, const dppo_obs_io* io);
int dppo_denoise_mse_fwd_bwd_obs(const dppo_net_desc* actor, int prec, const float* params, const void* packed,
                                 const dppo_step* tsteps, int n_time, const float* obs, const float* pairs,
                                 const int64_t* kinds, int64_t N, float* grad, double* loss, void* workspace,
                                 int64_t workspace_bytes, dppo_stream_t stream, float* d_obs);
int dppo_unet_denoise_mse_fwd_bwd_obs(const dppo_unet_desc* net, int prec, const float* params, const void* packed,
                                      const dppo_step* tsteps, int n_time, const float* obs, const float* pairs,
                                      const int64_t* kinds, int64_t N, float* grad, double* loss, void* workspace,
                                      int64_t workspace_bytes, dppo_stream_t stream, float* d_obs);

typedef struct dppo_vis_desc {
  int32_t in_ch;
  int32_t img_h, img_w;
  int32_t embed_dim, num_heads, depth;
  int32_t embed_norm;
  int32_t prop_dim;
  int32_t spatial_emb;
  int32_t num_img;
} dppo_vis_desc;
int64_t dppo_vis_param_count(const dppo_vis_desc* net);
int64_t dppo_vis_packed_bytes(const dppo_vis_desc* net, int prec);
int dppo_vis_pack(const dppo_vis_desc* net, int prec, const float* params, void* packed, dppo_stream_t stream);
int64_t dppo_vis_workspace_bytes(const dppo_vis_desc* net, int prec, int64_t B, int train);
int dppo_vis_encode(const dppo_vis_desc* net, int prec, const float* params, const void* packed, const void* rgb, int rgb_u8,
                    const float* state, int64_t B, float* obs, int ld_obs, int train, void* workspace,
                    int64_t workspace_bytes, dppo_stream_t stream);
int dppo_vis_backward(const dppo_vis_desc* net, int prec, const float* params, const void* packed, const float* d_obs,
                      int ld_dobs, int64_t B, float* grad, void* workspace, int64_t workspace_bytes, dppo_stream_t stream);

typedef struct dppo_idql_batch {
  const float* obs;
  const float* next_obs;
  const float* actions;
  const float* reward;
  const float* terminated;
  const int64_t* inds;
  int64_t cap, n_envs, head, count;
} dppo_idql_batch;
#define DPPO_IDQL_STAT_COUNT 3
int64_t dppo_idql_v_loss_workspace_bytes(const dppo_net_desc* q, const dppo_net_desc* v, int prec, int64_t N, int double_q);
int dppo_idql_v_loss_fwd_bwd(const dppo_net_desc* q, const dppo_net_desc* v, int prec, const float* target_q_params,
                             const void* target_q1_packed, const void* target_q2_packed, const float* v_params,
                             const void* v_packed, const dppo_idql_batch* batch, int64_t N, double expectile, int double_q,
                             float* v_grad, float* adv_out, double* stats, void* workspace, int64_t workspace_bytes,
                             dppo_stream_t stream);
int64_t dppo_idql_q_loss_workspace_bytes(const dppo_net_desc* q, const dppo_net_desc* v, int prec, int64_t N, int double_q);
int dppo_idql_q_loss_fwd_bwd(const dppo_net_desc* q, const dppo_net_desc* v, int prec, const float* q_params,
                             const void* q1_packed, const void* q2_packed, const float* v_params, const void* v_packed,
                             const dppo_idql_batch* batch, int64_t N, double gamma, int double_q, float* q_grad, double* stats,
                             void* workspace, int64_t workspace_bytes, dppo_stream_t stream);
int64_t dppo_idql_q_forward_workspace_bytes(const dppo_net_desc* q, int prec, int64_t N, int double_q);
int dppo_idql_q_forward(const dppo_net_desc* q, int prec, const float* q_params, const void* q1_packed, const void* q2_packed,
                        const float* obs, int obs_dim, int64_t obs_rows, const float* actions, int64_t N, int double_q,
                        float* q1_out, float* q2_out, void* workspace, int64_t workspace_bytes, dppo_stream_t stream);
int dppo_idql_select(const float* q1, const float* q2, const float* v, int v_per_env, const float* candidates, const float* u,
                     int64_t B, int S, int width, int mode, double h, uint64_t seed, float* actions, int32_t* idx,
                     dppo_stream_t stream);
int dppo_polyak(float* target, const float* source, double tau, int64_t n, dppo_stream_t stream);

#ifdef __cplusplus
}
#endif
// ... 2 lines not shown
```

Baseline: 142.9 million samples/s.

## Fuse PPO policy loss into merged actor forward kernel epilogue

Adds a loss-fused variant of the merged fused forward kernel. It computes per-element diffusion log-probs, the clipped PPO policy loss, the d_eps gradient and per-tile loss partials directly from the output tile held in LDS, instead of writing eps to global memory and launching a separate loss kernel. The chain, logprob and advantage loads are prefetched while the GEMMs run, to hide their latency. In exchange it adds LDS use, pins VGPRs at 112, and depends on narrow shape conditions: bf16, hidden 512, two streams, and the moment rider off.

```diff
diff --git a/dppo_amd/csrc/api.hip b/dppo_amd/csrc/api.hip
--- a/dppo_amd/csrc/api.hip
+++ b/dppo_amd/csrc/api.hip
@@ -497,9 +497,13 @@
 
 template <class P>
 static void mlp_forward(const dppo_net_desc& d, const float* prm, const char* pk, const PackLayout& L, int64_t M,
-                        MlpBufs<P>& B, bool keep, hipStream_t s) {
+                        MlpBufs<P>& B, bool keep, hipStream_t s, const LossArgs* fuse_loss = nullptr) {
   const ParamLayout pl = param_layout(d);
   const int H = d.hidden, nb = d.n_blocks;
+  if (fuse_loss != nullptr && !(fused_ok<P>(d) && B.route.merged)) {
+    g_fused_fault = -8;
+    return;
+  }
   if (fused_ok<P>(d)) {
     FusedFwdArgs f;
     memset(&f, 0, sizeof(f));
@@ -525,7 +529,7 @@
       f.ostream0 = (const u32x4*)(pk + L.ostream0), f.ostream2 = (const u32x4*)(pk + L.ostream2);
       f.cbias2 = (const float*)(pk + L.cbias2);
     }
-    g_fused_fault = launch_fused_forward<P>(d, f, s);
+    g_fused_fault = launch_fused_forward<P>(d, f, s, fuse_loss);
     return;
   }
   if (d.plain) {
@@ -593,9 +597,9 @@
   }
   return &t;
 }
+static bool side_stream_on(int idx) { return (((g_overlap == 1 ? 7 : g_overlap >> 1) >> idx) & 1) != 0; }
 static hipStream_t fork_side(hipStream_t main, int idx = 0) {
-  const int mask = g_overlap == 1 ? 7 : g_overlap >> 1;
-  SideStream* t = ((mask >> idx) & 1) ? side_stream(idx) : nullptr;
+  SideStream* t = side_stream_on(idx) ? side_stream(idx) : nullptr;
   if (t == nullptr) return main;
   (void)hipEventRecord(t->fork, main);
   (void)hipStreamWaitEvent(t->s, t->fork, 0);
@@ -621,6 +625,7 @@
 }
 static int g_mom_rider = 0;
 constexpr int64_t MOM_RIDER_MAX_N = 16384;
+static bool mom_rider_on(int64_t N, bool has_gmom) { return !has_gmom && (g_mom_rider == 1 || (g_mom_rider == 0 && N <= MOM_RIDER_MAX_N)); }
 static int g_temb_onehot = 1;
 static int g_dw0 = 1;
 static int g_side_tail = 1;
@@ -1600,6 +1605,14 @@
   });
 }
 
+static int g_fuse_loss = 1;
+template <class P>
+static bool fuse_loss_ok(const dppo_net_desc& d, int64_t N, bool has_gmom, bool two_streams, int Kft) {
+  if (!g_fuse_loss || P::ESIZE != 2 || !two_streams || mom_rider_on(N, has_gmom)) return false;
+  if (!fused_ok<P>(d) || !fused_can_merge<P>(d) || !fused_loss_shape(d, Kft)) return false;
+  return d.kind == 0 && d.out_dim == d.act_flat && d.act_flat <= 16 && pack_layout<P>(d, 0).Kpo % 8 == 0;
+}
+
 template <class P>
 static int ppo_impl(const dppo_net_desc& a, const dppo_net_desc& cr, const float* ap, const char* ak, const float* cp,
                     const char* ck, const dppo_diffusion_cfg& dcfg, const dppo_ppo_cfg& pcfg, const dppo_step* ksteps,
@@ -1630,7 +1643,7 @@
   br.inA = W.A.in, br.KpA = LA.Kp0, br.inC = W.C.in, br.KpC = LC.Kp0, br.brow = W.brow, br.krow = W.krow;
   br.obs_in_a = a.cond_hidden > 0 ? 0 : 1;
   br.onehot0 = W.A.route.onehot_col;
-  const bool mom_rider = gmom == nullptr && (g_mom_rider == 1 || (g_mom_rider == 0 && N <= MOM_RIDER_MAX_N));
+  const bool mom_rider = mom_rider_on(N, gmom != nullptr);
   if (mom_rider) br.mom_adv = adv_k, br.mom_out = W.moments, br.n_zero_b = 8;
   const float* obs_c = oio && oio->obs_critic ? oio->obs_critic : nullptr;
   const bool split = s2 != s || obs_c != nullptr;
@@ -1659,6 +1672,9 @@
   la.tab = Kft <= 1024 ? W.loss_tab : nullptr;
   la.d_eps = W.A.d_out, la.ldde = LA.Kpo, la.d_v = W.C.d_out, la.lddv = LC.Kpo, la.stats = stats;
   const bool two_streams = s2 != s;
+  LossArgs lpol = la;
+  lpol.part = 1, lpol.partial = W.loss_partial;
+  const bool fuse_loss = fuse_loss_ok<P>(a, N, gmom != nullptr, two_streams, Kft);
   mlp_forward<P>(cr, cp, ck, LC, N, W.C, true, s2);
   if (two_streams) {
     la.part = 2, la.partial = W.loss_partial_v;
@@ -1671,9 +1687,9 @@
     if (oio && oio->d_obs_critic) obs_grad<P>(cr, cp, N, W.C, oio->d_obs_critic, s2);
     if (hook && hook->critic_grads_enqueued) hook->critic_grads_enqueued(hook->user, (dppo_stream_t)s2);
   }
-  mlp_forward<P>(a, ap, ak, LA, N, W.A, true, s);
+  mlp_forward<P>(a, ap, ak, LA, N, W.A, true, s, fuse_loss ? &lpol : nullptr);
   la.part = two_streams ? 1 : 3, la.partial = W.loss_partial;
-  launch_ppo_loss<P>(la, s);
+  if (!fuse_loss) launch_ppo_loss<P>(la, s);
   if (!two_streams) {
     mlp_backward<P>(cr, cp, ck, LC, N, W.C, cgrad, nullptr, nullptr, 0, s);
     if (oio && oio->d_obs_critic) obs_grad<P>(cr, cp, N, W.C, oio->d_obs_critic, s);
@@ -2754,6 +2770,7 @@
     case 38: g_side_tail = value; return 0;
     case 39: case 40: return retired_knob(knob);
     case 41: g_tail_post = value; return 0;
+    case 42: g_fuse_loss = value; return 0;
     default: break;
   }
   return fail(-1, "unknown tuning knob %d", knob);
@@ -2779,6 +2796,15 @@
 #define CALL(P) route_mask<P>(*net, M, Kft, flags, mask_out)
   return DPPO_DISPATCH(prec, CALL);
 #undef CALL
+}
+
+int dppo_ppo_loss_route(const dppo_net_desc* actor, const dppo_net_desc* critic, int prec, int64_t N, int has_global_moments) {
+  if (int e = check_net(actor)) return e;
+  if (int e = check_net(critic)) return e;
+  if (int e = check_prec(prec)) return e;
+  if (N < 2 || N > 0x7fffffff) return fail(-1, "N out of range");
+  if (prec == DPPO_PREC_F32) return fuse_loss_ok<F32>(*actor, N, has_global_moments != 0, side_stream_on(0), 0) ? 1 : 0;
+  return fuse_loss_ok<BF16>(*actor, N, has_global_moments != 0, side_stream_on(0), 0) ? 1 : 0;
 }
 
 int dppo_gemm_nt_raw(int prec, const void* X, const void* W, const float* bias, int64_t M, int N, int Kp, float* out_f32,
diff --git a/dppo_amd/csrc/fused.h b/dppo_amd/csrc/fused.h
--- a/dppo_amd/csrc/fused.h
+++ b/dppo_amd/csrc/fused.h
@@ -64,8 +64,10 @@
 int fused_bwd_one_grid(const dppo_net_desc& d, int64_t M);
 bool fused_dw0_shape(const dppo_net_desc& d);
 
+struct LossArgs;
 template <class P>
-int launch_fused_forward(const dppo_net_desc& d, const FusedFwdArgs& a, hipStream_t s);
+int launch_fused_forward(const dppo_net_desc& d, const FusedFwdArgs& a, hipStream_t s, const LossArgs* loss = nullptr);
+bool fused_loss_shape(const dppo_net_desc& d, int Kft);
 template <class P>
 int launch_fused_backward(const dppo_net_desc& d, const FusedBwdArgs& a, hipStream_t s);
 void set_fused_short_tiles(int v);
diff --git a/dppo_amd/csrc/fused.hip b/dppo_amd/csrc/fused.hip
--- a/dppo_amd/csrc/fused.hip
+++ b/dppo_amd/csrc/fused.hip
@@ -4,6 +4,7 @@
 #include "gemm.h"
 #include "tile_ln.h"
 #include "pack_dev.h"
+#include "loss_dev.h"
 
 #ifndef DPPO_BWD_LATE
 #define DPPO_BWD_LATE 1
@@ -662,8 +663,9 @@
   }
 }
 
-template <class P, int TPW, int MR, int OT, int ACT, int S1>
-__device__ __forceinline__ void fused_forward_merged_body(const FusedFwdArgs& a) {
+template <class P, int TPW, int MR, int OT, int ACT, int S1, bool LOSSF>
+__device__ __forceinline__ void fused_forward_merged_body(const FusedFwdArgs& a, const LossArgs& la) {
+  static_assert(!LOSSF || (OT == 1 && MR == 4 && TPW == 4 && S1 > 0 && P::ESIZE == 2), "fused policy loss: bf16, one out tile, 64-row tiles of H = 512");
   constexpr int PD = ring_depth<TPW, MR>(), ES = P::ESIZE, KB = P::KB;
   static_assert(S1 == 0 || PD == 4, "the compact walk is written for a ring of four positions");
   constexpr int H = 128 * TPW, KSH = H / KB, HRB = H * ES, MT = 16 * MR;
@@ -689,6 +691,16 @@
   u32x4* woutL = (u32x4*)(biasL + ((2 * H + OT * 16 + 3) & ~3));
   u32x4* w0cL = woutL + (WIDE ? 0 : KSH * OT * 64);
   char* xin = WIDE ? (char*)(w0cL + ks0v * OT * 64) : bufB;
+  long long* metaL = (long long*)(w0cL + ks0v * OT * 64);
+  double* statL = (double*)(metaL + 3 * MT);
+  float* stepL = (float*)(statL + 4 * MT);
+  float* tabL = stepL + (LOSSF ? la.pcfg.ft_denoising_steps * LOSS_STEP : 0);
+  float* epsL = (float*)(bufA + 16 * 1024);
+  float* lpnL = (float*)(bufA + 40 * 1024);
+  float* lpoL = lpnL + MT * LOSS_ROW;
+  float* gsL = lpoL + MT * LOSS_ROW;
+  float* coefL = (float*)(bufA + 56 * 1024);
+  static_assert(!LOSSF || (40 * 1024 + 3 * MT * LOSS_ROW * 4 <= 56 * 1024 && 56 * 1024 + MT * 4 <= MT * HRB), "fused policy loss: buffer A layout");
   const int wbase = wid * 16 * TPW;
   const int to_w = wid % OT, kh_w = wid / OT;
   for (int idx = tid; idx < 2 * H; idx += 512) biasL[idx] = a.params[a.bias_off[idx / H] + idx % H];
@@ -696,6 +708,23 @@
   if constexpr (!WIDE)
     for (int idx = tid; idx < KSH * OT * 64; idx += 512) woutL[idx] = a.ostream2[idx];
   for (int idx = tid; idx < ks0v * OT * 64; idx += 512) w0cL[idx] = a.ostream0[idx];
+  if constexpr (LOSSF) {
+    const int Kft = la.pcfg.ft_denoising_steps;
+    for (int k = tid; k < 2 * Kft; k += 512) tabL[k] = la.tab[k];
+    for (int k = tid; k < Kft; k += 512) {
+      const dppo_step st = la.ksteps[k];
+      float* sl = stepL + k * LOSS_STEP;
+      sl[0] = st.c0, sl[1] = st.c1, sl[2] = st.c2, sl[3] = st.c3, sl[4] = st.std;
+      sl[5] = la.tab[2 * Kft + k];
+    }
+    if (tid == 0) {
+      const double Nm = la.moments[2], mean = la.moments[0] / Nm;
+      const double varu = (la.moments[1] - Nm * mean * mean) / (Nm - 1.0);
+      tabL[2 * Kft] = (float)mean;
+      tabL[2 * Kft + 1] = (float)sqrt(varu > 0 ? varu : 0);
+      tabL[2 * Kft + 2] = (float)(la.n_count > 0 ? la.n_count : Nm);
+    }
+  }
   if (tid < 16) flags[tid] = 0;
   uint32_t seq = 0;
 
@@ -712,8 +741,32 @@
     const int row0 = tile * MT;
     STAMP(0);
     load_tile<MT>(xin, in_rb, in_km, (const char*)a.in, a.ld_in * ES, row0, M);
+    if constexpr (LOSSF) {
+      int t_ = tid;
+      asm volatile("" : "+v"(t_));
+      if (t_ < MT) {
+        const int n = row0 + t_, Kft = la.pcfg.ft_denoising_steps, AF = la.AF;
+        const long long b = n < M ? la.brow[n] : 0, k = n < M ? la.krow[n] : 0;
+        metaL[3 * t_] = la.gathered ? b * 2 * AF : (b * (Kft + 1) + k) * AF;
+        metaL[3 * t_ + 1] = la.gathered ? b * AF : (b * Kft + k) * AF;
+        metaL[3 * t_ + 2] = (b << 32) | k;
+      }
+    }
     __syncthreads();
     STAMP(1);
+    uint32_t warm = 0;
+    if constexpr (LOSSF) {
+      int t_ = tid;
+      asm volatile("" : "+v"(t_));
+      const int row = t_ / 5, part = t_ - row * 5;
+      if (row < MT && row0 + row < M) {
+        const int AF = la.AF;
+        const float* src = part < 2   ? la.chains + lds_load(metaL + 3 * row) + (part ? 2 * AF - 1 : 0)
+                           : part < 4 ? la.logprobs_k + lds_load(metaL + 3 * row + 1) + (part == 3 ? AF - 1 : 0)
+                                      : la.adv_k + (int)(lds_load(metaL + 3 * row + 2) >> 32);
+        warm = *(const uint32_t*)src;
+      }
+    }
     f32x4 acc[TPW][MR];
     auto bias_init = [&](int layer) {
 #pragma unroll
@@ -759,6 +812,25 @@
       eng.run(acc, bufA, HRB, 15, KSH, r, g, FLAGS ? flags : nullptr, seq);
     }
     STAMP(5);
+    float lx[2] = {0.f, 0.f}, lxn[2] = {0.f, 0.f}, lo[2] = {0.f, 0.f}, ladv = 0.f;
+    if constexpr (LOSSF) {
+      asm volatile("" ::"v"(warm));
+      int ln = lane;
+      asm volatile("" : "+v"(ln));
+      const int AF = la.AF, sm = 8 * wid + (ln >> 3), slot = ln & 7;
+      const int cnt = (la.pcfg.reward_horizon < la.pcfg.horizon_steps ? la.pcfg.reward_horizon : la.pcfg.horizon_steps) * la.pcfg.action_dim;
+      if (row0 + sm < M) {
+        const float* ch = la.chains + lds_load(metaL + 3 * sm);
+        const float* ol = la.logprobs_k + lds_load(metaL + 3 * sm + 1);
+#pragma unroll
+        for (int q = 0; q < 2; ++q) {
+          const int j = slot + 8 * q;
+          if (j < cnt) lx[q] = glb_load(ch + j), lxn[q] = glb_load(ch + AF + j), lo[q] = glb_load(ol + j);
+        }
+      }
+      if (ln < 8 && row0 + 8 * wid + ln < M) ladv = glb_load(la.adv_k + (int)(lds_load(metaL + 3 * (8 * wid + ln) + 2) >> 32));
+      asm volatile("" : "+v"(lx[0]), "+v"(lxn[0]), "+v"(lo[0]), "+v"(lx[1]), "+v"(lxn[1]), "+v"(lo[1]), "+v"(ladv)::"memory");
+    }
     emit<P, TPW, MR>(acc, ACT, bufB, a.a2[0], H, wbase, g, r, row0, M, a.z1[0]);
     STAMP(6);
     __syncthreads();
@@ -815,18 +887,78 @@
       float s = biasL[2 * H + j];
 #pragma unroll
       for (int kh = 0; kh < KSPLIT; ++kh) s += part[(((kh * MR + m) * OT + to) * 16 + jj) * 16 + rr];
-      if (row0 + row < M)
+      if constexpr (LOSSF)
+        epsL[row * 16 + j] = s;
+      else if (row0 + row < M)
         a.out[(size_t)(row0 + row) * a.ldout + j] = s;
     }
     STAMP(13);
+    if constexpr (LOSSF) {
+      __syncthreads();
+      int ln = lane;
+      asm volatile("" : "+v"(ln));
+      const int cnt = (la.pcfg.reward_horizon < la.pcfg.horizon_steps ? la.pcfg.reward_horizon : la.pcfg.horizon_steps) * la.pcfg.action_dim;
+      const int sm = 8 * wid + (ln >> 3), slot = ln & 7;
+      {
+        const int k = (int)(lds_load(metaL + 3 * sm + 2) & 0xffffffffll);
+#pragma unroll
+        for (int q = 0; q < 2; ++q) {
+          const int j = slot + 8 * q;
+          if (j < cnt) {
+            float lpn, lpo, gs;
+            loss_element_nc(la.dcfg, stepL + k * LOSS_STEP, lx[q], lxn[q], lds_load(epsL + sm * 16 + j), lo[q], lpn, lpo, gs);
+            lpnL[sm * LOSS_ROW + j] = lpn, lpoL[sm * LOSS_ROW + j] = lpo, gsL[sm * LOSS_ROW + j] = gs;
+          }
+        }
+      }
+      asm volatile("s_waitcnt lgkmcnt(0)" ::: "memory");
+      __builtin_amdgcn_wave_barrier();
+      if (ln < 8) {
+        const int s1 = 8 * wid + ln;
+        double s4[4] = {0, 0, 0, 0};
+        float coef = 0.f;
+        if (row0 + s1 < M) {
+          const int k = (int)(lds_load(metaL + 3 * s1 + 2) & 0xffffffffll);
+          coef = policy_loss_sample_nc(la.pcfg, tabL, k, ladv, lpnL + s1 * LOSS_ROW, lpoL + s1 * LOSS_ROW, cnt, s4);
+        }
+        coefL[s1] = coef;
+#pragma unroll
+        for (int q = 0; q < 4; ++q) statL[4 * s1 + q] = s4[q];
+      }
+      asm volatile("s_waitcnt lgkmcnt(0)" ::: "memory");
+      __builtin_amdgcn_wave_barrier();
+      if (row0 + sm < M) {
+        const float coef = lds_load(coefL + sm);
+        typename P::elem_t* de = (typename P::elem_t*)la.d_eps + (size_t)(row0 + sm) * la.ldde;
+        for (int c = slot; c < la.ldde / 8; c += 8) *(u32x4*)(de + c * 8) = policy_loss_chunk_nc(coef, gsL + sm * LOSS_ROW, c, cnt);
+      }
+    }
     __syncthreads();
     STAMP(14);
+    if constexpr (LOSSF) {
+      if (wid < 4) {
+        int ln = lane;
+        asm volatile("" : "+v"(ln));
+        double v = lds_load(statL + 4 * ln + wid);
+        for (int off = 32; off > 0; off >>= 1) v += __shfl_down(v, off);
+        if (ln == 0) {
+          double* po = la.partial + (size_t)tile * 8;
+          po[wid == 0 ? DPPO_STAT_PG_LOSS : wid == 1 ? DPPO_STAT_APPROX_KL : wid == 2 ? DPPO_STAT_CLIPFRAC : DPPO_STAT_RATIO] = v;
+          if (wid == 0) po[DPPO_STAT_V_LOSS] = 0.0;
+        }
+      }
+    }
   }
 }
 
 template <class P, int TPW, int MR, int OT, int ACT, int S1>
 __global__ __launch_bounds__(512, 2) void fused_forward_merged_kernel(const FusedFwdArgs a) {
-  fused_forward_merged_body<P, TPW, MR, OT, ACT, S1>(a);
+  fused_forward_merged_body<P, TPW, MR, OT, ACT, S1, false>(a, LossArgs{});
+}
+template <class P, int TPW, int MR, int ACT, int S1>
+__global__ __launch_bounds__(512, 2) __attribute__((amdgpu_num_vgpr(112))) void fused_forward_merged_loss_kernel(const FusedFwdArgs a,
+                                                                                                              const LossArgs la) {
+  fused_forward_merged_body<P, TPW, MR, 1, ACT, S1, true>(a, la);
 }
 
 template <class P, int TPW, int MR, bool LN, int ACT, int OCC>
@@ -1347,22 +1479,42 @@
 template bool fused_can_merge<F32>(const dppo_net_desc&);
 template bool fused_can_merge<BF16>(const dppo_net_desc&);
 
-template <class P, int TPW, int MR, int ACT, int S1, int OT = 1>
-static int launch_fwd_merged_cfg2(const FusedFwdArgs& a, hipStream_t s) {
+constexpr int FUSED_LOSS_MAX_KFT = 64;
+static size_t fused_loss_lds(int Kft) { return (size_t)64 * (3 * 8 + 4 * 8) + ((size_t)(Kft * (LOSS_STEP + 2) + 3) * 4 + 15) / 16 * 16; }
+template <class P, int TPW, int MR, int ACT, int S1, int OT = 1, bool LOSSF = false>
+static int launch_fwd_merged_cfg2(const FusedFwdArgs& a, hipStream_t s, const LossArgs* loss = nullptr) {
   constexpr int MT = 16 * MR, H = 128 * TPW;
-  const size_t lds = merged_lds<P>(H, OT, a.ks0v);
+  const size_t lds = merged_lds<P>(H, OT, a.ks0v) + (LOSSF ? fused_loss_lds(loss->pcfg.ft_denoising_steps) : 0);
   if (lds > 160 * 1024 || a.Kp0 > H || a.nb != 1) return -2;
+  if (LOSSF != (loss != nullptr)) return -4;
   static DevLatch attr;
   const int ntiles = (a.M + MT - 1) / MT;
+  if constexpr (LOSSF) {
+    if (loss->pcfg.ft_denoising_steps > FUSED_LOSS_MAX_KFT) return -4;
+    raise_lds(fused_forward_merged_loss_kernel<P, TPW, MR, ACT, S1>, attr);
+    const bool probe = probe_begin(PROBE_FUSED_FWD, s);
+    hipLaunchKernelGGL((fused_forward_merged_loss_kernel<P, TPW, MR, ACT, S1>), dim3(ntiles < NUM_CUS ? ntiles : NUM_CUS), dim3(512), lds, s,
+                       a, *loss);
+    if (probe) probe_end(s, 2.0 * a.M * ((double)a.in_valid * H + 2.0 * a.nb * H * H + (double)H * a.out_dim));
+    return 0;
+  } else {
   raise_lds(fused_forward_merged_kernel<P, TPW, MR, OT, ACT, S1>, attr);
   const bool probe = probe_begin(PROBE_FUSED_FWD, s);
   hipLaunchKernelGGL((fused_forward_merged_kernel<P, TPW, MR, OT, ACT, S1>), dim3(ntiles < NUM_CUS ? ntiles : NUM_CUS), dim3(512),
                      lds, s, a);
   if (probe) probe_end(s, 2.0 * a.M * ((double)a.in_valid * H + 2.0 * a.nb * H * H + (double)H * a.out_dim));
   return 0;
+  }
 }
 template <class P, int TPW, int MR, int ACT>
-static int launch_fwd_merged_cfg(const FusedFwdArgs& a, hipStream_t s) {
+static int launch_fwd_merged_cfg(const FusedFwdArgs& a, hipStream_t s, const LossArgs* loss) {
+  if (loss != nullptr) {
+    if constexpr (P::ESIZE == 2 && MR == 4 && TPW == 4 && ring_depth<TPW, MR>() == 4) {
+      if (a.out_dim <= 16 && fused_compact_on() && a.ks0v == 1) return launch_fwd_merged_cfg2<P, TPW, MR, ACT, 1, 1, true>(a, s, loss);
+      if (a.out_dim <= 16 && fused_compact_on() && a.ks0v == 2) return launch_fwd_merged_cfg2<P, TPW, MR, ACT, 2, 1, true>(a, s, loss);
+    }
+    return -4;
+  }
   if (a.out_dim > 16) {
     if constexpr (TPW == 4) {
       if (a.ks0v == 1) return launch_fwd_merged_cfg2<P, TPW, MR, ACT, 1, 4>(a, s);
@@ -1378,15 +1530,19 @@
   return launch_fwd_merged_cfg2<P, TPW, MR, ACT, 0>(a, s);
 }
 
+bool fused_loss_shape(const dppo_net_desc& d, int Kft) {
+  return fused_compact_on() && d.hidden == 512 && d.out_dim <= 16 && d.in_dim <= 2 * BF16::KB && Kft <= FUSED_LOSS_MAX_KFT &&
+         fused_can_merge<BF16>(d) && pick_mr<BF16>(d.hidden) == 4;
+}
 template <class P>
-int launch_fused_forward(const dppo_net_desc& d, const FusedFwdArgs& a, hipStream_t s) {
+int launch_fused_forward(const dppo_net_desc& d, const FusedFwdArgs& a, hipStream_t s, const LossArgs* loss) {
   const int tpw = d.hidden / 128, mr = pick_mr<P>(d.hidden);
   const int nt = (d.out_dim + 15) / 16, ot = nt <= 1 ? 1 : (nt <= 4 ? 4 : (nt <= 8 ? 8 : 0));
   if (mr == 0 || ot == 0 || a.M <= 0) return -1;
   const bool relu = a.act == ACT_RELU;
   if (a.merge_top) {
 #define DPPO_FWDM(T, R) \
-  if (tpw == T && mr == R) return relu ? launch_fwd_merged_cfg<P, T, R, ACT_RELU>(a, s) : launch_fwd_merged_cfg<P, T, R, ACT_MISH>(a, s);
+  if (tpw == T && mr == R) return relu ? launch_fwd_merged_cfg<P, T, R, ACT_RELU>(a, s, loss) : launch_fwd_merged_cfg<P, T, R, ACT_MISH>(a, s, loss);
     if constexpr (P::ESIZE == 2) {
       DPPO_FWDM(2, 8) DPPO_FWDM(4, 4)
     } else {
@@ -1395,6 +1551,7 @@
 #undef DPPO_FWDM
     return -1;
   }
+  if (loss != nullptr) return -4;
   if constexpr (P::ESIZE == 2) {
     if (short_tiles<P>(d.hidden, a.use_ln, 1) && ot == 1)
       return relu ? launch_fwd_cfg<P, 4, 2, 1, false, ACT_RELU, 2>(a, s) : launch_fwd_cfg<P, 4, 2, 1, false, ACT_MISH, 2>(a, s);
@@ -1415,8 +1572,8 @@
 #undef DPPO_FWD
   return -1;
 }
-template int launch_fused_forward<F32>(const dppo_net_desc&, const FusedFwdArgs&, hipStream_t);
-template int launch_fused_forward<BF16>(const dppo_net_desc&, const FusedFwdArgs&, hipStream_t);
+template int launch_fused_forward<F32>(const dppo_net_desc&, const FusedFwdArgs&, hipStream_t, const LossArgs*);
+template int launch_fused_forward<BF16>(const dppo_net_desc&, const FusedFwdArgs&, hipStream_t, const LossArgs*);
 
 template <class P, int TPW, int MR, bool LN, int ACT, int OCC = 1>
 static int launch_bwd_cfg(const FusedBwdArgs& a, hipStream_t s) {
diff --git a/dppo_amd/csrc/loss_dev.h b/dppo_amd/csrc/loss_dev.h
--- /dev/null
+++ b/dppo_amd/csrc/loss_dev.h
@@ -0,0 +1,111 @@
+#pragma once
+#include "common.h"
+#include "dppo_hip.h"
+#include "ppo.h"
+
+namespace dppo {
+
+#ifndef DPPO_LOG_SQRT_2PI
+#define DPPO_LOG_SQRT_2PI 0.91893853320467274178f
+#endif
+
+__device__ __forceinline__ void posterior_nc(const dppo_diffusion_cfg& c, const dppo_step& st, float x, float eps, float& mu,
+                                             float& dmu_deps) {
+#pragma clang fp contract(off)
+  if (!c.use_ddim) {
+    float x0 = st.c0 * x - st.c1 * eps;
+    float pass = 1.f;
+    if (c.has_denoised_clip) {
+      pass = (x0 >= -c.denoised_clip && x0 <= c.denoised_clip) ? 1.f : 0.f;
+      x0 = fminf(fmaxf(x0, -c.denoised_clip), c.denoised_clip);
+    }
+    mu = st.c2 * x0 + st.c3 * x;
+    dmu_deps = -(st.c2 * st.c1) * pass;
+  } else {
+    float x0 = (x - st.c1 * eps) / st.c0;
+    float dx0 = -st.c1 / st.c0;
+    float e2 = eps, de2 = 1.f;
+    if (c.has_denoised_clip) {
+      const float pass = (x0 >= -c.denoised_clip && x0 <= c.denoised_clip) ? 1.f : 0.f;
+      x0 = fminf(fmaxf(x0, -c.denoised_clip), c.denoised_clip);
+      dx0 *= pass;
+      e2 = (x - st.c0 * x0) / st.c1;
+      de2 = -(st.c0 / st.c1) * dx0;
+    }
+    if (c.has_eps_clip) {
+      const float pass = (e2 >= -c.eps_clip && e2 <= c.eps_clip) ? 1.f : 0.f;
+      e2 = fminf(fmaxf(e2, -c.eps_clip), c.eps_clip);
+      de2 *= pass;
+    }
+    mu = st.c2 * x0 + st.c3 * e2;
+    dmu_deps = st.c2 * dx0 + st.c3 * de2;
+  }
+}
+
+constexpr int LOSS_ROW = 17;
+constexpr int LOSS_STEP = 8;
+
+__device__ __forceinline__ void loss_element_nc(const dppo_diffusion_cfg& dc, const float* step, float x, float xn, float e, float o,
+                                                float& lpn, float& lpo, float& gs) {
+#pragma clang fp contract(off)
+  dppo_step st;
+  st.c0 = lds_load(step), st.c1 = lds_load(step + 1), st.c2 = lds_load(step + 2), st.c3 = lds_load(step + 3);
+  st.std = lds_load(step + 4);
+  const float var = st.std * st.std, lstd = lds_load(step + 5);
+  float mu, dmu;
+  posterior_nc(dc, st, x, e, mu, dmu);
+  const float d = xn - mu;
+  const float lp = -(d * d) / (2.f * var) - lstd - DPPO_LOG_SQRT_2PI;
+  lpn = fminf(fmaxf(lp, -5.f), 2.f);
+  lpo = fminf(fmaxf(o, -5.f), 2.f);
+  gs = (lp >= -5.f && lp <= 2.f) ? (d / var) * dmu : 0.f;
+}
+
+__device__ __forceinline__ float policy_loss_sample_nc(const dppo_ppo_cfg& pc, const float* tab, int k, float adv, const float* lpn,
+                                                       const float* lpo, int cnt, double (&s4)[4]) {
+#pragma clang fp contract(off)
+  const int Kft = pc.ft_denoising_steps;
+  float vn[16], vo[16];
+#pragma unroll
+  for (int j = 0; j < 16; ++j) vn[j] = lds_load(lpn + j), vo[j] = lds_load(lpo + j);
+  float sum_new = 0.f, sum_old = 0.f;
+#pragma unroll
+  for (int j = 0; j < 16; ++j) {
+    if (j < cnt) {
+      sum_new += vn[j];
+      sum_old += vo[j];
+    }
+  }
+  const float newlp = sum_new / (float)cnt, oldlp = sum_old / (float)cnt;
+  if (pc.norm_adv) adv = (adv - lds_load(tab + 2 * Kft)) / (lds_load(tab + 2 * Kft + 1) + 1e-8f);
+  if (pc.has_adv_clip) adv = fminf(fmaxf(adv, pc.adv_clip_lo), pc.adv_clip_hi);
+  adv *= lds_load(tab + k);
+  const float logratio = newlp - oldlp;
+  const float ratio = expf(logratio);
+  const float eps_k = lds_load(tab + Kft + k);
+  const float lo = 1.f - eps_k, hi = 1.f + eps_k;
+  const float rc = fminf(fmaxf(ratio, lo), hi);
+  const float pg1 = -adv * ratio, pg2 = -adv * rc;
+  const float w1 = pg1 > pg2 ? 1.f : (pg1 == pg2 ? 0.5f : 0.f);
+  const float within = (ratio >= lo && ratio <= hi) ? 1.f : 0.f;
+  const float dL_dratio = -adv * (w1 + (1.f - w1) * within);
+  const float coef = dL_dratio * ratio / (lds_load(tab + 2 * Kft + 2) * (float)cnt);
+  s4[0] = fmaxf(pg1, pg2);
+  s4[1] = (double)((ratio - 1.f) - logratio);
+  s4[2] = fabsf(ratio - 1.f) > eps_k ? 1.0 : 0.0;
+  s4[3] = ratio;
+  return coef;
+}
+
+__device__ __forceinline__ u32x4 policy_loss_chunk_nc(float coef, const float* gs, int c, int cnt) {
+#pragma clang fp contract(off)
+  float v[8];
+#pragma unroll
+  for (int q = 0; q < 8; ++q) v[q] = c * 8 + q < cnt ? coef * lds_load(gs + c * 8 + q) : 0.f;
+  u32x4 w;
+#pragma unroll
+  for (int q = 0; q < 4; ++q) w[q] = (uint32_t)f2bf(v[2 * q]) | ((uint32_t)f2bf(v[2 * q + 1]) << 16);
+  return w;
+}
+
+}
diff --git a/dppo_amd/hip.py b/dppo_amd/hip.py
--- a/dppo_amd/hip.py
+++ b/dppo_amd/hip.py
@@ -212,6 +212,7 @@
                                       C.POINTER(C.c_double)]),
     "dppo_tune_set": (_I, [_I, _I]),
     "dppo_backward_route": (_I, [_ND, _I, _L, _I, _I, C.POINTER(C.c_int)]),
+    "dppo_ppo_loss_route": (_I, [_ND, _ND, _I, _L, _I]),
     "dppo_gemm_nt_raw": (_I, [_I, _P, _P, _P, _L, _I, _I, _P, _P, _I, _I, _P]),
     "dppo_gemm_tn_raw": (_I, [_I, _P, _I, _I, _P, _I, _I, _L, _I, _P, _P, _P]),
     "dppo_gemm_nt_desc_raw": (_I, [_I, C.POINTER(GemmNTDesc), _P]),
diff --git a/include/dppo_hip.h b/include/dppo_hip.h
--- a/include/dppo_hip.h
+++ b/include/dppo_hip.h
@@ -281,6 +281,7 @@
 #define DPPO_ROUTE_TAIL_POST 0x400
 #define DPPO_ROUTE_POST_ONE 0x800
 int dppo_backward_route(const dppo_net_desc* net, int prec, int64_t M, int Kft, int flags, int* mask_out);
+int dppo_ppo_loss_route(const dppo_net_desc* actor, const dppo_net_desc* critic, int prec, int64_t N, int has_global_moments);
 int dppo_gemm_nt_raw(int prec, const void* X, const void* W, const float* bias, int64_t M, int N, int Kp,
                      float* out_f32, void* out_elem, int ldo, int act, dppo_stream_t stream);
 int dppo_gemm_tn_raw(int prec, const void* A, int lda, int N1, const void* B, int ldb, int N2, int64_t M,
```

Result: faster. 146.4 million samples/s (median of 6 runs) (+2.4%).
